# AY-Liu/Image-Editing-Framework

Hardware: AMD Instinct MI355X
Metric: denoising steps/sec (SD1.5 512x512 P2P edit step, UNet batch 4) (higher is better)
Workload: dtype f16x3; 1 GPU; sd15 UNet (859.5M params) P2P AttentionRefine edit step, 2 prompts x CFG = batch 4, 64x64 latents (512x512 px), 50-step DDIM, guidance 7.5, cross 0.8 / self 0.4, per-step null-text unconditional embeddings (P2P_NTI, edit_real.py); one independent edit per GPU; precision mode f16x3: fp32 storage; every contraction on split operands: hi + lo fp16 halves of each fp32 element, Ah Bh + Al Bh + Ah Bl =

## Files before the change

image-editing-framework_amd/control.py:

```python
from typing import Optional

import torch

from . import hip

XL = 96


def _step_hook(c):
    fn = getattr(c, "between_steps", None) or getattr(c, "after_step", None)
    if fn is not None:
        fn()


def advance_controller(c):
    c.cur_att_layer += 1
    uncond = c.num_att_layers if getattr(c, "LOW_RESOURCE", False) else 0
    if c.cur_att_layer == c.num_att_layers + uncond:
        c.cur_att_layer = 0
        c.cur_step += 1
        _step_hook(c)


class StepCounter:

    def __init__(self, num_att_layers: int = 0):
        self.cur_step, self.cur_att_layer, self.num_att_layers = 0, 0, num_att_layers

    def between_steps(self):
        pass

    def reset(self):
        self.cur_step, self.cur_att_layer = 0, 0


class ControlPlan:
    MASA_KINDS = ("masactrl", "masactrl_mask", "masactrl_mask_auto", "masactrl_union")
    GATED_KINDS = ("masactrl_mask", "masactrl_mask_auto")
    MAP_TOKENS, CTX_TOKENS = 256, 77

    def __init__(self, controller, kind: str, device, num_prompts: int = 1, num_steps: int = 0,
                 mt: Optional[torch.Tensor] = None, coef_table: Optional[torch.Tensor] = None,
                 self_window=(0, 0), self_max_tokens: int = 256, masa_steps=(), masa_layers=(),
                 pnp_layers=(), pnp_qk_steps: int = 0, pnp_conv_steps: int = 0, cond_only: bool = False,
                 mask_s: Optional[torch.Tensor] = None, mask_t: Optional[torch.Tensor] = None, mask_tokens=(),
                 auto_slots=None, auto_layers=None, auto_thres: float = 0.1, auto_ref=(), auto_cur=(), blend=None):
        self.controller = controller
        self.kind = kind
        self.device = torch.device(device)
        self.num_prompts = num_prompts
        self.cond_only = bool(cond_only)
        self.batch = num_prompts if cond_only else 2 * num_prompts
        self.num_steps = num_steps
        self.self_window = self_window
        self.self_max_tokens = self_max_tokens
        self.captured = False
        self.muted = False
        dev = self.device
        self.step = torch.zeros(1, dtype=torch.int32, device=dev)
        B, Bp = self.batch, num_prompts
        self.blend_modules = ()
        self.blend_w = self.blend_w_cur = self.blend_acc = self.blend_thres = None
        if blend is not None:
            mods, bw, thres = blend
            assert kind == "p2p" and not cond_only and tuple(bw.shape) == (num_steps + 1, Bp, 2, XL)
            self.blend_modules = tuple(int(i) for i in mods)
            self.blend_w = bw.to(device=dev, dtype=torch.float32).contiguous()
            self.blend_w_cur = torch.zeros(Bp, 2, XL, dtype=torch.float32, device=dev)
            self.blend_acc = torch.zeros(Bp, self.MAP_TOKENS, dtype=torch.float32, device=dev)
            self.blend_thres = torch.tensor([float(thres)], dtype=torch.float32, device=dev)
        if kind == "p2p":
            slots = Bp - 1
            assert mt.shape == (slots, XL, XL) and coef_table.shape == (num_steps + 1, slots, 2, XL)
            self.mt = mt.to(device=dev, dtype=torch.float16).contiguous()
            self.mt32 = mt.to(device=dev, dtype=torch.float32).contiguous()
            self.coef_table = coef_table.to(device=dev, dtype=torch.float32).contiguous()
            self.coef_cur = torch.zeros(slots, 2, XL, dtype=torch.float32, device=dev)
            ct = coef_table.detach().float()
            self.coef_bound = float((ct[:, :, 0].abs() + ct[:, :, 1].abs()).max()) if ct.numel() else 1.0
            off = 0 if cond_only else Bp
            es = torch.full((B,), -1, dtype=torch.int32)
            sl = torch.zeros(B, dtype=torch.int32)
            for k in range(slots):
                es[off + 1 + k] = off
                sl[off + 1 + k] = k
            self.edit_src, self.edit_slot = es.to(dev), sl.to(dev)
            ident = torch.arange(B, dtype=torch.int32)
            repl = ident.clone()
            repl[off + 1:] = off
            tab = ident.repeat(num_steps + 1, 1)
            lo, hi = self_window
            tab[lo:hi] = repl
            self.self_table = tab.contiguous().to(dev)
            self.self_cur = ident.clone().to(dev)
        self.masa_steps = set(int(s) for s in masa_steps)
        self.masa_layers = set(int(l) for l in masa_layers)
        self._masa = {}
        self._union = {}
        self._step_synced = -1
        self.mask_s = None if mask_s is None else mask_s.detach().float().cpu()
        self.mask_t = None if mask_t is None else mask_t.detach().float().cpu()
        self.mask_tokens = tuple(sorted(set(int(n) for n in mask_tokens)))
        self._mask_lists = {}
        self._gate = None
        self._mask_rows = {}
        self.auto_slots = dict(auto_slots or {})
        self.auto_layers = dict(auto_layers or {})
        self.auto_thres = float(auto_thres)
        self.auto_ref, self.auto_cur = [int(i) for i in auto_ref], [int(i) for i in auto_cur]
        self._auto = None
        self._auto_cls = {}
        self.pnp_layers = set(pnp_layers)
        self.pnp_qk_steps, self.pnp_conv_steps = int(pnp_qk_steps), int(pnp_conv_steps)
        self._pnp = {}

    @staticmethod
    def masa_table(masa_steps, B: int):
        n = (max(masa_steps) + 2) if masa_steps else 1
        ident = torch.arange(B, dtype=torch.int32)
        src = ident.clone()
        half = B // 2
        if half > 0:
            src[:half] = 0
            src[half:] = half
        tab = ident.repeat(n, 1)
        for st in masa_steps:
            tab[int(st)] = src
        return tab.contiguous()

    @classmethod
    def union_tables(cls, masa_steps):
        tab = cls.masa_table(masa_steps, 4)
        k2 = torch.full_like(tab, -1)
        for st in masa_steps:
            k2[int(st)] = torch.tensor([-1, 1, -1, 3], dtype=torch.int32)
        return tab, k2.contiguous()

    def prepare(self, B: int):
        if self.kind == "masactrl_union":
            if B != 4:
                raise RuntimeError(f"MasaCtrl Union acts on the UNet batch [u_src, u_tgt, c_src, c_tgt]; got batch {B}")
            if B not in self._union:
                k2 = self.union_tables(self.masa_steps)[1]
                self._union[B] = (k2.to(self.device), torch.full((B,), -1, dtype=torch.int32, device=self.device))
        if self.kind in self.GATED_KINDS:
            if B != 4:
                raise RuntimeError(f"mask-guided MasaCtrl acts on the UNet batch [u_src, u_tgt, c_src, c_tgt]; got batch {B}")
            n = (max(self.masa_steps) + 2) if self.masa_steps else 1
            if self._gate is None:
                g = torch.zeros(n, 1, dtype=torch.int32)
                for st in self.masa_steps:
                    g[st] = 1
                self._gate = (g.to(self.device), torch.zeros(1, dtype=torch.int32, device=self.device))
            if B not in self._mask_rows:
                half = B // 2
                self._mask_rows[B] = (torch.tensor([half - 1, B - 1], dtype=torch.int32, device=self.device),
                                      torch.tensor([0, half], dtype=torch.int32, device=self.device))
            for N in self.mask_tokens:
                self.mask_lists(N)
            if self.kind == "masactrl_mask_auto":
                if self._auto is None:
                    K = max(len(self.auto_slots), 1)
                    self._auto = (torch.zeros(K, 2, self.MAP_TOKENS, dtype=torch.float32, device=self.device),
                                  self.auto_weights().to(self.device),
                                  torch.tensor([self.auto_thres], dtype=torch.float32, device=self.device))
                for ei, (c, N) in self.auto_layers.items():
                    if c >= 1:
                        self._class_words(ei, N)
        if self.kind in self.MASA_KINDS and B not in self._masa:
            tab = self.masa_table(self.masa_steps, B)
            self.num_steps = max(self.num_steps, tab.shape[0] - 1)
            self._masa[B] = (tab.to(self.device), torch.arange(B, dtype=torch.int32, device=self.device))
        if self.kind == "pnp" and B not in self._pnp:
            ident = torch.arange(B, dtype=torch.int32)
            inj = ident.clone()
            s = B // 4
            if s > 0 and B == 4 * s:
                inj[s:2 * s] = ident[2 * s:3 * s]
                inj[3 * s:4 * s] = ident[2 * s:3 * s]
            n = self.num_steps + 1
            qk, cv = ident.repeat(n, 1), ident.repeat(n, 1)
            qk[: self.pnp_qk_steps] = inj
            cv[: self.pnp_conv_steps] = inj
            dev = self.device
            self._pnp[B] = (qk.contiguous().to(dev), ident.clone().to(dev), cv.contiguous().to(dev), ident.clone().to(dev))

    @staticmethod
    def resized_mask(mask, N: int):
        H = W = int(N ** 0.5)
        if H * W != N:
            raise ValueError(f"mask-guided MasaCtrl needs square token grids, got {N} tokens")
        return torch.nn.functional.interpolate(mask[None, None], (H, W)).flatten()

    def mask_lengths(self, N: int):
        ms, mt = self.resized_mask(self.mask_s, N), self.resized_mask(self.mask_t, N)
        return tuple(int((m == v).sum()) for m, v in ((ms, 1), (ms, 0), (mt, 1), (mt, 0)))

    def mask_lists(self, N: int):
        if N not in self._mask_lists:
            if self.captured:
                raise RuntimeError(f"ControlPlan.prepare(B) must build the mask lists of {N} tokens before graph capture")
            ms, mt = self.resized_mask(self.mask_s, N), self.resized_mask(self.mask_t, N)
            ls = [torch.nonzero(m == v).flatten().to(torch.int32) for m, v in ((ms, 1), (ms, 0), (mt, 1), (mt, 0))]
            if ls[0].numel() == 0 or ls[1].numel() == 0:
                raise RuntimeError(f"mask_s has an empty key class at {N} tokens: no fused rule there.  The lowering checked the "
                                   f"token counts of the UNet's configured sample size {self.mask_tokens}; run at that size, "
                                   "or register a subclass of the editor to take the generic path")
            self._mask_lists[N] = tuple(t.to(self.device) for t in ls)
            self.mask_tokens = tuple(sorted(set(self.mask_tokens) | {N}))
        return self._mask_lists[N]

    def mask_launches(self, B: int, N: int, attn):
# ... 33 lines not shown
            raise RuntimeError(f"{attn.layer_name}: the auto-mask plan was lowered for the UNet's configured sample size, where "
                               f"this module has {'256' if slot is not None else 'not 256'} queries; it runs at {N}.  Run at "
                               "that size, or register a subclass of the editor to take the generic path")
        if slot is None or self.muted:
            return
        if B != 4 or q.shape[0] != B or k.shape[0] != B or k.shape[1] != self.CTX_TOKENS:
            raise RuntimeError(f"masactrl_mask_auto: cross-attention of batch {tuple(q.shape)} x {tuple(k.shape)}; the rule is "
                               f"stated for the batch [u_src, u_tgt, c_src, c_tgt] and {self.CTX_TOKENS} prompt tokens")
        slots, w, _ = self._auto
        hip.cross_token_mass(q, k, attn.heads, attn.scale, (B // 2, B - 1), w, slots[slot])

    def _blend_mass(self, B: int, N: int, attn, q, k):
        if attn._exec_index not in self.blend_modules:
            return
        if N != self.MAP_TOKENS:
            raise RuntimeError(f"{attn.layer_name}: the blend was lowered for the UNet's configured sample size, where this module has "
                               f"{self.MAP_TOKENS} queries; it runs at {N}, where LocalBlend's 16 x 16 reshape does not hold")
        if self.muted or not self.applies(B):
            return
        if q.shape[0] != B or k.shape[0] != B or k.shape[1] != self.CTX_TOKENS:
            raise RuntimeError(f"LocalBlend: cross-attention of batch {tuple(q.shape)} x {tuple(k.shape)}; the rule is stated for the "
                               f"full CFG batch of {B} rows and {self.CTX_TOKENS} prompt tokens")
        hip.cross_blend_mass(q, k, attn.heads, attn.scale, self.num_prompts, self.blend_w_cur, self.blend_acc)

    def blend_latents(self, x):
        if self.blend_w is not None and not self.muted:
            hip.local_blend(self.blend_acc, self.blend_thres, x)
        return x

    def _rewound(self, step: int):
        if self.blend_acc is not None and step == 0:
            self.blend_acc.zero_()

    def auto_launch(self, B: int, N: int, attn):
        if self.kind != "masactrl_mask_auto" or (attn._exec_index // 2) not in self.masa_layers:
            return None
        c = self.auto_layers.get(attn._exec_index, (0, N))[0]
        if c < 1:
            return None
        kc, qc = self._class_words(attn._exec_index, N)
        if self.muted:
            return None
        tgt, src = self._mask_rows[B]
        slots, _, thres = self._auto
        hip.masa_auto_classes(slots, c, thres, int(N ** 0.5), kc, qc, gate=self._gate[1])
        return tgt, src, self._gate[1], kc, qc

    def class_bits(self, layer: int, N: int = None):
        for (ei, n), (kc, qc) in self._auto_cls.items():
            if ei // 2 == layer and (N is None or n == N):
                return hip.unpack_class_bits(kc, n), hip.unpack_class_bits(qc, n)
        raise KeyError(f"no class words for layer {layer}")

    def controls_first_self(self, unet, tokens: int) -> bool:
        blk = unet.down_blocks[0]
        if not blk.attentions:
            return False
        first = blk.attentions[0].transformer_blocks[0].attn1
        if self.kind == "p2p":
            return tokens <= self.self_max_tokens or (first._exec_index + 1) in self.blend_modules
        if self.kind == "masactrl_mask_auto" and (first._exec_index + 1) in self.auto_slots:
            return True
        if self.kind in self.MASA_KINDS:
            return (first._exec_index // 2) in self.masa_layers
        if self.kind == "pnp":
            return id(first) in self.pnp_layers
        return False

    def signature(self, unet):
        if self.kind == "p2p":
            sig = ("p2p", self.num_prompts, self.num_steps, self.self_max_tokens, tuple(self.mt.shape), self.cond_only,
                   hip.map_split_scale(self.coef_bound))
            return sig if self.blend_w is None else sig + ("blend", self.blend_modules)
        if self.kind == "masactrl":
            return ("masactrl", tuple(sorted(self.masa_layers)), (max(self.masa_steps) + 2) if self.masa_steps else 1)
        if self.kind == "masactrl_union":
            return ("masactrl_union", tuple(sorted(self.masa_layers)), (max(self.masa_steps) + 2) if self.masa_steps else 1)
        if self.kind == "masactrl_mask":
            lens = tuple((N, self.mask_lengths(N)) for N in self.mask_tokens)
            return ("masactrl_mask", tuple(sorted(self.masa_layers)), (max(self.masa_steps) + 2) if self.masa_steps else 1, lens)
        if self.kind == "masactrl_mask_auto":
            return ("masactrl_mask_auto", tuple(sorted(self.masa_layers)), (max(self.masa_steps) + 2) if self.masa_steps else 1,
                    tuple(sorted(self.auto_slots.items())), tuple(sorted(self.auto_layers.items())))
        if self.kind == "pnp":
            idx = {id(m): m._exec_index for m in unet.attention_modules()}
            inj = (unet.up_blocks[1].resnets[0 if unet.cfg.addition_embed else 1]._inject is self
                   if len(unet.up_blocks) > 1 else False)
            return ("pnp", tuple(sorted(idx[i] for i in self.pnp_layers)), self.num_steps, bool(inj))
        return (self.kind,)

    def load_from(self, other: "ControlPlan", B: int):
        self.controller = other.controller
        if self.kind == "p2p":
            self.mt.copy_(other.mt)
            self.mt32.copy_(other.mt32)
            self.coef_table.copy_(other.coef_table)
            self.coef_bound = other.coef_bound
            self.self_table.copy_(other.self_table)
            self.self_window = other.self_window
            if self.blend_w is not None:
                self.blend_w.copy_(other.blend_w)
                self.blend_thres.copy_(other.blend_thres)
                if hasattr(self.controller, "_device_blend"):
                    self.controller._device_blend = self
        elif self.kind == "masactrl":
            other.prepare(B)
            self.masa_steps = set(other.masa_steps)
            self._masa[B][0].copy_(other._masa[B][0])
        elif self.kind == "masactrl_union":
            other.prepare(B)
            self.prepare(B)
            self.masa_steps = set(other.masa_steps)
            self._masa[B][0].copy_(other._masa[B][0])
            self._union[B][0].copy_(other._union[B][0])
        elif self.kind == "masactrl_mask":
            other.prepare(B)
            self.prepare(B)
            self.masa_steps = set(other.masa_steps)
            self.mask_s, self.mask_t = other.mask_s, other.mask_t
            self._masa[B][0].copy_(other._masa[B][0])
            self._gate[0].copy_(other._gate[0])
            for N in self.mask_tokens:
                if tuple(int(t.numel()) for t in self.mask_lists(N)) != other.mask_lengths(N):
                    raise RuntimeError(f"masactrl_mask: the captured graph holds lists of other lengths at {N} tokens than "
                                       "these masks give; this loop cannot be reused for them")
                for mine, theirs in zip(self.mask_lists(N), other.mask_lists(N)):
                    mine.copy_(theirs)
        elif self.kind == "masactrl_mask_auto":
            other.prepare(B)
            self.prepare(B)
            self.masa_steps = set(other.masa_steps)
            self.auto_thres, self.auto_ref, self.auto_cur = other.auto_thres, list(other.auto_ref), list(other.auto_cur)
            self._masa[B][0].copy_(other._masa[B][0])
            self._gate[0].copy_(other._gate[0])
            self._auto[1].copy_(other._auto[1])
            self._auto[2].copy_(other._auto[2])
        elif self.kind == "pnp":
            other.prepare(B)
            self.pnp_qk_steps, self.pnp_conv_steps = other.pnp_qk_steps, other.pnp_conv_steps
            self._pnp[B][0].copy_(other._pnp[B][0])
            self._pnp[B][2].copy_(other._pnp[B][2])

    def applies(self, B: int) -> bool:
        if self.kind == "empty" or self.muted:
            return False
        if self.kind in self.MASA_KINDS or self.kind == "pnp":
            return True
        if B != self.batch:
            raise RuntimeError(
                f"controller was built for {self.num_prompts} prompts (UNet batch {self.batch}) but the UNet was "
                f"called with batch {B}; the reference's AttentionControlEdit.forward would mis-reshape here")
        return True

    def begin_forward(self, B: int):
        if not self.applies(B):
            return
        if not self.captured:
            cs = int(self.controller.cur_step)
            if cs > self.num_steps and self.kind == "p2p":
                raise IndexError(f"cur_step {cs} exceeds the controller's {self.num_steps}-step tables")
            self.step.fill_(cs)
            self._rewound(cs)
        if self.kind == "p2p":
            hip.select_step(self.coef_table, self.coef_cur, self.step)
            hip.select_step(self.self_table, self.self_cur, self.step)
            if self.blend_w is not None:
                hip.select_step(self.blend_w, self.blend_w_cur, self.step)
        elif self.kind in self.MASA_KINDS:
            if B not in self._masa:
                if self.captured:
                    raise RuntimeError("ControlPlan.prepare(B) must run before graph capture")
                self.prepare(B)
            tab, cur = self._masa[B]
            if not self.captured and int(self.controller.cur_step) >= tab.shape[0]:
                self.step.fill_(tab.shape[0] - 1)
            hip.select_step(tab, cur, self.step)
            if self.kind in self.GATED_KINDS:
                hip.select_step(self._gate[0], self._gate[1], self.step)
            if self.kind == "masactrl_union":
                hip.select_step(self._union[B][0], self._union[B][1], self.step)
        elif self.kind == "pnp":
            if B not in self._pnp:
                if self.captured:
                    raise RuntimeError("ControlPlan.prepare(B) must run before graph capture")
                self.prepare(B)
            qk, qk_cur, cv, cv_cur = self._pnp[B]
            if not self.captured and int(self.controller.cur_step) >= qk.shape[0]:
                self.step.fill_(qk.shape[0] - 1)
            hip.select_step(qk, qk_cur, self.step)
            hip.select_step(cv, cv_cur, self.step)

    def end_forward(self, B: int):
        if (self.kind in self.MASA_KINDS or self.kind == "pnp") and not self.muted:
            hip.advance_step(self.step)
        elif self.kind != "empty" and not self.muted and B == self.batch:
            hip.advance_step(self.step)

    def layer_done(self, attn):
        if not self.captured and not self.muted and self.controller is not None:
            advance_controller(self.controller)

    def sync_step(self):
        self.step.fill_(int(self.controller.cur_step))
        self._rewound(int(self.controller.cur_step))

    def replay_done(self):
        c = self.controller
        if c is not None:
            c.cur_step += 1
            _step_hook(c)

    def self_sources(self, B: int, N: int, attn):
        if self.kind == "p2p" and self.applies(B) and N <= self.self_max_tokens:
            return self.self_cur, self.self_cur, None
        if self.kind in self.MASA_KINDS and not self.muted and (attn._exec_index // 2) in self.masa_layers:
            cur = self._masa[B][1]
            return None, cur, cur
        if self.kind == "pnp" and not self.muted and id(attn) in self.pnp_layers:
            cur = self._pnp[B][1]
            return cur, cur, None
        return None, None, None

    def second_sources(self, B: int, attn):
        if self.kind == "masactrl_union" and not self.muted and (attn._exec_index // 2) in self.masa_layers:
            return self._union[B][1]
        return None

    def feature_source(self, B: int):
        if self.kind == "pnp" and not self.muted and B in self._pnp:
            return self._pnp[B][3]
        return None

    def cross_edit(self, B: int, attn):
        if self.kind == "p2p" and self.applies(B):
            mt = self.mt32 if attn.to_q.weight.dtype == torch.float32 else self.mt
            args = dict(edit_src=self.edit_src, edit_slot=self.edit_slot, mt=mt, coef=self.coef_cur)
            if attn.to_q.weight.dtype == torch.float32:
                args["coef_bound"] = self.coef_bound
            return args
        return {}
```

image-editing-framework_amd/csrc/elementwise.hip:

```cpp
#include "ief_common.h"
#include "ief_params.h"

__global__ __launch_bounds__(256) void cfg_ddim_kernel(const float* __restrict__ eu, const float* __restrict__ ec,
                                                       const float* __restrict__ x, float* __restrict__ xo,
                                                       float* __restrict__ x0o, const float* __restrict__ coef,
                                                       long long n) {
    const float a_f = coef[0], a_t = coef[1], g = coef[2];
    const float sb_f = sqrtf(1.0f - a_f), sa_f = sqrtf(a_f), sa_t = sqrtf(a_t), sb_t = sqrtf(1.0f - a_t);
    for (long long i = (long long)blockIdx.x * 256 + threadIdx.x; i < n; i += (long long)gridDim.x * 256) {
        float e = ec[i];
        if (eu) { const float u = eu[i]; e = u + g * (e - u); }
        const float x0 = (x[i] - sb_f * e) / sa_f;
        if (x0o) x0o[i] = x0;
        xo[i] = sa_t * x0 + sb_t * e;
    }
}

extern "C" int ief_cfg_ddim_step_f32(const float* eps_u, const float* eps_c, const float* x, float* x_out,
                                     float* x0_out, const float* coef, long long n, void* stream) {
    if (!eps_c || !x || !x_out || !coef) return IEF_EINVAL;
    if (n <= 0) return IEF_ESHAPE;
    int grid = (int)((n + 255) / 256);
    if (grid > 2048) grid = 2048;
    hipLaunchKernelGGL(cfg_ddim_kernel, dim3(grid), dim3(256), 0, (hipStream_t)stream, eps_u, eps_c, x, x_out, x0_out,
// ... 109 lines not shown
}

__global__ __launch_bounds__(256) void pointwise_f32_kernel(const float* __restrict__ x, const float* __restrict__ w,
                                                            const float* __restrict__ bias, float* __restrict__ out,
                                                            int B, int Cin, int Cout, int HW) {
    const long long i = (long long)blockIdx.x * 256 + threadIdx.x;
    if (i >= (long long)B * HW) return;
    const int b = (int)(i / HW), p = (int)(i - (long long)b * HW);
    float xin[8];
    for (int c = 0; c < Cin; ++c) xin[c] = x[((long long)b * Cin + c) * HW + p];
    for (int o = 0; o < Cout; ++o) {
        float a = bias ? bias[o] : 0.f;
        for (int c = 0; c < Cin; ++c) a += w[o * Cin + c] * xin[c];
        out[((long long)b * Cout + o) * HW + p] = a;
    }
}
extern "C" int ief_pointwise_f32(const float* x, const float* w, const float* bias, float* out, int B, int Cin, int Cout,
                                 int HW, void* stream) {
    if (!x || !w || !out) return IEF_EINVAL;
    if (B <= 0 || HW <= 0 || Cin <= 0 || Cin > 8 || Cout <= 0 || Cout > 8) return IEF_ESHAPE;
    const long long n = (long long)B * HW;
    hipLaunchKernelGGL(pointwise_f32_kernel, dim3((unsigned)((n + 255) / 256)), dim3(256), 0, (hipStream_t)stream, x, w, bias,
                       out, B, Cin, Cout, HW);
    IEF_LAUNCH_CHECK();
    return IEF_OK;
}

__global__ __launch_bounds__(256) void add_f16_kernel(const half_t* __restrict__ a, const half_t* __restrict__ b,
                                                      half_t* __restrict__ o, long long n8, long long n) {
    for (long long i = (long long)blockIdx.x * 256 + threadIdx.x; i < n8; i += (long long)gridDim.x * 256) {
        const half8 x = ((const half8*)a)[i], y = ((const half8*)b)[i];
        half8 r;
#pragma unroll
        for (int e = 0; e < 8; ++e) r[e] = (half_t)((float)x[e] + (float)y[e]);
        ((half8*)o)[i] = r;
    }
    if (blockIdx.x == 0) for (long long i = n8 * 8 + threadIdx.x; i < n; i += 256) o[i] = (half_t)((float)a[i] + (float)b[i]);
}
extern "C" int ief_add_f16(const ief_half* a, const ief_half* b, ief_half* out, long long n, void* stream) {
    if (!a || !b || !out) return IEF_EINVAL;
    if (n <= 0) return IEF_ESHAPE;
    if (((uintptr_t)a | (uintptr_t)b | (uintptr_t)out) & 15) return IEF_EALIGN;
    const long long n8 = n / 8;
    int grid = (int)((n8 + 255) / 256);
    if (grid < 1) grid = 1;
    if (grid > 2048) grid = 2048;
    hipLaunchKernelGGL(add_f16_kernel, dim3(grid), dim3(256), 0, (hipStream_t)stream, a, b, out, n8, n);
    IEF_LAUNCH_CHECK();
    return IEF_OK;
}

__global__ __launch_bounds__(256) void gather_rows_kernel(const half_t* __restrict__ in, half_t* __restrict__ out,
                                                          const int* __restrict__ src, int B, long long row8) {
    const long long total = (long long)B * row8;
    for (long long i = (long long)blockIdx.x * 256 + threadIdx.x; i < total; i += (long long)gridDim.x * 256) {
        const int b = (int)(i / row8);
        const long long c = i - (long long)b * row8;
        ((half8*)out)[i] = ((const half8*)in)[(long long)src[b] * row8 + c];
    }
}
extern "C" int ief_gather_rows_f16(const ief_half* in, ief_half* out, const int* src, int B, long long row_elems, void* stream) {
    if (!in || !out || !src) return IEF_EINVAL;
    if (B <= 0 || row_elems <= 0 || (row_elems & 7)) return IEF_ESHAPE;
    if (((uintptr_t)in | (uintptr_t)out) & 15) return IEF_EALIGN;
    const long long total = (long long)B * (row_elems / 8);
    int grid = (int)((total + 255) / 256);
    if (grid > 2048) grid = 2048;
    hipLaunchKernelGGL(gather_rows_kernel, dim3(grid), dim3(256), 0, (hipStream_t)stream, in, out, src, B, row_elems / 8);
    IEF_LAUNCH_CHECK();
    return IEF_OK;
}

struct RepeatJobs { IefRepeatJob j[IEF_REPEAT_MAX_JOBS]; };
__global__ __launch_bounds__(256) void repeat_batch_kernel(const RepeatJobs jobs) {
    const IefRepeatJob jb = jobs.j[blockIdx.y];
    const long long per = jb.bytes >> 4, total = per * jb.blocks;
    const f32x4* __restrict__ src = (const f32x4*)jb.src;
    f32x4* __restrict__ dst = (f32x4*)jb.dst;
    for (long long i = (long long)blockIdx.x * 256 + threadIdx.x; i < total; i += (long long)gridDim.x * 256) {
        const long long k = i / per, c = i - k * per;
        const f32x4 v = src[i];
        dst[2 * k * per + c] = v;
        dst[(2 * k + 1) * per + c] = v;
    }
}
extern "C" int ief_repeat_batch(const IefRepeatJob* jobs, int njobs, void* stream) {
    if (!jobs) return IEF_EINVAL;
    if (njobs <= 0 || njobs > IEF_REPEAT_MAX_JOBS) return IEF_ESHAPE;
    RepeatJobs a = {};
    long long most = 0;
    for (int i = 0; i < njobs; ++i) {
        const IefRepeatJob& j = jobs[i];
        if (!j.src || !j.dst) return IEF_EINVAL;
        if (j.bytes <= 0 || j.blocks <= 0) return IEF_ESHAPE;
        if ((j.bytes & 15) || (((uintptr_t)j.src | (uintptr_t)j.dst) & 15)) return IEF_EALIGN;
        a.j[i] = j;
        const long long chunks = (j.bytes >> 4) * j.blocks;
        most = chunks > most ? chunks : most;
    }
    long long grid = (most + 255) / 256;
    if (grid > 2048) grid = 2048;
    hipLaunchKernelGGL(repeat_batch_kernel, dim3((unsigned)grid, (unsigned)njobs), dim3(256), 0, (hipStream_t)stream, a);
    IEF_LAUNCH_CHECK();
    return IEF_OK;
}

__global__ __launch_bounds__(256) void cast_f32_f16_kernel(const float* __restrict__ x, half_t* __restrict__ o, long long n) {
    for (long long i = (long long)blockIdx.x * 256 + threadIdx.x; i < n; i += (long long)gridDim.x * 256) o[i] = (half_t)x[i];
}
__global__ __launch_bounds__(256) void cast_f16_f32_kernel(const half_t* __restrict__ x, float* __restrict__ o, long long n) {
    for (long long i = (long long)blockIdx.x * 256 + threadIdx.x; i < n; i += (long long)gridDim.x * 256) o[i] = (float)x[i];
}
extern "C" int ief_cast_f32_to_f16(const float* x, ief_half* out, long long n, void* stream) {
    if (!x || !out) return IEF_EINVAL;
    if (n <= 0) return IEF_ESHAPE;
    int grid = (int)((n + 255) / 256);
    if (grid > 2048) grid = 2048;
    hipLaunchKernelGGL(cast_f32_f16_kernel, dim3(grid), dim3(256), 0, (hipStream_t)stream, x, out, n);
    IEF_LAUNCH_CHECK();
    return IEF_OK;
}
extern "C" int ief_cast_f16_to_f32(const ief_half* x, float* out, long long n, void* stream) {
    if (!x || !out) return IEF_EINVAL;
    if (n <= 0) return IEF_ESHAPE;
    int grid = (int)((n + 255) / 256);
    if (grid > 2048) grid = 2048;
    hipLaunchKernelGGL(cast_f16_f32_kernel, dim3(grid), dim3(256), 0, (hipStream_t)stream, x, out, n);
    IEF_LAUNCH_CHECK();
    return IEF_OK;
}

__global__ __launch_bounds__(256) void select_step_kernel(const uint32_t* __restrict__ table, uint32_t* __restrict__ out,
                                                          const int* __restrict__ step, long long words, int n_rows) {
    int row = step[0];
    row = row < 0 ? 0 : (row >= n_rows ? n_rows - 1 : row);
    const long long base = (long long)row * words;
    for (long long i = (long long)blockIdx.x * 256 + threadIdx.x; i < words; i += (long long)gridDim.x * 256)
        out[i] = table[base + i];
}
extern "C" int ief_select_step(const void* table, void* out, const int* step, long long bytes_per_step, int n_rows,
                               void* stream) {
    if (!table || !out || !step) return IEF_EINVAL;
    if (n_rows <= 0) return IEF_ESHAPE;
    if (bytes_per_step <= 0 || (bytes_per_step & 3)) return IEF_EALIGN;
    const long long words = bytes_per_step / 4;
    int grid = (int)((words + 255) / 256);
    if (grid > 1024) grid = 1024;
    hipLaunchKernelGGL(select_step_kernel, dim3(grid), dim3(256), 0, (hipStream_t)stream, (const uint32_t*)table,
                       (uint32_t*)out, step, words, n_rows);
    IEF_LAUNCH_CHECK();
    return IEF_OK;
}

__global__ void advance_step_kernel(int* step) { if (threadIdx.x == 0 && blockIdx.x == 0) step[0] += 1; }
extern "C" int ief_advance_step(int* step, void* stream) {
    if (!step) return IEF_EINVAL;
    hipLaunchKernelGGL(advance_step_kernel, dim3(1), dim3(64), 0, (hipStream_t)stream, step);
    IEF_LAUNCH_CHECK();
    return IEF_OK;
}

extern "C" int ief_abi_version(void) { return IEF_ABI_VERSION; }
extern "C" int ief_struct_size(int which) {
    switch (which) {
        case 0: return (int)sizeof(IefGemmParams);
        case 1: return (int)sizeof(IefAttnParams);
        case 2: return (int)sizeof(IefCrossParams);
        case 3: return (int)sizeof(IefAttnBwdParams);
        case 4: return (int)sizeof(IefMapLossParams);
        case 5: return (int)sizeof(IefGemmF32Params);
        case 6: return (int)sizeof(IefAttnF32Params);
        case 7: return (int)sizeof(IefGemmX3pParams);
        default: return -1;
    }
}
extern "C" const char* ief_target_arch(void) { return "gfx950"; }
```

image-editing-framework_amd/csrc/exact_f32.hip:

```cpp
#include "ief_common.h"
#include "ief_params.h"
#include "x3_common.h"

#define XBM 128
#define XBK 32
#define XLD 36

__device__ __forceinline__ float silu_x(float x) { return x / (1.0f + expf(-x)); }

struct RowCoord { int b, oy, ox, ok; };

template <bool CONV, bool TRANSB, int NT>
__global__ __launch_bounds__(256) void igemm_f32_kernel(const IefGemmF32Params p) {
    constexpr int XBN = 64 * NT;
    __shared__ __attribute__((aligned(16))) float smem_x[2 * (XBM + XBN) * XLD];
    float* As = smem_x;
    float* Bs = smem_x + 2 * XBM * XLD;
    const int tid = threadIdx.x, lane = tid & 63, wid = tid >> 6;
    const int wm = wid >> 1, wn = wid & 1;
    const int li = lane & 31, lh = lane >> 5;
    const int ntn = (p.N + XBN - 1) / XBN;
    const int tm = blockIdx.x / ntn, tn = blockIdx.x - tm * ntn;
    const int m0 = tm * XBM, n0 = tn * XBN;
    const float* A = p.A;
// ... 1342 lines not shown
}
extern "C" int ief_gather_rows_f32(const float* in, float* out, const int* src, int B, long long row_elems, void* stream) {
    if (!in || !out || !src) return IEF_EINVAL;
    if (B <= 0 || row_elems <= 0 || (row_elems & 3)) return IEF_ESHAPE;
    if (((uintptr_t)in | (uintptr_t)out) & 15) return IEF_EALIGN;
    const long long total = (long long)B * (row_elems / 4);
    int grid = (int)((total + 255) / 256);
    if (grid > 2048) grid = 2048;
    hipLaunchKernelGGL(gather_rows_f32_kernel, dim3(grid), dim3(256), 0, (hipStream_t)stream, (const f32x4*)in, (f32x4*)out, src,
                       B, row_elems / 4);
    IEF_LAUNCH_CHECK();
    return IEF_OK;
}

template <int CIN, bool PL = false>
__global__ __launch_bounds__(256) void conv_in_f32_kernel(const float* __restrict__ x, const float* __restrict__ w,
                                                          const float* __restrict__ bias, float* __restrict__ out, int B, int Cin,
                                                          int H, int Wd, int Cout, half_t* __restrict__ outp = nullptr,
                                                          long long plane = 0) {
    const int C4 = Cout >> 2;
    const long long total = (long long)B * H * Wd * C4;
    for (long long i = (long long)blockIdx.x * 256 + threadIdx.x; i < total; i += (long long)gridDim.x * 256) {
        const long long pix = i / C4;
        const int c4 = (int)(i - pix * C4);
        const int b = (int)(pix / (H * Wd));
        const int rem = (int)(pix - (long long)b * H * Wd);
        const int oy = rem / Wd, ox = rem - oy * Wd;
        f32x4 acc = {0.f, 0.f, 0.f, 0.f};
        if constexpr (CIN > 0) {
#pragma unroll
            for (int ky = 0; ky < 3; ++ky) {
                const int iy = oy + ky - 1;
                const bool yok = (unsigned)iy < (unsigned)H;
                float v[3][CIN];
                f32x4 wv[3][CIN];
#pragma unroll
                for (int kx = 0; kx < 3; ++kx) {
                    const int ix = ox + kx - 1;
                    const bool ok = yok && (unsigned)ix < (unsigned)Wd;
#pragma unroll
                    for (int ci = 0; ci < CIN; ++ci) {
                        v[kx][ci] = ok ? x[(((long long)b * CIN + ci) * H + iy) * Wd + ix] : 0.f;
                        wv[kx][ci] = *(const f32x4*)(w + ((long long)((ky * 3 + kx) * CIN + ci)) * Cout + c4 * 4);
                    }
                }
#pragma unroll
                for (int kx = 0; kx < 3; ++kx) {
                    const int ix = ox + kx - 1;
                    if (!(yok && (unsigned)ix < (unsigned)Wd)) continue;
#pragma unroll
                    for (int ci = 0; ci < CIN; ++ci)
#pragma unroll
                        for (int e = 0; e < 4; ++e) acc[e] += v[kx][ci] * wv[kx][ci][e];
                }
            }
        } else {
            for (int tap = 0; tap < 9; ++tap) {
                const int iy = oy + tap / 3 - 1, ix = ox + tap % 3 - 1;
                if ((unsigned)iy >= (unsigned)H || (unsigned)ix >= (unsigned)Wd) continue;
                for (int ci = 0; ci < Cin; ++ci) {
                    const float v = x[(((long long)b * Cin + ci) * H + iy) * Wd + ix];
                    const f32x4 wv = *(const f32x4*)(w + ((long long)(tap * Cin + ci)) * Cout + c4 * 4);
#pragma unroll
                    for (int e = 0; e < 4; ++e) acc[e] += v * wv[e];
                }
            }
        }
        if (bias) {
#pragma unroll
            for (int e = 0; e < 4; ++e) acc[e] += bias[c4 * 4 + e];
        }
        *(f32x4*)(out + pix * Cout + c4 * 4) = acc;
        if constexpr (PL) {
            half4 hh, ll;
            split4(acc, 1.0f, hh, ll);
            half_t* op = outp + pix * Cout + c4 * 4;
            *(half4*)op = hh;
            *(half4*)(op + plane) = ll;
        }
    }
}
extern "C" int ief_conv_in_f32act(const float* x, const float* w, const float* bias, float* out, int B, int Cin, int H, int Wd,
                                  int Cout, void* stream) {
    if (!x || !w || !out) return IEF_EINVAL;
    if (B <= 0 || H <= 0 || Wd <= 0 || Cin <= 0 || Cin > 8 || Cout <= 0 || (Cout & 3)) return IEF_ESHAPE;
    if (((uintptr_t)w | (uintptr_t)out) & 15) return IEF_EALIGN;
    const long long total = (long long)B * H * Wd * (Cout / 4);
    int grid = (int)((total + 255) / 256);
    if (grid > 8192) grid = 8192;
    if (Cin == 4) hipLaunchKernelGGL((conv_in_f32_kernel<4, false>), dim3(grid), dim3(256), 0, (hipStream_t)stream, x, w, bias, out, B, Cin, H, Wd, Cout, (half_t*)nullptr, 0ll);
    else hipLaunchKernelGGL((conv_in_f32_kernel<0, false>), dim3(grid), dim3(256), 0, (hipStream_t)stream, x, w, bias, out, B, Cin, H, Wd, Cout, (half_t*)nullptr, 0ll);
    IEF_LAUNCH_CHECK();
    return IEF_OK;
}

extern "C" int ief_conv_in_f32act_planes(const float* x, const float* w, const float* bias, float* out, ief_half* outp, long long plane,
                                         int B, int Cin, int H, int Wd, int Cout, void* stream) {
    if (!x || !w || !out || !outp) return IEF_EINVAL;
    if (B <= 0 || H <= 0 || Wd <= 0 || Cin <= 0 || Cin > 8 || Cout <= 0 || (Cout & 3) || plane <= 0 || (plane & 3)) return IEF_ESHAPE;
    if ((((uintptr_t)w | (uintptr_t)out) & 15) || ((uintptr_t)outp & 7)) return IEF_EALIGN;
    const long long total = (long long)B * H * Wd * (Cout / 4);
    int grid = (int)((total + 255) / 256);
    if (grid > 8192) grid = 8192;
    if (Cin == 4) hipLaunchKernelGGL((conv_in_f32_kernel<4, true>), dim3(grid), dim3(256), 0, (hipStream_t)stream, x, w, bias, out, B, Cin, H, Wd, Cout, (half_t*)outp, plane);
    else hipLaunchKernelGGL((conv_in_f32_kernel<0, true>), dim3(grid), dim3(256), 0, (hipStream_t)stream, x, w, bias, out, B, Cin, H, Wd, Cout, (half_t*)outp, plane);
    IEF_LAUNCH_CHECK();
    return IEF_OK;
}

__global__ __launch_bounds__(256) void conv_out_f32_kernel(const float* __restrict__ x, const float* __restrict__ w,
                                                           const float* __restrict__ bias, float* __restrict__ out, int B, int C,
                                                           int H, int Wd, int Cout) {
    const int sub = threadIdx.x & 15;
    const long long pix = (long long)blockIdx.x * 16 + (threadIdx.x >> 4);
    const long long total = (long long)B * H * Wd;
    const bool live = pix < total;
    const long long pc = live ? pix : 0;
    const int b = (int)(pc / (H * Wd));
    const int rem = (int)(pc - (long long)b * H * Wd);
    const int oy = rem / Wd, ox = rem - oy * Wd;
    const int C4 = C >> 2;
    float acc[8];
#pragma unroll
    for (int o = 0; o < 8; ++o) acc[o] = 0.f;
    if (live) {
        for (int tap = 0; tap < 9; ++tap) {
            const int ky = tap / 3, kx = tap - ky * 3;
            const int iy = oy + ky - 1, ix = ox + kx - 1;
            if ((unsigned)iy >= (unsigned)H || (unsigned)ix >= (unsigned)Wd) continue;
            const float* xp = x + (((long long)b * H + iy) * Wd + ix) * C;
            for (int c4 = sub; c4 < C4; c4 += 16) {
                const f32x4 v = *(const f32x4*)(xp + c4 * 4);
#pragma unroll
                for (int o = 0; o < 8; ++o) {
                    if (o < Cout) {
                        const f32x4 wv = *(const f32x4*)(w + ((long long)o * 9 + tap) * C + c4 * 4);
#pragma unroll
                        for (int e = 0; e < 4; ++e) acc[o] += v[e] * wv[e];
                    }
                }
            }
        }
    }
#pragma unroll
    for (int o = 0; o < 8; ++o) {
#pragma unroll
        for (int off = 8; off > 0; off >>= 1) acc[o] += __shfl_xor(acc[o], off);
    }
    if (live && sub == 0) {
        for (int o = 0; o < Cout; ++o) out[(((long long)b * Cout + o) * H + oy) * Wd + ox] = acc[o] + (bias ? bias[o] : 0.f);
    }
}
template <int CH>
__global__ __launch_bounds__(256) void conv_out_f32_lds_kernel(const float* __restrict__ x, const float* __restrict__ w,
                                                               const float* __restrict__ bias, float* __restrict__ out, int B, int C,
                                                               int H, int Wd, int Cout) {
    extern __shared__ __attribute__((aligned(16))) float wl_f32[];
    const int sub = threadIdx.x & 15;
    const long long pix = (long long)blockIdx.x * 16 + (threadIdx.x >> 4);
    const long long total = (long long)B * H * Wd;
    const bool live = pix < total;
    const long long pc = live ? pix : 0;
    const int b = (int)(pc / (H * Wd));
    const int rem = (int)(pc - (long long)b * H * Wd);
    const int oy = rem / Wd, ox = rem - oy * Wd;
    const int C4 = C >> 2;
    const int nw4 = (Cout * 9 * C) >> 2;
    for (int i = threadIdx.x; i < nw4; i += 256) ((f32x4*)wl_f32)[i] = ((const f32x4*)w)[i];
    __syncthreads();
    float acc[8];
#pragma unroll
    for (int o = 0; o < 8; ++o) acc[o] = 0.f;
#pragma unroll
    for (int ky = 0; ky < 3; ++ky) {
        const int iy = oy + ky - 1;
        const bool yok = live && (unsigned)iy < (unsigned)H;
        f32x4 v[3][CH];
#pragma unroll
        for (int kx = 0; kx < 3; ++kx) {
            const int ix = ox + kx - 1;
            const bool ok = yok && (unsigned)ix < (unsigned)Wd;
            const float* xp = x + (((long long)b * H + (ok ? iy : 0)) * Wd + (ok ? ix : 0)) * C;
#pragma unroll
            for (int j = 0; j < CH; ++j) {
                const int c4 = sub + 16 * j;
                v[kx][j] = (ok && c4 < C4) ? *(const f32x4*)(xp + c4 * 4) : f32x4{0.f, 0.f, 0.f, 0.f};
            }
        }
#pragma unroll
        for (int kx = 0; kx < 3; ++kx) {
            const int ix = ox + kx - 1;
            if (!(yok && (unsigned)ix < (unsigned)Wd)) continue;
            const int tap = ky * 3 + kx;
#pragma unroll
            for (int j = 0; j < CH; ++j) {
                const int c4 = sub + 16 * j;
                if (c4 < C4) {
#pragma unroll
                    for (int o = 0; o < 8; ++o) {
                        if (o < Cout) {
                            const f32x4 wv = *(const f32x4*)(wl_f32 + (o * 9 + tap) * C + c4 * 4);
#pragma unroll
                            for (int e = 0; e < 4; ++e) acc[o] += v[kx][j][e] * wv[e];
                        }
                    }
                }
            }
        }
    }
#pragma unroll
    for (int o = 0; o < 8; ++o) {
#pragma unroll
        for (int off = 8; off > 0; off >>= 1) acc[o] += __shfl_xor(acc[o], off);
    }
    if (live && sub == 0) {
        for (int o = 0; o < Cout; ++o) out[(((long long)b * Cout + o) * H + oy) * Wd + ox] = acc[o] + (bias ? bias[o] : 0.f);
    }
}
extern "C" int ief_conv_out_f32act(const float* x, const float* w, const float* bias, float* out, int B, int C, int H, int Wd,
                                   int Cout, void* stream) {
    if (!x || !w || !out) return IEF_EINVAL;
    if (B <= 0 || H <= 0 || Wd <= 0 || C <= 0 || (C & 3) || Cout <= 0 || Cout > 8) return IEF_ESHAPE;
    if (((uintptr_t)x | (uintptr_t)w) & 15) return IEF_EALIGN;
    const long long total = (long long)B * H * Wd;
    const size_t lds = (size_t)Cout * 9 * C * sizeof(float);
    const dim3 grid((unsigned)((total + 15) / 16));
    if (lds <= 48 * 1024 && C <= 320 && Cout <= 4) {
        if (C <= 128) hipLaunchKernelGGL(conv_out_f32_lds_kernel<2>, grid, dim3(256), lds, (hipStream_t)stream, x, w, bias, out, B, C, H, Wd, Cout);
        else hipLaunchKernelGGL(conv_out_f32_lds_kernel<5>, grid, dim3(256), lds, (hipStream_t)stream, x, w, bias, out, B, C, H, Wd, Cout);
    } else {
        hipLaunchKernelGGL(conv_out_f32_kernel, grid, dim3(256), 0, (hipStream_t)stream, x, w, bias, out, B, C, H, Wd, Cout);
    }
    IEF_LAUNCH_CHECK();
    return IEF_OK;
}

__global__ __launch_bounds__(256) void image_u8_kernel(const float* __restrict__ x, uint8_t* __restrict__ out, int B, int C, int H,
                                                       int Wd) {
    const long long total = (long long)B * H * Wd * C;
    for (long long i = (long long)blockIdx.x * 256 + threadIdx.x; i < total; i += (long long)gridDim.x * 256) {
        const int c = (int)(i % C);
        const long long pix = i / C;
        const int b = (int)(pix / ((long long)H * Wd));
        const long long rem = pix - (long long)b * H * Wd;
        float v = x[((long long)b * C + c) * H * Wd + rem] / 2.0f + 0.5f;
        v = fminf(fmaxf(v, 0.f), 1.f);
        out[i] = (uint8_t)(v * 255.0f);
    }
}
extern "C" int ief_image_u8(const float* x, unsigned char* out, int B, int C, int H, int Wd, void* stream) {
    if (!x || !out) return IEF_EINVAL;
    if (B <= 0 || C <= 0 || H <= 0 || Wd <= 0) return IEF_ESHAPE;
    const long long total = (long long)B * H * Wd * C;
    int grid = (int)((total + 255) / 256);
    if (grid > 4096) grid = 4096;
    hipLaunchKernelGGL(image_u8_kernel, dim3(grid), dim3(256), 0, (hipStream_t)stream, x, out, B, C, H, Wd);
    IEF_LAUNCH_CHECK();
    return IEF_OK;
}
```

image-editing-framework_amd/csrc/gemm_x3p.hip:

```cpp
#include "ief_common.h"
#include "ief_params.h"
#include "x3_common.h"

#include "x3p_common.h"

template <int BM, int BN, int WAVES_M, int WAVES_N, int NS, int NL, bool CONV>
__global__ __launch_bounds__(64 * (WAVES_M * WAVES_N + NL)) void igemm_x3p_kernel(const IefGemmX3pParams p) {
    constexpr int BK = XP_BK;
    constexpr int NWC = WAVES_M * WAVES_N;
    constexpr int NSW = NL > 0 ? NL : NWC;
    constexpr int PA = BM / 16, PB = BN / 16;
    constexpr int P = 2 * (PA + PB);
    constexpr int G = (P + NSW - 1) / NSW;
    constexpr int WM = BM / WAVES_M, WN = BN / WAVES_N, TM = WM / 16, TN = WN / 16;
    constexpr int SLOT = P * 16 * BK;
    constexpr int DUMP = NS * SLOT;
    static_assert(BM % 16 == 0 && BN % 16 == 0 && WM % 16 == 0 && WN % 16 == 0, "tile");
    static_assert(NS >= 2 && NS <= 4, "ring depth");
    static_assert((NS * SLOT + 512) * 2 <= 160 * 1024, "LDS");
    __shared__ __attribute__((aligned(1024))) half_t smem[NS * SLOT + 512];

    const int tid = threadIdx.x, lane = tid & 63;
    const int wave = __builtin_amdgcn_readfirstlane(tid >> 6);
    const int wr = wave / WAVES_N, wc = wave % WAVES_N;
// ... 232 lines not shown
                        asm volatile("s_waitcnt lgkmcnt(0)" ::: "memory");
                    }
                    XP_BARRIER();
                    if (k > kt_lo) mfma_frags();
                    if constexpr (NL == 0) { if (k + NS - 1 < nk) stage_tile((s + NS - 1) % NS); }
                    read_frags(smem + s * SLOT);
                }
            }
        }
        if (nk > kt_lo) mfma_frags();
    }
    if (!computes) return;

    constexpr int NP2 = TN / 2;
    const int cb = n0 + wc * WN;
    const float inv = p.inv_scale;
    if (p.splits > 1) {
        float* slab = p.ws + (long long)blockIdx.y * p.M * p.N;
#pragma unroll
        for (int i = 0; i < TM; ++i) {
            const int m = m0 + wr * WM + i * 16 + fr;
            if (m >= p.M) continue;
#pragma unroll
            for (int j = 0; j < TN; ++j) {
                const int n = j < 2 * NP2 ? cb + 32 * (j >> 1) + 8 * fq + 4 * (j & 1) : cb + j * 16 + 4 * fq;
                if (n < p.N) *(f32x4*)(slab + (long long)m * p.N + n) = acc[j][i] * inv;
            }
        }
        return;
    }
    if (p.geglu) {
#pragma unroll
        for (int i = 0; i < TM; ++i) {
            const int m = m0 + wr * WM + i * 16 + fr;
            float mu = 0.f, rs = 1.f;
            if (p.rstat_in && m < p.M) xp_ln_row(p, m, mu, rs);
#pragma unroll
            for (int P = 0; P < NP2; ++P) {
                const int nh = cb + 32 * P + 16 * (fq >> 1) + 4 * (fq & 1), ng = nh + 8;
                if (m >= p.M || nh >= p.N) continue;
                f32x4 hv = acc[2 * P][i] * inv, gv = acc[2 * P + 1][i] * inv;
                if (p.rstat_in) {
                    hv = (hv - *(const f32x4*)(p.colsum + nh) * mu) * rs;
                    gv = (gv - *(const f32x4*)(p.colsum + ng) * mu) * rs;
                }
                if (p.bias) { hv += *(const f32x4*)(p.bias + nh); gv += *(const f32x4*)(p.bias + ng); }
                f32x4 o;
#pragma unroll
                for (int e = 0; e < 4; ++e) o[e] = hv[e] * gelu_nb(gv[e]) * p.out_scale;
                const int no = cb / 2 + 16 * P + 4 * fq;
                if (p.Out) *(f32x4*)(p.Out + (long long)m * p.ldo + no) = o;
                if (p.OutP) {
                    half4 h, l;
                    split4(o, 1.0f, h, l);
                    half_t* op = p.OutP + (long long)m * p.ldp + no;
                    *(half4*)op = h;
                    *(half4*)(op + p.planeO) = l;
                }
            }
            if constexpr (TN & 1) {
                constexpr int j = TN - 1;
                const int nb = cb + j * 16, n = nb + 4 * fq;
                const bool lo_half = fq < 2;
                f32x4 v = acc[j][i] * inv;
                if (p.rstat_in && n < p.N) v = (v - *(const f32x4*)(p.colsum + n) * mu) * rs;
                if (p.bias && n < p.N) v += *(const f32x4*)(p.bias + n);
                const float x0 = __shfl_xor(lo_half ? v[2] : v[0], 32), x1 = __shfl_xor(lo_half ? v[3] : v[1], 32);
                const float o0 = (lo_half ? v[0] * gelu_nb(x0) : x0 * gelu_nb(v[2])) * p.out_scale;
                const float o1 = (lo_half ? v[1] * gelu_nb(x1) : x1 * gelu_nb(v[3])) * p.out_scale;
                const int no = nb / 2 + (lo_half ? 4 * fq : 4 * (fq - 2) + 2);
                if (m < p.M && nb < p.N) {
                    if (p.Out) *(f32x2*)(p.Out + (long long)m * p.ldo + no) = f32x2{o0, o1};
                    if (p.OutP) {
                        const half2_t h = __builtin_convertvector(f32x2{o0, o1}, half2_t);
                        float r0, r1;
                        asm("v_fma_mix_f32 %0, %1, 1.0, -%2 op_sel:[0,0,0] op_sel_hi:[0,0,1]" : "=v"(r0) : "v"(o0), "v"(h));
                        asm("v_fma_mix_f32 %0, %1, 1.0, -%2 op_sel:[0,0,1] op_sel_hi:[0,0,1]" : "=v"(r1) : "v"(o1), "v"(h));
                        half_t* op = p.OutP + (long long)m * p.ldp + no;
                        *(half2_t*)op = h;
                        *(half2_t*)(op + p.planeO) = __builtin_convertvector(f32x2{r0, r1}, half2_t);
                    }
                }
            }
        }
        return;
    }
    const int slots_out = (p.N + WN - 1) / WN;
#pragma unroll
    for (int i = 0; i < TM; ++i) {
        const int m = m0 + wr * WM + i * 16 + fr;
        const bool mok = m < p.M;
        float mu = 0.f, rs = 1.f;
        if (p.rstat_in && mok) xp_ln_row(p, m, mu, rs);
        f32x4 vv[TN];
#pragma unroll
        for (int j = 0; j < TN; ++j) vv[j] = f32x4{0.f, 0.f, 0.f, 0.f};
#pragma unroll
        for (int P = 0; P < NP2; ++P) {
            const int n = cb + 32 * P + 8 * fq;
            if (!mok || n >= p.N) continue;
            f32x4 v0 = acc[2 * P][i] * inv, v1 = acc[2 * P + 1][i] * inv;
            if (n + 4 < p.N) {
                if (p.rstat_in) {
                    v0 = (v0 - *(const f32x4*)(p.colsum + n) * mu) * rs;
                    v1 = (v1 - *(const f32x4*)(p.colsum + n + 4) * mu) * rs;
                }
                xp_store8(p, v0, v1, m, n);
                vv[2 * P] = v0; vv[2 * P + 1] = v1;
            } else {
                if (p.rstat_in) v0 = (v0 - *(const f32x4*)(p.colsum + n) * mu) * rs;
                vv[2 * P] = xp_store(p, v0, m, n);
            }
        }
        if constexpr (TN & 1) {
            constexpr int j = TN - 1;
            const int n = cb + j * 16 + 4 * fq;
            if (mok && n < p.N) {
                f32x4 v = acc[j][i] * inv;
                if (p.rstat_in) v = (v - *(const f32x4*)(p.colsum + n) * mu) * rs;
                vv[j] = xp_store(p, v, m, n);
            }
        }
        if (p.rstat_out) {
            float sm, sq;
            xp_row_stats<TN>(vv, sm, sq);
            if (fq == 0 && mok && cb < p.N) {
                float* ro = p.rstat_out + ((long long)m * slots_out + cb / WN) * 2;
                ro[0] = sm; ro[1] = sq;
            }
        }
    }
}

__global__ __launch_bounds__(256) void x3p_reduce_kernel(const IefGemmX3pParams p) {
    const int N4 = p.N >> 2;
    const long long total = (long long)p.M * N4, slab = (long long)p.M * p.N;
    for (long long i = (long long)blockIdx.x * 256 + threadIdx.x; i < total; i += (long long)gridDim.x * 256) {
        const int m = (int)(i / N4), n = (int)(i - (long long)m * N4) * 4;
        const float* w = p.ws + (long long)m * p.N + n;
        f32x4 a = *(const f32x4*)w;
        int s = 1;
        for (; s + 3 < p.splits; s += 4) {
            f32x4 t[4];
#pragma unroll
            for (int u = 0; u < 4; ++u) t[u] = *(const f32x4*)(w + (s + u) * slab);
#pragma unroll
            for (int u = 0; u < 4; ++u) a += t[u];
        }
        for (; s < p.splits; ++s) a += *(const f32x4*)(w + s * slab);
        xp_store(p, a, m, n);
    }
}

__global__ __launch_bounds__(256) void x3_split_act_kernel(const float* __restrict__ x, half_t* __restrict__ planes, long long plane,
                                                           long long rows, int C4, int ldx, int ldp, float scale) {
    const long long total = rows * C4;
    for (long long i = (long long)blockIdx.x * 256 + threadIdx.x; i < total; i += (long long)gridDim.x * 256) {
        const long long r = i / C4;
        const int c = (int)(i - r * C4) * 4;
        half4 h, l;
        split4(*(const f32x4*)(x + r * ldx + c), scale, h, l);
        half_t* o = planes + r * ldp + c;
        *(half4*)o = h;
        *(half4*)(o + plane) = l;
    }
}
extern "C" int ief_x3_split_act(const float* x, ief_half* planes, long long plane, long long rows, int C, int ldx, int ldp, float scale,
                                void* stream) {
    if (!x || !planes) return IEF_EINVAL;
    if (rows <= 0 || C <= 0 || (C & 3) || (ldx & 3) || (ldp & 3) || (plane & 3) || !(scale > 0.f)) return IEF_ESHAPE;
    if (((uintptr_t)x & 15) || ((uintptr_t)planes & 7)) return IEF_EALIGN;
    long long grid = (rows * (C / 4) + 255) / 256;
    if (grid > 16384) grid = 16384;
    hipLaunchKernelGGL(x3_split_act_kernel, dim3((unsigned)grid), dim3(256), 0, (hipStream_t)stream, x, (half_t*)planes, plane, rows,
                       C / 4, ldx, ldp, scale);
    IEF_LAUNCH_CHECK();
    return IEF_OK;
}

extern "C" int ief_gemm_x3p_tile_bm(int tile) {
    switch (tile) {
        case 1: case 2: case 3: case 7: return 128;
        case 4: case 8: case 11: case 12: case 13: return 256;
        case 5: return 64;
        case 6: return 128;
        default: return 0;
    }
}
extern "C" int ief_gemm_x3p_tile_wn(int tile) { return tile == 6 ? 64 : tile == 8 ? 160 : 80; }
extern "C" int ief_gemm_x3p_tile_bn(int tile) {
    switch (tile) {
        case 1: case 2: case 4: case 5: case 7: return 160;
        case 3: case 11: case 12: case 13: return 80;
        case 6: return 64;
        case 8: return 320;
        default: return 0;
    }
}

template <int BM, int BN, int WAVES_M, int WAVES_N, int NS, int NL>
static int launch_x3p(const IefGemmX3pParams& p, hipStream_t st) {
    const int tiles = ((p.M + BM - 1) / BM) * ((p.N + BN - 1) / BN);
    const int splits = p.splits > 1 ? p.splits : 1;
    constexpr int NT = 64 * (WAVES_M * WAVES_N + NL);
    if (p.conv) hipLaunchKernelGGL((igemm_x3p_kernel<BM, BN, WAVES_M, WAVES_N, NS, NL, true>), dim3(tiles, splits), dim3(NT), 0, st, p);
    else hipLaunchKernelGGL((igemm_x3p_kernel<BM, BN, WAVES_M, WAVES_N, NS, NL, false>), dim3(tiles, splits), dim3(NT), 0, st, p);
    IEF_LAUNCH_CHECK();
    return IEF_OK;
}

int ief_conv_halo_x3p_dispatch(const IefGemmX3pParams& p, hipStream_t st);

extern "C" int ief_gemm_x3p(const IefGemmX3pParams* pp, void* stream) {
    if (!pp || !pp->A || !pp->W || !pp->zeros || (!pp->Out && !pp->OutP)) return IEF_EINVAL;
    IefGemmX3pParams p = *pp;
    if (p.M <= 0 || p.N <= 0 || p.K <= 0 || (p.K % XP_BK) || (p.N & 3)) return IEF_ESHAPE;
    if (p.rowvec && p.rows_per_batch <= 0) return IEF_ESHAPE;
    if (p.splits > 1 && (!p.ws || p.splits > 64 || p.geglu || p.rstat_out || p.cstat_out)) return IEF_EINVAL;
    if (!(p.inv_scale > 0.f)) return IEF_EINVAL;
    if ((p.ldw & 7) || (p.planeW & 7) || ((uintptr_t)p.W & 15)) return IEF_EALIGN;
    if (p.Out && ((p.ldo & 3) || ((uintptr_t)p.Out & 15))) return IEF_EALIGN;
    if (p.OutP && ((p.ldp & 3) || (p.planeO & 3) || ((uintptr_t)p.OutP & 7))) return IEF_EALIGN;
    if ((p.bias && ((uintptr_t)p.bias & 15)) || (p.rowvec && ((uintptr_t)p.rowvec & 15)) ||
        (p.residual && (((uintptr_t)p.residual & 15) || (p.ldr & 3)))) return IEF_EALIGN;
    if (p.geglu && ((p.N & 15) || p.residual || p.rowvec)) return IEF_EINVAL;
    if (p.rstat_out && (p.splits > 1 || p.geglu || p.tile == 11 || p.tile == 12 || p.tile == 13 || (p.N % ief_gemm_x3p_tile_wn(p.tile)))) return IEF_EINVAL;
    if (p.rstat_in && (!p.colsum || p.rstat_slots <= 0 || p.rstat_cnt <= 0 || p.rstat_slots * p.rstat_cnt != p.K || p.splits > 1 ||
                       p.conv || !(p.ln_eps > 0.f) || ((uintptr_t)p.colsum & 15))) return IEF_EINVAL;
    if (p.conv) {
        if (p.C1 <= 0 || p.C2 < 0 || (p.C1 % XP_BK) || (p.C2 % XP_BK) || (p.CE1 % XP_BK) || (p.CE2 % XP_BK)) return IEF_ESHAPE;
        if ((p.C2 > 0 && !p.A2) || (p.CE1 > 0 && !p.E1) || (p.CE2 > 0 && !p.E2) || (p.CE2 > 0 && p.CE1 == 0)) return IEF_EINVAL;
        if (p.stride != 1 && p.stride != 2) return IEF_ESHAPE;
        if (p.ups != 0 && p.ups != 1) return IEF_ESHAPE;
        if (p.ups && ((p.H | p.Wd) & 1)) return IEF_ESHAPE;
        if ((p.CE1 + p.CE2) > 0 && (p.stride != 1 || p.ups)) return IEF_ESHAPE;
        const int ktaps = p.tile == 13 ? 4 : 9;
        if (p.K != ktaps * (p.C1 + p.C2) + p.CE1 + p.CE2 || p.batch_images <= 0 || p.M != p.batch_images * p.Ho * p.Wo) return IEF_ESHAPE;
        const long long in_pix = (long long)p.batch_images * (p.H >> p.ups) * (p.Wd >> p.ups);
        const int cmax = p.C1 > p.C2 ? p.C1 : p.C2, emax = p.CE1 > p.CE2 ? p.CE1 : p.CE2;
        if (in_pix * cmax * 2 >= (1ll << 32) || (long long)p.M * emax * 2 >= (1ll << 32)) return IEF_ESHAPE;
        if (((uintptr_t)p.A & 15) || (p.planeA & 7) || (p.A2 && (((uintptr_t)p.A2 & 15) || (p.planeA2 & 7))) ||
            (p.E1 && (((uintptr_t)p.E1 & 15) || (p.planeE1 & 7))) || (p.E2 && (((uintptr_t)p.E2 & 15) || (p.planeE2 & 7)))) return IEF_EALIGN;
    } else {
        if ((p.lda & 7) || (p.planeA & 7) || ((uintptr_t)p.A & 15)) return IEF_EALIGN;
    }
    hipStream_t st = (hipStream_t)stream;
    int rc;
    switch (p.tile) {
        case 2: rc = launch_x3p<128, 160, 4, 2, 4, 4>(p, st); break;
        case 3: rc = launch_x3p<128, 80, 4, 1, 3, 0>(p, st); break;
        case 4: rc = launch_x3p<256, 160, 4, 2, 3, 0>(p, st); break;
        case 5: rc = launch_x3p<64, 160, 2, 2, 4, 0>(p, st); break;
        case 6: rc = launch_x3p<128, 64, 4, 1, 3, 0>(p, st); break;
        case 7: rc = launch_x3p<128, 160, 2, 2, 2, 0>(p, st); break;
        case 8: rc = launch_x3p<256, 320, 4, 2, 2, 0>(p, st); break;
        case 11: case 12: case 13: rc = ief_conv_halo_x3p_dispatch(p, st); break;
        case 1: default: rc = launch_x3p<128, 160, 4, 2, 4, 0>(p, st); break;
    }
    if (rc) return rc;
    if (p.splits > 1) {
        const long long total = (long long)p.M * (p.N / 4);
        int grid = (int)((total + 255) / 256);
        if (grid > 8192) grid = 8192;
        hipLaunchKernelGGL(x3p_reduce_kernel, dim3(grid), dim3(256), 0, st, p);
        IEF_LAUNCH_CHECK();
    }
    return IEF_OK;
}
```

image-editing-framework_amd/csrc/x3p_common.h:

```cpp
#pragma once
#include "ief_common.h"
#include "ief_params.h"
#include "x3_common.h"

typedef __attribute__((address_space(3))) void lds_void_t;
typedef const __attribute__((address_space(1))) void glb_void_t;
__device__ __forceinline__ void glds16(const char* g, half_t* lds_wave_base) {
    __builtin_amdgcn_global_load_lds((glb_void_t*)g, (lds_void_t*)lds_wave_base, 16, 0, 0);
}

#define XP_BK 32
#define XP_GROUP_M 8
#define XP_BARRIER() asm volatile("s_barrier" ::: "memory")
__device__ __forceinline__ int xp_swz(int row) { return (row >> 1) & 2; }
#define XP_LANE_CHUNK(lane) (((lane) & 3) ^ (((lane) >> 3) & 2))

__device__ __forceinline__ f32x4 xp_store(const IefGemmX3pParams& p, f32x4 v, int m, int n) {
    if (p.bias) v += *(const f32x4*)(p.bias + n);
    if (p.rowvec) v += *(const f32x4*)(p.rowvec + (long long)(m / p.rows_per_batch) * p.N + n);
    if (p.residual) v += *(const f32x4*)(p.residual + (long long)m * p.ldr + n);
    v = v * p.out_scale;
    if (p.Out) *(f32x4*)(p.Out + (long long)m * p.ldo + n) = v;
    if (p.OutP) {
        half4 h, l;
        split4(v, 1.0f, h, l);
        half_t* o = p.OutP + (long long)m * p.ldp + n;
        *(half4*)o = h;
        *(half4*)(o + p.planeO) = l;
    }
    return v;
}

template <int WN>
__device__ __forceinline__ int xp_perm_col(int q, bool geglu) {
    constexpr int TN = WN / 16, NP2 = TN / 2;
    const int w = q / WN, lq = q - w * WN, jb = lq >> 4, rho = lq & 15;
    if (jb >= 2 * NP2) return q;
    const int P = jb >> 1, b = jb & 1;
    const int off = geglu ? 32 * P + 16 * (rho >> 3) + 8 * b + (rho & 7) : 32 * P + 8 * (rho >> 2) + 4 * b + (rho & 3);
    return w * WN + off;
}

__device__ __forceinline__ void xp_store8(const IefGemmX3pParams& p, f32x4& v0, f32x4& v1, int m, int n) {
    if (p.bias) { v0 += *(const f32x4*)(p.bias + n); v1 += *(const f32x4*)(p.bias + n + 4); }
    if (p.rowvec) {
        const float* rv = p.rowvec + (long long)(m / p.rows_per_batch) * p.N + n;
        v0 += *(const f32x4*)rv; v1 += *(const f32x4*)(rv + 4);
    }
    if (p.residual) {
        const float* rr = p.residual + (long long)m * p.ldr + n;
        v0 += *(const f32x4*)rr; v1 += *(const f32x4*)(rr + 4);
    }
    v0 = v0 * p.out_scale; v1 = v1 * p.out_scale;
    if (p.Out) {
        float* o = p.Out + (long long)m * p.ldo + n;
        *(f32x4*)o = v0; *(f32x4*)(o + 4) = v1;
    }
    if (p.OutP) {
        half4 h0, l0, h1, l1;
        split4(v0, 1.0f, h0, l0);
        split4(v1, 1.0f, h1, l1);
        half_t* o = p.OutP + (long long)m * p.ldp + n;
        if ((((uintptr_t)o | (uintptr_t)(p.planeO * 2)) & 15) == 0) {
            *(half8*)o = half8{h0[0], h0[1], h0[2], h0[3], h1[0], h1[1], h1[2], h1[3]};
            *(half8*)(o + p.planeO) = half8{l0[0], l0[1], l0[2], l0[3], l1[0], l1[1], l1[2], l1[3]};
        } else {
            *(half4*)o = h0; *(half4*)(o + 4) = h1;
            *(half4*)(o + p.planeO) = l0; *(half4*)(o + p.planeO + 4) = l1;
        }
    }
}

__device__ __forceinline__ void xp_ln_row(const IefGemmX3pParams& p, int m, float& mean, float& rstd) {
    const float* rs = p.rstat_in + (long long)m * p.rstat_slots * 2;
    const float cnt = (float)p.rstat_cnt;
    float n = cnt, mu = rs[0], m2 = rs[1];
    for (int t = 1; t < p.rstat_slots; ++t) {
        const float mb = rs[2 * t], qb = rs[2 * t + 1];
        const float nn = n + cnt, d = mb - mu;
        mu += d * (cnt / nn);
        m2 += qb + d * d * (n * cnt / nn);
        n = nn;
    }
    mean = mu;
    rstd = 1.0f / sqrtf(m2 / n + p.ln_eps);
}
template <int NV>
__device__ __forceinline__ void xp_row_stats(const f32x4 (&v)[NV], float& mean, float& m2) {
    float s = 0.f;
#pragma unroll
    for (int j = 0; j < NV; ++j) s += (v[j][0] + v[j][1]) + (v[j][2] + v[j][3]);
    float mu = s * (1.0f / (4 * NV)), q = 0.f;
#pragma unroll
    for (int j = 0; j < NV; ++j) {
        const f32x4 d = v[j] - mu;
        q += (d[0] * d[0] + d[1] * d[1]) + (d[2] * d[2] + d[3] * d[3]);
    }
    float n = 4.f * NV;
#pragma unroll
    for (int off = 16; off <= 32; off <<= 1) {
        const float mb = __shfl_xor(mu, off), qb = __shfl_xor(q, off);
        const float d = mb - mu;
        q = q + qb + d * d * (n * 0.5f);
        mu = 0.5f * (mu + mb);
        n *= 2.f;
    }
    mean = mu; m2 = q;
}
```

image-editing-framework_amd/denoise.py:

```python
import logging
import os
from typing import Dict, List, Optional

import torch

from . import hip

REUSE_GRAPHS = os.environ.get("IEF_REUSE_GRAPHS", "1") == "1"
_POOL: Dict[tuple, list] = {}
_POOL_CAP = 8

CFG_SHARED_PREFIX = os.environ.get("IEF_CFG_SHARED_PREFIX", "1") == "1"
_log = logging.getLogger("ief_amd.denoise")
_said = set()


def cfg_shared_prefix_reason(*, mode, cfg, x3p, aug, first_block_cross, native, fused_cross, ln_folded, plan_on_first_self,
                             taps=False, enabled=True):
    if not enabled:
        return "switched off (IEF_CFG_SHARED_PREFIX=0)"
    if mode != "denoise" or not cfg:
        return "not a classifier-free-guidance denoising loop"
    if not x3p:
        return "the trunk does not run on f16x3 operand planes"
    if aug:
        return "the additional (text-time) embedding differs between the halves of the batch"
    if not first_block_cross:
        return "down_blocks[0] has no cross-attention"
    if not native:
        return "an attention module of down_blocks[0] is on the generic (hooked) path"
    if not fused_cross:
        return "the first cross-attention does not take the fused split-operand kernel"
    if ln_folded:
        return "the transformer LayerNorms are folded (IEF_X3P_FOLD_LN=1)"
    if taps:
        return "intermediate tensors are tapped"
    if plan_on_first_self:
        return "the control plan acts on the self-attention of the first transformer"
    return None


def _check_finite(lat, unet):
    if not bool(torch.isfinite(lat).all()):
        mode = getattr(unet, "precision", "f16")
        hint = ("an operand left the fp16 range (|x| > 65504): run this model with precision=\"f32\" (IEF_PRECISION=f32 / --precision f32), "
                "the fp32-input MFMA has the fp32 range" if mode != "f32" else "check the inputs / weights")
        raise FloatingPointError(f"non-finite latents after the denoising loop (precision={mode}): {hint}")


class FusedDenoiser:
    def __init__(self, model, context: torch.Tensor, num_latents: int, latent_hw, guidance_scale: Optional[float],
                 mode: str = "denoise", uncond_list: Optional[List[torch.Tensor]] = None, use_graph: bool = True,
                 added_cond_kwargs=None):
        self.model, self.unet, self.sched = model, model.unet, model.scheduler
        dev = self.unet.device
        self.mode = mode
        self.cfg = guidance_scale is not None
        self.Bp = num_latents
        self.B = 2 * num_latents if self.cfg else num_latents
        if context.shape[0] != self.B:
            raise ValueError(f"context batch {context.shape[0]} != UNet batch {self.B}")
        h, w = latent_hw
        C = self.unet.config.in_channels
        self.lat = torch.zeros(self.Bp, C, h, w, dtype=torch.float32, device=dev)
        self.shared_reason = self._shared_reason(context.shape[1])
        self.shared = self.shared_reason is None
        if (self.cfg and not self.shared and mode == "denoise" and CFG_SHARED_PREFIX and getattr(self.unet, "x3p", False)
                and self.shared_reason not in _said):
            _said.add(self.shared_reason)
            _log.warning("CFG step without the shared prefix: %s", self.shared_reason)
        self.lat_in = self.lat if (self.shared or not self.cfg) else torch.zeros(self.B, C, h, w, dtype=torch.float32, device=dev)
        self.step = torch.zeros(1, dtype=torch.int32, device=dev)
        self.coef_cur = torch.zeros(4, dtype=torch.float32, device=dev)
        self.coef_table = self.temb_table = self.temb_cur = self.ctx = self.ctx_table = None
        self._fill(context, guidance_scale, uncond_list, added_cond_kwargs)
        self.use_graph = use_graph
        self.graph = None
        self.plan = self.unet._plan
        self._keep, self._pooled_started, self._pool_key = None, False, None
        self._done = 0

    def _fill(self, context, guidance_scale, uncond_list, added_cond_kwargs=None):
        dev = self.unet.device
        ts = self.sched.timesteps.tolist()
        if self.mode == "invert":
            ts = ts[::-1]
            coef = [self.sched.reverse_coeffs(t) for t in ts]
        else:
            coef = [self.sched.step_coeffs(t) for t in ts]
        g = float(guidance_scale) if self.cfg else 1.0
        self.num_steps = len(ts)

        def put(name, value):
            cur = getattr(self, name)
            if cur is None:
                setattr(self, name, value)
            else:
                cur.copy_(value)

        put("coef_table", torch.tensor([[a, b, g, 0.0] for a, b in coef], dtype=torch.float32, device=dev))
        aug = self.unet.aug_embedding(added_cond_kwargs)
        if aug is not None and aug.shape[0] != self.B:
            raise ValueError(f"added_cond_kwargs batch {aug.shape[0]} != UNet batch {self.B}")
        rows = self.unet.time_rows(torch.tensor(ts, dtype=torch.float32, device=dev), aug)
        nb = 1 if aug is None else self.B
        put("temb_table", rows.reshape(len(ts), nb, -1).contiguous())
        if self.temb_cur is None:
            self.temb_cur = torch.zeros(nb, self.temb_table.shape[2], dtype=torch.float32, device=dev)
        ctx16 = self.unet._act(context.to(dev))
        if uncond_list is not None:
            rows = []
            for u in uncond_list:
                u16 = self.unet._act(u.to(dev)).expand(self.Bp, *ctx16.shape[1:])
                rows.append(torch.cat([u16, ctx16[self.Bp:]], 0))
            put("ctx_table", torch.stack(rows).contiguous())
            if self.ctx is None:
                self.ctx = torch.zeros_like(ctx16)
        else:
            put("ctx", ctx16.clone())

    def _shared_reason(self, ctx_len):
        facts = getattr(self.unet, "cfg_shared_facts", None)
        if facts is None:
            return "the UNet has no shared-prefix form"
        return cfg_shared_prefix_reason(mode=self.mode, cfg=self.cfg, enabled=CFG_SHARED_PREFIX and type(self)._step_body is FusedDenoiser._step_body,
                                        **facts(tuple(self.lat.shape[-2:]), ctx_len))

    def _key(self, context, uncond_list):
        plan = self.unet._plan
        return (id(self.unet), self.mode, self.Bp, tuple(self.lat.shape[-2:]), self.cfg, tuple(context.shape),
                None if uncond_list is None else len(uncond_list), len(self.sched.timesteps),
                None if plan is None else plan.signature(self.unet), self._shared_reason(context.shape[1]) is None,
                getattr(self.unet, "attn_key_splits", 1))

    def rebind(self, context, guidance_scale, uncond_list, added_cond_kwargs=None):
        self._fill(context, guidance_scale, uncond_list, added_cond_kwargs)
        if self.ctx_table is None:
            with hip.f32_contraction(getattr(self.unet, "contract", "f32")):
                for m, kv in self._keep:
                    hip.gemm(self.ctx, m.w_kv, out=kv)
        fresh = self.unet._plan
        if self.plan is not None:
            self.plan.load_from(fresh, self.B)
            self.plan.sync_step()
        self.step.zero_()
        self._done = 0

    def _step_body(self):
        hip.select_step(self.temb_table, self.temb_cur, self.step)
        hip.select_step(self.coef_table, self.coef_cur, self.step)
        if self.ctx_table is not None:
            hip.select_step(self.ctx_table, self.ctx, self.step)
        if self.cfg and self.shared:
            eps = self.unet(self.lat, encoder_hidden_states=self.ctx, temb_row=self.temb_cur, cfg_pair=True)["sample"]
        else:
            if self.cfg:
                self.lat_in[: self.Bp].copy_(self.lat)
                self.lat_in[self.Bp:].copy_(self.lat)
            eps = self.unet(self.lat_in, encoder_hidden_states=self.ctx, temb_row=self.temb_cur)["sample"]
        if self.cfg:
            hip.cfg_ddim_step(eps[: self.Bp], eps[self.Bp:], self.lat, self.coef_cur, out=self.lat)
        else:
            hip.cfg_ddim_step(None, eps, self.lat, self.coef_cur, out=self.lat)
        if self.plan is not None and self.cfg:
            self.plan.blend_latents(self.lat)
        hip.advance_step(self.step)

    def _set_kv_cache(self, on: bool):
        for m in self.unet.attention_modules():
            m.cache_kv = on

    def _capture(self):
        plan = self.plan
        self._set_kv_cache(self.ctx_table is None)
        saved = self.lat.clone()
        if plan is not None:
            plan.prepare(self.B)
            plan.muted = True
        used0 = hip.counters_used()
        s = torch.cuda.Stream()
        s.wait_stream(torch.cuda.current_stream())
        with torch.cuda.stream(s):
            self._step_body()
        torch.cuda.current_stream().wait_stream(s)
        torch.cuda.synchronize()
        if plan is not None:
            plan.muted = False
        self.lat.copy_(saved)
        self.step.zero_()
        if plan is not None:
            plan.sync_step()
            plan.captured = True
        self._arena = hip.counter_arena(hip.counters_used() - used0, self.lat.device)
        self.graph = torch.cuda.CUDAGraph()
        with self._arena, torch.cuda.graph(self.graph):
            self._step_body()
        self.lat.copy_(saved)
        self.step.zero_()
        if plan is not None:
            plan.sync_step()

    def start(self, latents: torch.Tensor):
        self.lat.copy_(latents.to(self.lat.device).float().expand_as(self.lat))
        self.step.zero_()
        self._done = 0
        if self.use_graph and self.graph is None:
            self._capture()
        elif not self.use_graph:
            self._set_kv_cache(self.ctx_table is None)
        if getattr(self, "_keep", None) is None or not self._pooled_started:
            self._keep = [(m, m._kv) for m in self.unet.attention_modules() if m.is_cross and m._kv is not None]
            self._pooled_started = True
        if self.plan is not None and self.graph is not None:
            self.plan.sync_step()

    def rewind(self, latents: Optional[torch.Tensor] = None):
        if latents is not None:
            self.lat.copy_(latents.to(self.lat.device).float().expand_as(self.lat))
        self.step.zero_()
        self._done = 0
        if self.plan is not None:
            self.plan.sync_step()

    def step_once(self):
        if self._done >= self.num_steps:
            raise IndexError(f"step {self._done} is past the {self.num_steps}-step schedule this loop was built for; "
                             "rewind() or start() it first")
        self._done += 1
        if self.graph is not None:
            self.graph.replay()
            if self.plan is not None:
                self.plan.replay_done()
        else:
            self._step_body()

    def result(self) -> torch.Tensor:
        return self.lat.clone()

    def run(self, latents: torch.Tensor, num_steps: Optional[int] = None, keep_all: bool = False):
        self.start(latents)
        n = self.num_steps if num_steps is None else num_steps
        traj = [self.lat.clone()] if keep_all else None
        for _ in range(n):
            self.step_once()
            if keep_all:
                traj.append(self.lat.clone())
        out = self.lat.clone()
        _check_finite(out, self.unet)
        return (out, traj) if keep_all else out

    def release(self):
        key = getattr(self, "_pool_key", None)
        if REUSE_GRAPHS and key is not None and self.graph is not None and len(_POOL.setdefault(key, [])) < _POOL_CAP:
            _POOL[key].append(self)
            return
        if self.plan is not None:
            self.plan.captured = False
        self.graph = None


def cfg_split_rows(context: torch.Tensor, num_latents: int, half: int) -> torch.Tensor:
    if context.shape[0] != 2 * num_latents or half not in (0, 1):
        raise ValueError("cfg_split_rows: context must be [2 * num_latents, ...] and half 0 or 1")
    return context[:num_latents] if half == 0 else context[num_latents:]


def exchange_eps(eps_all: torch.Tensor, mine: torch.Tensor, group=None):
    import torch.distributed as dist
    if dist.get_backend(group) == "gloo":
        parts = [torch.empty(mine.shape, dtype=mine.dtype) for _ in range(dist.get_world_size(group))]
        dist.all_gather(parts, mine.detach().cpu().contiguous(), group=group)
        eps_all.copy_(torch.cat(parts).to(eps_all.device))
    else:
        dist.all_gather_into_tensor(eps_all, mine.contiguous(), group=group)
    return eps_all


class CfgSplitDenoiser(FusedDenoiser):

    def __init__(self, model, context, num_latents, latent_hw, guidance_scale: float, group=None, uncond_list=None,
                 use_graph: bool = True):
        import torch.distributed as dist
        if dist.get_world_size(group) != 2:
            raise ValueError("a CFG split runs on a group of exactly two ranks")
        self.group = group
        self.half = dist.get_rank(group)
        self._guidance = float(guidance_scale)
        plan = model.unet._plan
        want = num_latents
        if plan is not None and plan.kind == "p2p" and (not plan.cond_only or self.half != 1 or plan.batch != want):
            raise ValueError('CFG split: register the controller with rows="cond" on rank 1 and rows="uncond" on rank 0')
        if plan is not None and plan.kind not in ("p2p", "empty"):
            raise ValueError(f"CFG split: a '{plan.kind}' control plan addresses the full CFG batch; only Prompt-to-Prompt "
                             'controllers registered with rows="cond" / "uncond" (or no controller) can be split')
        if plan is None and not all(m.is_native() for m in model.unet.attention_modules()):
            raise ValueError("CFG split: an attention hook is installed that was written for the full CFG batch")
        super().__init__(model, cfg_split_rows(context, num_latents, self.half), num_latents, latent_hw, None, mode="denoise",
                         uncond_list=uncond_list if self.half == 0 else None, use_graph=use_graph)
        C = self.unet.config.in_channels
        h, w = latent_hw
        self.eps_all = torch.zeros(2 * self.Bp, C, h, w, dtype=torch.float32, device=self.lat.device)
        self.eps_mine = torch.zeros(self.Bp, C, h, w, dtype=torch.float32, device=self.lat.device)
        self.graph_b = None

    def _fill(self, context, guidance_scale, uncond_list, added_cond_kwargs=None):
        super()._fill(context, None, uncond_list, added_cond_kwargs)
        self.coef_table[:, 2] = self._guidance

    def _forward_part(self):
        hip.select_step(self.temb_table, self.temb_cur, self.step)
        hip.select_step(self.coef_table, self.coef_cur, self.step)
        if self.ctx_table is not None:
            hip.select_step(self.ctx_table, self.ctx, self.step)
        eps = self.unet(self.lat, encoder_hidden_states=self.ctx, temb_row=self.temb_cur)["sample"]
        self.eps_mine.copy_(eps)

    def _update_part(self):
        hip.cfg_ddim_step(self.eps_all[: self.Bp], self.eps_all[self.Bp:], self.lat, self.coef_cur, out=self.lat)
        hip.advance_step(self.step)

    def _step_body(self):
        self._forward_part()
        exchange_eps(self.eps_all, self.eps_mine, self.group)
        self._update_part()

    def _capture(self):
        plan = self.plan
        self._set_kv_cache(self.ctx_table is None)
        saved = self.lat.clone()
        if plan is not None:
            plan.prepare(self.B)
            plan.muted = True
        used0 = hip.counters_used()
        s = torch.cuda.Stream()
        s.wait_stream(torch.cuda.current_stream())
        with torch.cuda.stream(s):
            self._forward_part()
        torch.cuda.current_stream().wait_stream(s)
        torch.cuda.synchronize()
        if plan is not None:
            plan.muted = False
        self.step.zero_()
        if plan is not None:
            plan.sync_step()
            plan.captured = True
        self._arena = hip.counter_arena(hip.counters_used() - used0, self.lat.device)
        self.graph = torch.cuda.CUDAGraph()
        with self._arena, torch.cuda.graph(self.graph):
            self._forward_part()
        self.graph_b = torch.cuda.CUDAGraph()
        with torch.cuda.graph(self.graph_b):
            self._update_part()
        self.lat.copy_(saved)
        self.step.zero_()
        if plan is not None:
            plan.sync_step()

    def step_once(self):
        if self._done >= self.num_steps:
            raise IndexError(f"step {self._done} is past the {self.num_steps}-step schedule this loop was built for")
        self._done += 1
        if self.graph is not None:
            self.graph.replay()
            exchange_eps(self.eps_all, self.eps_mine, self.group)
            self.graph_b.replay()
            if self.plan is not None:
                self.plan.replay_done()
        else:
            self._step_body()

    def release(self):
        if self.plan is not None:
            self.plan.captured = False
        self.graph = self.graph_b = None


def acquire(model, context, num_latents, latent_hw, guidance_scale, mode="denoise", uncond_list=None,
            use_graph=True, added_cond_kwargs=None) -> FusedDenoiser:
    if REUSE_GRAPHS and use_graph:
        probe = FusedDenoiser.__new__(FusedDenoiser)
        probe.unet, probe.sched, probe.mode = model.unet, model.scheduler, mode
        probe.cfg, probe.Bp = guidance_scale is not None, num_latents
        probe.lat = torch.empty(0, 0, *latent_hw)
        key = probe._key(context, uncond_list)
        free = _POOL.get(key)
        if free:
            loop = free.pop()
            loop.rebind(context, guidance_scale, uncond_list, added_cond_kwargs)
            return loop
        loop = FusedDenoiser(model, context, num_latents, latent_hw, guidance_scale, mode, uncond_list, use_graph,
                             added_cond_kwargs)
        loop._pool_key = key
        return loop
    return FusedDenoiser(model, context, num_latents, latent_hw, guidance_scale, mode, uncond_list, use_graph,
                         added_cond_kwargs)


def drop_pool():
    for loops in _POOL.values():
        for l in loops:
            l.graph = None
    _POOL.clear()


def run_interleaved(loops: List[FusedDenoiser], num_steps: Optional[int] = None):
    if not loops:
        return
    cur = torch.cuda.current_stream()
    streams = [torch.cuda.Stream() for _ in loops]
    for s in streams:
        s.wait_stream(cur)
    n = min(l.num_steps for l in loops) if num_steps is None else num_steps
    for _ in range(n):
        for loop, s in zip(loops, streams):
            with torch.cuda.stream(s):
                loop.step_once()
    for s in streams:
        cur.wait_stream(s)
```

image-editing-framework_amd/hip.py:

```python
import collections
import ctypes
import os
from ctypes import byref

import torch

from . import cabi

ABI_VERSION = cabi.defines["IEF_ABI_VERSION"]
REPEAT_MAX_JOBS = cabi.defines["IEF_REPEAT_MAX_JOBS"]
_LIB_PATH = os.environ.get("IEF_HIP_LIB") or os.path.join(os.path.dirname(os.path.abspath(__file__)), "libief_hip.so")
_lib = None


class HipExtensionMissing(RuntimeError):
    pass


IefGemmParams = cabi.structs["IefGemmParams"]
IefAttnParams = cabi.structs["IefAttnParams"]
IefCrossParams = cabi.structs["IefCrossParams"]
IefGemmF32Params = cabi.structs["IefGemmF32Params"]
IefAttnF32Params = cabi.structs["IefAttnF32Params"]
IefRepeatJob = cabi.structs["IefRepeatJob"]
IefGemmX3pParams = cabi.structs["IefGemmX3pParams"]
IefAttnBwdParams = cabi.structs["IefAttnBwdParams"]
IefAttnBwdF32Params = cabi.structs["IefAttnBwdF32Params"]
IefMapLossParams = cabi.structs["IefMapLossParams"]


def lib_path() -> str:
    return _LIB_PATH


def load():
    global _lib
    if _lib is not None:
        return _lib
    if not os.path.exists(_LIB_PATH):
        raise HipExtensionMissing(
            f"{_LIB_PATH} not found: build it with `python -c 'import __graft_entry__ as g; g.build()'` "
            "(or `make -C image-editing-framework_amd/csrc`).  There is no CPU fallback."
        )
    lib = ctypes.CDLL(_LIB_PATH)
    for name, (restype, argtypes) in cabi.functions.items():
        fn = getattr(lib, name)
        fn.restype, fn.argtypes = restype, argtypes
    if os.environ.get("IEF_X3_WIDE"):
        lib.ief_gemm_x3_set_variant(int(os.environ["IEF_X3_WIDE"]))
    if lib.ief_abi_version() != ABI_VERSION:
        raise HipExtensionMissing("libief_hip.so ABI version mismatch; rebuild")
    for which, st in ((0, IefGemmParams), (1, IefAttnParams), (2, IefCrossParams), (3, IefAttnBwdParams), (4, IefMapLossParams),
                      (5, IefGemmF32Params), (6, IefAttnF32Params), (7, IefGemmX3pParams)):
        if lib.ief_struct_size(which) != ctypes.sizeof(st):
            raise HipExtensionMissing(f"{st.__name__}: ctypes layout ({ctypes.sizeof(st)} B) != library "
                                      f"({lib.ief_struct_size(which)} B); rebuild libief_hip.so")
    _lib = lib
    return lib


_ERR = {-1: "IEF_EINVAL (null / missing pointer)", -2: "IEF_ESHAPE (unsupported shape)", -3: "IEF_EALIGN (alignment)"}


def _check(rc: int, what: str):
    if rc != 0:
        raise RuntimeError(f"{what} failed: {_ERR.get(rc, f'hipError {rc}')}")


def _stream() -> int:
    return torch.cuda.current_stream().cuda_stream


_prof = None
PROF_SHAPES = os.environ.get("IEF_PROF_SHAPES", "0") == "1"
_TILES = {1: (128, 128, 2, 2), 2: (64, 128, 2, 2), 3: (64, 64, 2, 2), 4: (128, 64, 2, 2), 5: (64, 160, 2, 2),
          6: (128, 160, 2, 2), 7: (128, 160, 4, 2), 8: (256, 128, 4, 2), 9: (128, 128, 4, 2),
          14: (256, 80, 8, 1), 15: (256, 80, 8, 1),
          16: (128, 160, 4, 2), 17: (128, 128, 4, 2), 18: (256, 128, 4, 2), 19: (64, 160, 2, 2), 20: (64, 64, 2, 2),
          21: (128, 160, 2, 2)}
_TILE_NL = {16: 4, 17: 4, 18: 4, 19: 2, 20: 2, 21: 2}
_HALO_TILES = (14, 15)


def _kname(tile, conv, stages=2):
    bm, bn, wm, wn = _TILES[tile]
    if tile in _HALO_TILES:
        return f"conv3x3_halo_kernel<{bm}, {bn}, {wm}, {wn}, {4 if tile == 15 else 0}>"
    return f"igemm_f16_kernel<{bm}, {bn}, {wm}, {wn}, {stages or 2}, {_TILE_NL.get(tile, 0)}, {'true' if conv else 'false'}>"


def _ring_bytes(tile, stages):
    bm, bn, wm, wn = _TILES[tile]
    if tile in _HALO_TILES:
        return 155776 if stages == 4 else 1 << 30
    rp = 64 * (_TILE_NL.get(tile, 0) or wm * wn) // 8
    rows = -(-bm // rp) * rp + -(-bn // rp) * rp
    return 2 * stages * rows * 64


_prof_staged = None


def profile_begin():
    global _prof, _prof_staged
    _prof = []
    _prof_staged = {}


def note_staged(name: str, nbytes: float):
    if _prof is not None and _prof_staged is not None:
        _prof_staged[name] = _prof_staged.get(name, 0.0) + nbytes


def profile_staged():
    return dict(_prof_staged or {})


def profile_end(with_bytes=False):
    global _prof
    rec, _prof = _prof, None
    torch.cuda.synchronize()
    if with_bytes:
        return [(name, flops, e0.elapsed_time(e1), nbytes) for name, flops, nbytes, e0, e1 in rec]
    return [(name, flops, e0.elapsed_time(e1)) for name, flops, nbytes, e0, e1 in rec]


class _Timed:

    def __init__(self, name, flops, nbytes=0.0):
        self.name, self.flops, self.nbytes = name, flops, nbytes

    def __enter__(self):
        if _prof is not None:
            self.e0, self.e1 = torch.cuda.Event(enable_timing=True), torch.cuda.Event(enable_timing=True)
            self.e0.record(torch.cuda.current_stream())

    def __exit__(self, *a):
        if _prof is not None:
            self.e1.record(torch.cuda.current_stream())
            _prof.append((self.name, self.flops, self.nbytes, self.e0, self.e1))


GN_CSTAT = os.environ.get("IEF_GN_CSTAT", "1") == "1"
HALO_HEURISTIC = os.environ.get("IEF_HALO_HEURISTIC", "1") == "1"
_CSTAT_MIN_HW = 256


class ColStats:
    __slots__ = ("buf", "bm", "hw", "ptr", "numel")

    def __init__(self, buf, bm, hw, out):
        self.buf, self.bm, self.hw = buf, bm, hw
        self.ptr, self.numel = out.data_ptr(), out.numel()

    def describes(self, t) -> bool:
        return t.data_ptr() == self.ptr and t.numel() == self.numel


def _attach_cstat(lib, p, out, M, N, hw):
    if not GN_CSTAT or hw is None or hw < _CSTAT_MIN_HW or (p.splits > 1 and not p.cnt) or (p.flags & 2) or AUTOTUNE:
        return None
    bm = lib.ief_gemm_tile_bm(p.tile_hint)
    if bm <= 0 or hw % bm or M % hw:
# ... 1175 lines not shown
            if o is not None:
                return o
        elif _F32_CONTRACT == "x3" and X3_FUSE_CROSS and k.shape[1] <= 96 and q.shape[2] // heads in (40, 64, 80, 160):
            return _attn_cross_p2p_x3(q, k, v, heads, scale, edit_src, edit_slot, mt, coef, out, out_planes, coef_bound)
        probs = _attn_scores_f32(q, k, heads, scale)
        if edit_src is not None:
            p2p_cross_edit_(probs, q.shape[0], heads, edit_src, edit_slot, mt, coef)
        o = _attn_apply_f32(probs, v, heads, None, out, map_scale=map_split_scale(coef_bound) if edit_src is not None else None)
        if out_planes:
            from . import planes as _pl
            return _pl.split(o)
        return o
    lib = load()
    if out is None:
        out = torch.empty(q.shape[0], q.shape[1], q.shape[2], dtype=torch.float16, device=q.device)
    p = IefCrossParams()
    _attn_common(p, q, k, v, out, heads)
    p.scale = scale
    p.edit_src, p.edit_slot = _ptr(_devi32(edit_src, "edit_src")), _ptr(_devi32(edit_slot, "edit_slot"))
    if edit_src is not None:
        _dev16(mt, "mt")
        _dev32(coef, "coef")
        if tuple(mt.shape[-2:]) != (96, 96) or not mt.is_contiguous() or coef.shape[-1] != 96:
            raise ValueError("attn_cross_p2p: mt must be [slots,96,96] fp16, coef [slots,2,96] fp32")
        p.MT, p.coef = mt.data_ptr(), coef.data_ptr()
    with _Timed(f"attn_cross_p2p_kernel<{p.d}>", 4.0 * p.B * p.heads * p.N * p.L * p.d,
                2.0 * p.B * p.heads * p.d * (2 * p.N + 2 * p.L)):
        _check(lib.ief_attn_cross_p2p_f16(byref(p), _stream()), "ief_attn_cross_p2p_f16")
    return out


def attn_probs(q, k, heads, scale, out=None):
    if _is32(q):
        return _attn_scores_f32(q, k, heads, scale, out=out)
    lib = load()
    B, N, C = q.shape
    L = k.shape[1]
    if out is None:
        probs = torch.empty(B * heads, N, L, dtype=torch.float16, device=q.device)
    else:
        probs = _dev16(out, "out")
        if tuple(probs.shape) != (B * heads, N, L) or not probs.is_contiguous():
            raise ValueError("attn_probs: out must be contiguous fp16 [B*heads, N, L]")
    p = IefAttnParams()
    _attn_common(p, q, k, k, q, heads)
    p.scale = scale
    _check(lib.ief_attn_probs_f16(byref(p), probs.data_ptr(), _stream()), "ief_attn_probs_f16")
    return probs


def attn_apply(probs, v, heads, out=None):
    if _is32(probs):
        return _attn_apply_f32(probs, v, heads, None, out)
    lib = load()
    _dev16(probs, "probs")
    if not probs.is_contiguous():
        raise ValueError("attn_apply: probs must be contiguous")
    B = v.shape[0]
    N, L = probs.shape[1], probs.shape[2]
    if probs.shape[0] != B * heads or v.shape[1] != L:
        raise ValueError("attn_apply: shape mismatch")
    if out is None:
        out = torch.empty(B, N, v.shape[2], dtype=torch.float16, device=v.device)
    p = IefAttnParams()
    _attn_common(p, out, v, v, out, heads)
    p.N, p.L = N, L
    _check(lib.ief_attn_apply_f16(byref(p), probs.data_ptr(), _stream()), "ief_attn_apply_f16")
    return out


def cfg_ddim_step(eps_u, eps_c, x, coef, out=None, x0_out=None):
    lib = load()
    _dev32(eps_c, "eps_c")
    _dev32(x, "x")
    _dev32(coef, "coef")
    if out is None:
        out = torch.empty_like(x)
    _check(lib.ief_cfg_ddim_step_f32(_ptr(eps_u), eps_c.data_ptr(), x.data_ptr(), out.data_ptr(), _ptr(x0_out),
                                     coef.data_ptr(), x.numel(), _stream()), "ief_cfg_ddim_step_f32")
    return out


def ddim_step(eps, x, a_from: float, a_to: float):
    coef = torch.tensor([a_from, a_to, 1.0], dtype=torch.float32, device=x.device)
    x0 = torch.empty_like(x, dtype=torch.float32)
    xf = x.float().contiguous()
    out = cfg_ddim_step(None, eps.float().contiguous(), xf, coef, x0_out=x0)
    return out, x0


def timestep_embedding(t, dim, dtype=torch.float16):
    lib = load()
    _dev32(t, "t")
    if dtype == torch.float32:
        out = torch.empty(t.shape[0], dim, dtype=torch.float32, device=t.device)
        _check(lib.ief_timestep_embedding_f32(t.data_ptr(), out.data_ptr(), t.shape[0], dim, _stream()),
               "ief_timestep_embedding_f32")
        return out
    out = torch.empty(t.shape[0], dim, dtype=torch.float16, device=t.device)
    _check(lib.ief_timestep_embedding_f16(t.data_ptr(), out.data_ptr(), t.shape[0], dim, _stream()),
           "ief_timestep_embedding_f16")
    return out


def silu(x):
    lib = load()
    if _is32(x):
        out = torch.empty_like(_act32(x, "x"))
        _check(lib.ief_silu_f32(x.contiguous().data_ptr(), out.data_ptr(), x.numel(), _stream()), "ief_silu_f32")
        return out
    _dev16(x, "x")
    out = torch.empty_like(x)
    _check(lib.ief_silu_f16(x.data_ptr(), out.data_ptr(), x.numel(), _stream()), "ief_silu_f16")
    return out


def to_f16(x, out=None):
    lib = load()
    _dev32(x, "x")
    if out is None:
        out = torch.empty(x.shape, dtype=torch.float16, device=x.device)
    _check(lib.ief_cast_f32_to_f16(x.data_ptr(), out.data_ptr(), x.numel(), _stream()), "ief_cast_f32_to_f16")
    return out


def to_f32(x, out=None):
    lib = load()
    _dev16(x, "x")
    if out is None:
        out = torch.empty(x.shape, dtype=torch.float32, device=x.device)
    _check(lib.ief_cast_f16_to_f32(x.contiguous().data_ptr(), out.data_ptr(), x.numel(), _stream()), "ief_cast_f16_to_f32")
    return out


def image_u8(x):
    lib = load()
    _dev32(x, "x")
    B, C, H, Wd = x.shape
    out = torch.empty(B, H, Wd, C, dtype=torch.uint8, device=x.device)
    _check(lib.ief_image_u8(x.data_ptr(), out.data_ptr(), B, C, H, Wd, _stream()), "ief_image_u8")
    return out


def select_step(table, out, step):
    lib = load()
    nbytes = out.numel() * out.element_size()
    if table[0].numel() * table.element_size() != nbytes or not table.is_contiguous() or not out.is_contiguous():
        raise ValueError("select_step: table[step] and out must have identical contiguous byte size")
    _check(lib.ief_select_step(table.data_ptr(), out.data_ptr(), _devi32(step, "step").data_ptr(), nbytes, table.shape[0],
                               _stream()), "ief_select_step")
    return out


def advance_step(step):
    lib = load()
    _check(lib.ief_advance_step(_devi32(step, "step").data_ptr(), _stream()), "ief_advance_step")


def cross_token_mass(q, k, heads, scale, rows, w, out):
    lib = load()
    _act32(q, "q"), _act32(k, "k"), _dev32(w, "w"), _dev32(out, "out")
    B, N, C = q.shape
    L = k.shape[1]
    if q.dim() != 3 or k.dim() != 3 or k.shape[0] != B or k.shape[2] != C or C % heads:
        raise ValueError("cross_token_mass: q [B, N, heads*d] and k [B, L, heads*d]")
    r0, r1 = int(rows[0]), int(rows[1])
    if not (0 <= r0 < B and 0 <= r1 < B):
        raise ValueError(f"cross_token_mass: rows {tuple(rows)} outside the batch of {B}")
    if tuple(w.shape) != (2, L) or tuple(out.shape) != (2, N):
        raise ValueError(f"cross_token_mass: w must be [2, {L}] and out [2, {N}]")
    with _Timed("cross_token_mass_f32_kernel", 4.0 * heads * N * L * (C // heads), 4.0 * 2 * C * (N + L)):
        _check(lib.ief_cross_token_mass_f32(q.data_ptr(), k.data_ptr(), w.data_ptr(), out.data_ptr(), r0, r1, heads, N, L, C // heads,
                                            q.stride(1), k.stride(1), q.stride(0), k.stride(0), float(scale), _stream()),
               "ief_cross_token_mass_f32")
    return out


def masa_auto_classes(slots, c, thres, res, k_cls, q_cls, gate=None):
    lib = load()
    _dev32(slots, "slots"), _dev32(thres, "thres"), _devi32(k_cls, "k_cls"), _devi32(q_cls, "q_cls"), _devi32(gate, "gate")
    c, res = int(c), int(res)
    if slots.dim() != 3 or tuple(slots.shape[1:]) != (2, 256) or not 1 <= c <= slots.shape[0]:
        raise ValueError("masa_auto_classes: slots must be [K, 2, 256] with 1 <= c <= K")
    if (res * res) % 32 or k_cls.numel() != res * res // 32 or q_cls.numel() != res * res // 32:
        raise ValueError("masa_auto_classes: k_cls / q_cls hold res*res / 32 words each")
    _check(lib.ief_masa_auto_classes(slots.data_ptr(), c, thres.data_ptr(), res, k_cls.data_ptr(), q_cls.data_ptr(), _ptr(gate),
                                     _stream()), "ief_masa_auto_classes")


def cross_blend_mass(q, k, heads, scale, row0, w, acc):
    lib = load()
    _act32(q, "q"), _act32(k, "k"), _dev32(w, "w"), _dev32(acc, "acc")
    if q.dim() != 3 or k.dim() != 3 or k.shape[0] != q.shape[0] or k.shape[2] != q.shape[2] or q.shape[2] % heads:
        raise ValueError("cross_blend_mass: q [B, N, heads*d] and k [B, L, heads*d]")
    B, N, C = q.shape
    L = k.shape[1]
    if w.dim() != 3 or w.shape[1] != 2 or w.shape[2] < L or acc.dim() != 2 or tuple(acc.shape) != (w.shape[0], N):
        raise ValueError(f"cross_blend_mass: w must be [Bp, 2, >= {L}] and acc [Bp, {N}]")
    Bp, row0 = w.shape[0], int(row0)
    if not (0 <= row0 and row0 + Bp <= B):
        raise ValueError(f"cross_blend_mass: rows {row0} .. {row0 + Bp - 1} outside the batch of {B}")
    with _Timed("cross_blend_mass_f32_kernel", 2.0 * (2 * Bp - 1) * heads * N * L * (C // heads), 4.0 * Bp * C * (N + L)):
        _check(lib.ief_cross_blend_mass_f32(q.data_ptr(), k.data_ptr(), w.data_ptr(), acc.data_ptr(), row0, Bp, heads, N, L, w.shape[2],
                                            C // heads, q.stride(1), k.stride(1), q.stride(0), k.stride(0), float(scale), _stream()),
               "ief_cross_blend_mass_f32")
    return acc


def local_blend(acc, thres, x):
    lib = load()
    _dev32(acc, "acc"), _dev32(thres, "thres"), _dev32(x, "x")
    if x.dim() != 4 or acc.dim() != 2 or tuple(acc.shape) != (x.shape[0], 256):
        raise ValueError("local_blend: x must be [Bp, C, H, W] and acc [Bp, 256]")
    Bp, C, H, W = x.shape
    _check(lib.ief_local_blend_f32(acc.data_ptr(), thres.data_ptr(), x.data_ptr(), Bp, C, H, W, _stream()), "ief_local_blend_f32")
    return x


def unpack_class_bits(words, n):
    w = words.detach().cpu().to(torch.int64) & 0xFFFFFFFF
    return ((w[:, None] >> torch.arange(32)) & 1).flatten()[:n].bool()


def pack_class_bits(bits, device=None):
    b = bits.detach().cpu().flatten().to(torch.int64)
    if b.numel() % 32:
        raise ValueError("pack_class_bits: the token count must be a multiple of 32")
    w = (b.reshape(-1, 32) << torch.arange(32)).sum(1)
    w = torch.where(w >= 2 ** 31, w - 2 ** 32, w).to(torch.int32)
    return w if device is None else w.to(device)


def map_loss_blocks(N, d):
    return load().ief_map_loss_blocks(int(N), int(d))


def attn_map_loss_bwd(q, k, ref, dq, heads, scale, gcoef, accumulate=True, loss=None, loss_coef=1.0):
    lib = load()
    if _is32(q):
        return _attn_map_loss_bwd_f32(q, k, ref, dq, heads, scale, gcoef, accumulate, loss, loss_coef)
    _dev16(q, "q"), _dev16(k, "k"), _dev16(ref, "ref"), _dev16(dq, "dq")
    B, N, C = q.shape
    L = k.shape[1]
    d = C // heads
    if tuple(ref.shape) != (B * heads, N, L) or not ref.is_contiguous():
        raise ValueError("attn_map_loss_bwd: ref must be contiguous fp16 [B*heads, N, L]")
    if tuple(dq.shape) != (B, N, C) or k.shape[0] != B or k.shape[2] != C:
        raise ValueError("attn_map_loss_bwd: shape mismatch")
    for nm, t in (("q", q), ("k", k), ("dq", dq)):
        if t.stride(2) != 1 or (t.shape[0] > 1 and t.stride(0) != t.shape[1] * t.stride(1)):
            raise ValueError(f"attn_map_loss_bwd: {nm} must be [B, rows, h*d] with batch stride rows * ld")
    p = IefMapLossParams()
    p.Q, p.K, p.ref, p.dQ = q.data_ptr(), k.data_ptr(), ref.data_ptr(), dq.data_ptr()
    p.B, p.heads, p.N, p.L, p.d = B, heads, N, L, d
    p.ldq, p.ldk, p.lddq = q.stride(1), k.stride(1), dq.stride(1)
    p.scale, p.gcoef, p.loss_coef, p.accumulate = scale, gcoef, loss_coef, 1 if accumulate else 0
    if loss is not None:
        if _dev32(loss, "loss").numel() < B * heads * lib.ief_map_loss_blocks(N, d):
            raise ValueError("attn_map_loss_bwd: loss needs B*heads*map_loss_blocks(N, d) floats")
        p.loss = loss.data_ptr()
    _check(lib.ief_attn_map_loss_bwd_f16(byref(p), _stream()), "ief_attn_map_loss_bwd_f16")
    return dq



def _transpose_maps_f32(x):
    lib = load()
    R, N, L = x.shape
    out = torch.empty(R, L, N, dtype=torch.float32, device=x.device)
    _check(lib.ief_transpose_batched_f32(_act32(x, "maps").data_ptr(), out.data_ptr(), R, N, L, _stream()), "ief_transpose_batched_f32")
    return out


def _attn_apply_t_f32(maps, x, heads, out=None):
    lib = load()
    _act32(maps, "maps"), _act32(x, "x")
    B, N, Cx = x.shape
    d = Cx // heads
    L = maps.shape[2]
    if tuple(maps.shape) != (B * heads, N, L) or not maps.is_contiguous():
        raise ValueError("attn_apply_t: maps must be contiguous [B*heads, N, L]")
    xt = x.reshape(B, N, heads, d).permute(0, 2, 3, 1).contiguous()
    tmp = torch.empty(B * heads, d, L, dtype=torch.float32, device=x.device)
    p = IefGemmF32Params()
    p.A, p.W, p.Out = xt.data_ptr(), maps.data_ptr(), tmp.data_ptr()
    p.M, p.N, p.K = d, L, N
    p.sAb, p.sAh, p.lda = heads * d * N, d * N, N
    p.sWb, p.sWh, p.ldw = heads * N * L, N * L, L
    p.sOb, p.sOh, p.ldo = heads * d * L, d * L, L
    p.batch, p.heads, p.out_scale, p.transb = B, heads, 1.0, 1
    kn = _set_x3(p, X3_SCALE_ACT, X3_SCALE_PROB)
    with _Timed(f"{kn}<apply^T {d}>", 2.0 * B * heads * N * L * d, 4.0 * B * heads * (N * d + L * d + N * L)):
        _check(lib.ief_gemm_f32(byref(p), _stream()), "ief_gemm_f32 (attention apply, transposed maps)")
    res = tmp.reshape(B, heads, d, L).permute(0, 3, 1, 2).reshape(B, L, heads * d)
    if out is None:
        return res.contiguous()
    out.copy_(res)
    return out


def _softmax_bwd_f32_(probs, dprobs, scale):
    lib = load()
    L = probs.shape[-1]
    _check(lib.ief_softmax_bwd_rows_f32(probs.data_ptr(), dprobs.data_ptr(), probs.numel() // L, L, float(scale), _stream()),
           "ief_softmax_bwd_rows_f32")
    return dprobs
# ... 437 lines not shown
```

image-editing-framework_amd/planes.py:

```python
import os
from ctypes import byref

import torch

from . import hip
from .hip import IefGemmX3pParams, _check, _dev32, _ptr, _stream, _Timed, _zeros

ACT_SCALE = 1.0
W_SCALE = hip.X3_SCALE_W


class Planes:
    __slots__ = ("t",)

    def __init__(self, t):
        if not (isinstance(t, torch.Tensor) and t.dtype == torch.float16 and t.dim() >= 2 and t.shape[0] == 2 and t.stride(-1) == 1):
            raise TypeError("Planes: expected an fp16 tensor [2, ...] with a contiguous last dimension")
        if not t.is_cuda:
            raise TypeError("Planes: device tensor expected (no CPU path)")
        self.t = t

    @staticmethod
    def empty(*shape, device):
        return Planes(torch.empty(2, *shape, dtype=torch.float16, device=device))
# ... 75 lines not shown
    global _plans
    if _plans is None:
        _plans = hip.read_plans(_PLAN_FILE)
    return _plans


def save_plans(path=None):
    hip.write_plans(path or _PLAN_FILE, _plan_table())


_TILES = {1: (128, 160), 2: (128, 160), 3: (128, 80), 4: (256, 160), 5: (64, 160), 6: (128, 64), 7: (128, 160), 8: (256, 320),
          11: (256, 80), 12: (256, 80), 13: (256, 80)}
_HALO = (11, 12, 13)


def heuristic_plan(M, N, K, conv=False):
    nk = K // 32
    if N % 80 and N % 64 == 0:
        tile = 6
    elif N % 160:
        tile = 3
    elif M <= 64:
        tile = 5
    else:
        t1 = -(-M // 128) * (N // 160)
        tile = 4 if t1 >= 1024 and M % 256 == 0 else 1
    bm, bn = _TILES[tile]
    tiles = -(-M // bm) * -(-N // bn)
    splits = 1
    if tiles < 160 and nk >= 16:
        splits = max(1, min(-(-256 // tiles), nk // 8, 16))
    return tile, splits


def pick_plan(M, N, K, conv=False, variant=""):
    hit = _plan_table().get(f"{'conv' if conv else 'gemm'}|{M}|{N}|{K}{variant}")
    if hit is None:
        hit = heuristic_plan(M, N, K, conv)
    if TILE_FORCE and (TILE_FORCE < 10 or conv):
        return TILE_FORCE, hit[1]
    return hit[0], hit[1]


AUTOTUNE = os.environ.get("IEF_AUTOTUNE_X3", "0") == "1"


def candidate_plans(M, N, K, conv=False, halo_ok=False, ncb=0, geglu=False, phase_ok=False):
    nk = K // 32
    out = []
    for t, (bm, bn) in _TILES.items():
        if t in _HALO:
            continue
        if N % bn or (t == 6 and N % 80 == 0):
            continue
        tiles = -(-M // bm) * (N // bn)
        for sp in (1, 2, 3, 4, 6, 8, 12, 16):
            if sp > 1 and (geglu or nk // sp < 4 or tiles * sp > 2048 or tiles >= 512):
                continue
            if tiles * sp < 40 and sp < 16:
                continue
            out.append((t, sp))
    if conv and halo_ok:
        tiles = -(-M // 256) * (N // 80)
        for sp in (1, 2, 3, 4, 5, 6, 8, 10, 12, 16, 20):
            if sp > 1 and (sp > ncb // 2 or tiles * sp > 1024 or tiles >= 384):
                continue
            if tiles * sp < 40 and sp < 16:
                continue
            out.append((11, sp))
    if conv and phase_ok:
        tiles = -(-(M // 4) // 256) * (N // 80) * 4
        for sp in (1, 2, 3, 4, 5, 6, 8, 10, 12, 16, 20):
            if sp > 1 and (sp > ncb // 2 or tiles * sp > 1024 or tiles >= 384):
                continue
            if tiles * sp < 40 and sp < 16:
                continue
            out.append((13, sp))
    return out


def _autotune(key, cands, run, w):
    wc = hip._cold_copies(w)
    for x in wc:
        weight_planes(x)
        if any(t == 13 for t, _ in cands):
            hip.x3_upsample_phase_planes(x, W_SCALE)
    best = None
    for t, sp in cands:
        try:
            us = hip._time_graph(lambda i: run(t, sp, wc[i % len(wc)]))
        except (RuntimeError, ValueError):
            continue
        if best is None or us < best[0]:
            best = (us, t, sp)
    for x in wc[1:]:
        hip._x3_planes.pop((x.data_ptr(), tuple(x.shape), float(W_SCALE)), None)
        hip._x3_planes.pop((x.data_ptr(), tuple(x.shape), float(W_SCALE), "phase"), None)
    if best is not None:
        _plan_table()[key] = (best[1], best[2])
    return best


def supported(N, K):
    return (N % 80 == 0 or N % 64 == 0) and K % 32 == 0


def _out_args(p, M, No, out, out_planes, device, lead_shape):
    o32 = op = None
    if out is True or isinstance(out, torch.Tensor) or (out is None and out_planes in (None, False)):
        o32 = out if isinstance(out, torch.Tensor) else torch.empty(*lead_shape, No, dtype=torch.float32, device=device)
        Mo, Nn, ldo = hip._rows_ld32(o32, "out")
        if (Mo, Nn) != (M, No):
            raise ValueError("x3p: out shape mismatch")
        p.Out, p.ldo = o32.data_ptr(), ldo
    if out_planes not in (None, False):
        op = out_planes if isinstance(out_planes, Planes) else Planes.empty(*lead_shape, No, device=device)
        Mp, Np, ldp = op.rows_ld("out_planes")
        if (Mp, Np) != (M, No):
            raise ValueError("x3p: out_planes shape mismatch")
        p.OutP, p.planeO, p.ldp = op.t.data_ptr(), op.plane, ldp
    return o32, op


def _ret(o32, op):
    if o32 is not None and op is not None:
        return o32, op
    return o32 if op is None else op


class RowStats:
    __slots__ = ("buf", "slots", "cnt")

    def __init__(self, buf, slots, cnt):
        self.buf, self.slots, self.cnt = buf, slots, cnt


class FoldedLN:
    __slots__ = ("w", "bias", "colsum", "eps")

    def __init__(self, w, bias, gamma, beta, eps):
        wf = (w * gamma[None, :]).contiguous()
        self.w = wf
        b = w @ beta
        self.bias = (b if bias is None else b + bias).contiguous()
        pl = weight_planes(wf)
        self.colsum = ((pl[0].float().sum(1) + pl[1].float().sum(1)) / W_SCALE).contiguous()
        self.eps = eps


LN_FOLD = os.environ.get("IEF_X3P_FOLD_LN", "0") == "1"


def gemm(a, w, bias=None, residual=None, rowvec=None, rows_per_batch=0, out=None, out_planes=None, out_scale=1.0,
         geglu=False, tile=0, splits=0, row_stats=False, ln=None):
    lib = hip.load()
    if not isinstance(a, Planes):
        raise TypeError("planes.gemm: a must be Planes")
    M, K, lda = a.rows_ld("a")
    N = w.shape[0]
    if w.dim() != 2 or w.shape[1] != K:
        raise ValueError(f"planes.gemm: K mismatch {tuple(w.shape)} vs {K}")
    wp = weight_planes(w)
    p = IefGemmX3pParams()
    p.A, p.planeA, p.lda = a.t.data_ptr(), a.plane, lda
    p.W, p.planeW, p.ldw = wp.data_ptr(), wp.stride(0), K
    No = N // 2 if geglu else N
    o32, op = _out_args(p, M, No, out, out_planes, a.device, a.shape[:-1])
    p.M, p.N, p.K = M, N, K
    p.out_scale, p.inv_scale = out_scale, 1.0 / (ACT_SCALE * W_SCALE)
    p.geglu, p.zeros = 1 if geglu else 0, _zeros(a.device)
    if tile:
        p.tile, p.splits = tile, max(1, splits)
    else:
        key = f"gemm|{M}|{N}|{K}" + ("|g" if geglu else "")
        if AUTOTUNE and key not in _plan_table() and not hip._capturing() and hip._prof is None:
            _autotune(key, candidate_plans(M, N, K, geglu=geglu),
                      lambda t, sp, wi: gemm(a, wi, bias=bias, residual=residual, rowvec=rowvec, rows_per_batch=rows_per_batch, out=out,
                                             out_planes=out_planes, out_scale=out_scale, geglu=geglu, tile=t, splits=sp), w)
        p.tile, p.splits = pick_plan(M, N, K, variant="|g" if geglu else "")
    if geglu or row_stats or ln is not None:
        p.splits = 1
    rs = None
    if row_stats:
        wn = lib.ief_gemm_x3p_tile_wn(p.tile)
        if N % wn:
            raise ValueError("planes.gemm: row statistics need N to be a multiple of the tile's wave width")
        rs = RowStats(torch.empty(M, N // wn, 2, dtype=torch.float32, device=a.device), N // wn, wn)
        p.rstat_out = rs.buf.data_ptr()
    if ln is not None:
        st, colsum, eps = ln
        if st.buf.shape[0] != M or st.slots * st.cnt != K or _dev32(colsum, "colsum").numel() != N:
            raise ValueError("planes.gemm: ln statistics / colsum do not match this launch")
        p.rstat_in, p.rstat_slots, p.rstat_cnt, p.colsum, p.ln_eps = st.buf.data_ptr(), st.slots, st.cnt, colsum.data_ptr(), eps
    ws = hip._fill_epilogue(p, hip._rows_ld32, "planes.gemm", M, N, a.device, bias, rowvec, rows_per_batch, residual, p.splits)
    nbytes = 4.0 * (M * K + N * K + M * No * ((1 if o32 is not None else 0) + (1 if op is not None else 0)) + (M * N if residual is not None else 0))
    kn = f"igemm_x3p_kernel<false> t{p.tile}" + (f" {M}x{N}x{K} s{p.splits}" if hip.PROF_SHAPES else "")
    bm, bn = _TILES[p.tile]
    hip.note_staged(kn, 4.0 * K * (bm + bn) * -(-M // bm) * -(-N // bn))
    with _Timed(kn, 2.0 * M * N * K, nbytes):
        _check(lib.ief_gemm_x3p(byref(p), _stream()), "ief_gemm_x3p")
    r = _ret(o32, op)
    if row_stats:
        return (r + (rs,)) if isinstance(r, tuple) else (r, rs)
    return r


def conv3x3(x, w, bias=None, x2=None, stride=1, upsample=False, rowvec=None, residual=None, out=None, out_planes=None,
            extra=None, pad_hi_only=False, tile=0, splits=0):
    lib = hip.load()
    if not isinstance(x, Planes) or (x2 is not None and not isinstance(x2, Planes)):
        raise TypeError("planes.conv3x3: x / x2 must be Planes")
    if not x.is_contiguous() or (x2 is not None and not x2.is_contiguous()) or not w.is_contiguous():
        raise ValueError("planes.conv3x3: x, x2, w must be contiguous")
    e1, e2 = (None, None) if extra is None else extra
    for e in (e1, e2):
        if e is not None and (not isinstance(e, Planes) or not e.is_contiguous()):
            raise ValueError("planes.conv3x3: extra sources must be contiguous NHWC Planes at the output resolution")
    if residual is not None and not hip._act32(residual, "residual").is_contiguous():
        raise ValueError("planes.conv3x3: residual must be contiguous fp32 [B, Ho, Wo, Cout]")
    g = hip.conv_geometry(x.shape, w.shape, hip._shape(x2), None if extra is None else (e1.shape, hip._shape(e2)), hip._shape(rowvec),
                          hip._shape(residual), stride, upsample, pad_hi_only, "planes.conv3x3")
    B, Hp, Wp, C1, C2, CE1, CE2, Cout, H, Wd, Ho, Wo, M, K = g[:14]
    p = IefGemmX3pParams()
    p.A, p.planeA = x.t.data_ptr(), x.plane
    if x2 is not None:
        p.A2, p.planeA2 = x2.t.data_ptr(), x2.plane
    if e1 is not None:
        p.E1, p.planeE1 = e1.t.data_ptr(), e1.plane
    if e2 is not None:
        p.E2, p.planeE2 = e2.t.data_ptr(), e2.plane
    o32, op = _out_args(p, M, Cout, out, out_planes, x.device, (B, Ho, Wo))
    p.M, p.N, p.K = M, Cout, K
    p.conv, p.H, p.Wd, p.C1, p.C2, p.Ho, p.Wo = 1, H, Wd, C1, C2, Ho, Wo
    p.stride, p.ups, p.batch_images, p.pad_hi_only = stride, 1 if upsample else 0, B, 1 if pad_hi_only else 0
    p.CE1, p.CE2 = CE1, CE2
    p.out_scale, p.inv_scale, p.zeros = 1.0, 1.0 / (ACT_SCALE * W_SCALE), _zeros(x.device)
    halo_ok = HALO and g.halo_geom and Cout % 80 == 0
    phase_ok = HALO and g.phase_geom and Cout % 80 == 0
    if tile:
        p.tile, p.splits = tile, max(1, splits)
    else:
        variant = ("|u" if upsample else "") + (f"|s{stride}" if stride != 1 else "") + ("|e" if extra is not None else "")
        key = f"conv|{M}|{Cout}|{K}{variant}"
        if AUTOTUNE and key not in _plan_table() and not hip._capturing() and hip._prof is None:
            _autotune(key, candidate_plans(M, Cout, K, conv=True, halo_ok=halo_ok, ncb=(C1 + C2) // 32, phase_ok=phase_ok),
                      lambda t, sp, wi: conv3x3(x, wi, bias, x2=x2, stride=stride, upsample=upsample, rowvec=rowvec, residual=residual,
                                                out=out, out_planes=out_planes, extra=extra, pad_hi_only=pad_hi_only, tile=t, splits=sp), w)
        hit = _plan_table().get(key)
        if hit is not None and (hit[0] not in _HALO or (phase_ok if hit[0] == 13 else halo_ok)):
            p.tile, p.splits = hit[0], hit[1]
        elif halo_ok:
            tiles, ncb = -(-M // 256) * (Cout // 80), (C1 + C2) // 32
            sp = 1
            while tiles * sp < 192 and sp * 2 <= ncb // 2 and sp < 16:
                sp *= 2
            p.tile, p.splits = 11, sp
        else:
            p.tile, p.splits = heuristic_plan(M, Cout, K, conv=True)
            if TILE_FORCE and TILE_FORCE < 10:
                p.tile = TILE_FORCE
    if p.tile == 13:
        if not phase_ok:
            raise ValueError("planes.conv3x3: this geometry has no phase form (tile 13)")
        p.splits = min(p.splits, (C1 + C2) // 32)
        wp = hip.x3_upsample_phase_planes(w, W_SCALE)
        if wp is None:
            raise RuntimeError("phase weight planes missing while capturing: run one eager forward first")
        K = 4 * (C1 + C2)
        p.K = K
    else:
        if p.tile in (11, 12):
            if not halo_ok:
                raise ValueError("planes.conv3x3: this geometry has no halo form (tile 11 / 12)")
            p.tile = 12 if upsample else 11
            p.splits = min(p.splits, (C1 + C2) // 32)
        wp = weight_planes(w)
    p.W, p.planeW, p.ldw = wp.data_ptr(), wp.stride(0), K
    ws = hip._fill_epilogue(p, hip._rows_ld32, "planes.conv3x3", M, Cout, x.device, bias, rowvec, g.rows_per_batch, residual, p.splits)
    nbytes = 4.0 * (B * Hp * Wp * (C1 + C2) + M * (CE1 + CE2) + Cout * K + M * Cout * ((1 if o32 is not None else 0) + (1 if op is not None else 0) + (1 if residual is not None else 0)))
    kn = "conv3x3_halo_x3p_kernel_phase" if p.tile == 13 else \
        f"conv3x3_halo_x3p_kernel<{'true' if upsample else 'false'}>" if p.tile in (11, 12) else f"igemm_x3p_kernel<true> t{p.tile}"
    kn += f" {M}x{Cout}x{K} s{p.splits}" if hip.PROF_SHAPES else ""
    if p.tile == 13:
        hip.note_staged(kn, 4.0 * (C1 + C2) * (4 * 80 + 256 + 2 * (Wp + 1)) * -(-(M // 4) // 256) * -(-Cout // 80) * 4)
    elif p.tile in (11, 12):
        hip.note_staged(kn, 4.0 * (C1 + C2) * (9 * 80 + 256 + 2 * (Wd + 1)) * -(-M // 256) * -(-Cout // 80))
    else:
        bm, bn = _TILES[p.tile]
        hip.note_staged(kn, 4.0 * K * (bm + bn) * -(-M // bm) * -(-Cout // bn))
    with _Timed(kn, 2.0 * M * Cout * K, nbytes):
        _check(lib.ief_gemm_x3p(byref(p), _stream()), "ief_gemm_x3p (conv)")
    return _ret(o32, op)


GN_SMALL_ELEMS = int(os.environ.get("IEF_GN_SMALL_ELEMS", str(3 << 20)))
GN_REG_MAX_HW = int(os.environ.get("IEF_GN_REG_MAX_HW", "1024"))
HALO = os.environ.get("IEF_X3P_HALO", "1") == "1"
ENABLED = os.environ.get("IEF_X3P", "1") == "1"


def groupnorm(x, gamma, beta, groups, eps, silu=False, x2=None, out32=False):
    lib = hip.load()
    if not hip._act32(x, "x").is_contiguous() or (x2 is not None and not hip._act32(x2, "x2").is_contiguous()):
        raise ValueError("planes.groupnorm: inputs must be contiguous")
    B, C1 = x.shape[0], x.shape[-1]
    C2 = 0 if x2 is None else x2.shape[-1]
    HW = x.numel() // (B * C1)
    out = Planes.empty(*x.shape[:-1], C1 + C2, device=x.device)
    cpg = (C1 + C2) // groups
    if HW <= GN_REG_MAX_HW and lib.ief_groupnorm_reg_fits(C1, C2, HW, groups):
        o32 = torch.empty(*x.shape[:-1], C1 + C2, dtype=torch.float32, device=x.device) if out32 else None
        with _Timed("groupnorm_reg_kernel", 0.0, (12.0 if out32 else 8.0) * (x.numel() + (0 if x2 is None else x2.numel()))):
            _check(lib.ief_groupnorm_silu_reg(x.data_ptr(), _ptr(x2), C1, C2, _ptr(o32), out.t.data_ptr(), out.plane,
                                              _dev32(gamma, "gamma").data_ptr(), _dev32(beta, "beta").data_ptr(), B, HW, groups,
                                              eps, 1 if silu else 0, _stream()), "ief_groupnorm_silu_reg")
        return (out, o32) if out32 else out
    if not out32 and HW <= GN_REG_MAX_HW and B * HW * (C1 + C2) <= GN_SMALL_ELEMS and cpg % 2 == 0 and C1 % 2 == 0 and cpg // 2 <= 256:
        with _Timed("groupnorm_f32_kernel", 0.0, 12.0 * (x.numel() + (0 if x2 is None else x2.numel()))):
            _check(lib.ief_groupnorm_silu_x3p_small(x.data_ptr(), _ptr(x2), C1, C2, out.t.data_ptr(), out.plane,
                                                    _dev32(gamma, "gamma").data_ptr(), _dev32(beta, "beta").data_ptr(), B, HW, groups,
                                                    eps, 1 if silu else 0, _stream()), "ief_groupnorm_silu_x3p_small")
        return out
    o32 = torch.empty(*x.shape[:-1], C1 + C2, dtype=torch.float32, device=x.device) if out32 else None
    nws = lib.ief_groupnorm_f32_ws_floats(B, HW, C1 + C2)
    ws = torch.empty(nws, dtype=torch.float32, device=x.device)
    with _Timed("gn3_f32 (stats + finalize + apply)", 0.0, 12.0 * (x.numel() + (0 if x2 is None else x2.numel()))):
        _check(lib.ief_groupnorm_silu_x3p_ws(x.data_ptr(), _ptr(x2), C1, C2, _ptr(o32), out.t.data_ptr(), out.plane,
                                             _dev32(gamma, "gamma").data_ptr(), _dev32(beta, "beta").data_ptr(), B, HW, groups, eps,
                                             1 if silu else 0, ws.data_ptr(), nws, _stream()), "ief_groupnorm_silu_x3p_ws")
    return (out, o32) if out32 else out


def layernorm(x, gamma, beta, eps=1e-5):
    lib = hip.load()
    if not hip._act32(x, "x").is_contiguous():
        raise ValueError("planes.layernorm: x must be contiguous")
    C = x.shape[-1]
    out = Planes.empty(*x.shape, device=x.device)
    with _Timed("layernorm_f32_vec_kernel", 0.0, 8.0 * x.numel()):
        _check(lib.ief_layernorm_x3p(x.data_ptr(), out.t.data_ptr(), out.plane, _dev32(gamma, "gamma").data_ptr(),
                                     _dev32(beta, "beta").data_ptr(), x.numel() // C, C, eps, _stream()), "ief_layernorm_x3p")
    return out


def attn_out_args(p, B, N, C, device, out32=False):
    op = Planes.empty(B, N, C, device=device)
    p.OutP, p.planeO, p.sOPb, p.ldp = op.t.data_ptr(), op.plane, N * C, C
    o32 = None
    if out32:
        o32 = torch.empty(B, N, C, dtype=torch.float32, device=device)
        p.Out, p.sOb, p.ldo = o32.data_ptr(), N * C, C
    return op, o32


FLASH_PLANES = os.environ.get("IEF_X3P_FLASH", "1") == "1"
FLASH_PLANES_DIMS = (40, 64, 80)
# ... 169 lines not shown
```

image-editing-framework_amd/unet.py:

```python
import math
import os
from typing import Dict, Optional

import torch
from torch import nn

from . import hip, planes
from .config import UNetConfig


FOLD_LN = os.environ.get("IEF_FOLD_LN", "1") == "1"
KV_ONE_GEMM = os.environ.get("IEF_KV_ONE_GEMM", "1") == "1"


def _fold_ln(w16, bias32, gamma, beta):
    wf = w16.float()
    wp = (wf * gamma[None, :]).half().contiguous()
    b = wf @ beta
    if bias32 is not None:
        b = b + bias32
    return wp, b.contiguous(), wp.float().sum(1).contiguous()


class UNetOutput(dict):
# ... 47 lines not shown

    def forward(self, x, silu=False, x2=None, return_stats=False, cstat=None, cstat2=None):
        return hip.groupnorm(x, self.weight, self.bias, self.num_groups, self.eps, silu=silu, x2=x2, return_stats=return_stats,
                             cstat=cstat, cstat2=cstat2)


class LayerNorm(nn.Module):
    def __init__(self, weight, bias, eps=1e-5):
        super().__init__()
        self.weight, self.bias, self.eps = weight, bias, eps

    def forward(self, x):
        return hip.layernorm(x, self.weight, self.bias, self.eps)


class SiLU(nn.Module):
    def forward(self, x):
        return hip.silu(x)


class Dropout(nn.Module):
    def forward(self, x):
        return x


class Attention(nn.Module):

    def __init__(self, sd, prefix, dim, heads, cross_dim, dev, name):
        super().__init__()
        self.heads = heads
        self.inner_dim = dim
        self.dim_head = dim // heads
        self.scale = self.dim_head ** -0.5
        self.is_cross = cross_dim is not None
        self.layer_name = name
        wq, wk, wv = (_f16(sd[f"{prefix}.to_{n}.weight"], dev) for n in "qkv")
        if self.is_cross:
            self.w_kv = torch.cat([wk, wv], 0).contiguous()
            self.to_q = Linear(wq)
            self.to_k, self.to_v = Linear(self.w_kv[:dim]), Linear(self.w_kv[dim:])
            self.w_qkv = None
        else:
            self.w_qkv = torch.cat([wq, wk, wv], 0).contiguous()
            self.to_q, self.to_k, self.to_v = (Linear(self.w_qkv[i * dim:(i + 1) * dim]) for i in range(3))
            self.w_kv = None
        self.to_out = nn.ModuleList([
            Linear(_f16(sd[f"{prefix}.to_out.0.weight"], dev), _f32(sd[f"{prefix}.to_out.0.bias"], dev)), Dropout()])
        self.spatial_norm = None
        self.group_norm = None
        self.norm_cross = None
        self.residual_connection = False
        self.rescale_output_factor = 1.0
        self.processor = None
        self._plan = None
        self.map_out = None
        self._kv_key, self._kv = None, None
        self.cache_kv = True
        self._kv_view = None
        self.ln_w = self.ln_b = self.ln_c1 = None
        self.ln_eps = 1e-5
        self.attn_key_splits = 1

    def fold_layernorm(self, norm):
        w = self.w_qkv if self.w_qkv is not None else self.to_q.weight
        self.ln_w, self.ln_b, self.ln_c1 = _fold_ln(w, None, norm.weight, norm.bias)
        self.ln_eps = norm.eps

    def prepare_attention_mask(self, attention_mask, target_length, batch_size, out_dim=3):
        if attention_mask is not None:
            raise NotImplementedError("attention masks are not on the reference path (always None)")
        return None

    def head_to_batch_dim(self, t, out_dim=3):
        B, L, _ = t.shape
        t = t.reshape(B, L, self.heads, self.dim_head).permute(0, 2, 1, 3)
        return t.reshape(B * self.heads, L, self.dim_head) if out_dim == 3 else t

    def batch_to_head_dim(self, t):
        BH, L, d = t.shape
        B = BH // self.heads
        return t.reshape(B, self.heads, L, d).permute(0, 2, 1, 3).reshape(B, L, self.heads * d)

    def get_attention_scores(self, query, key, attention_mask=None):
        if attention_mask is not None:
            raise NotImplementedError("attention masks are not on the reference path")
        q = self.batch_to_head_dim(query).contiguous()
        k = self.batch_to_head_dim(key).contiguous()
        return hip.attn_probs(q, k, self.heads, self.scale)

    def apply_probs(self, probs, value):
        v = self.batch_to_head_dim(value).contiguous()
        return hip.attn_apply(probs.contiguous(), v, self.heads)

    def get_processor(self):
        return self.processor

    def set_processor(self, processor):
        self.processor = processor

    def is_native(self) -> bool:
        f = self.__dict__.get("forward")
        return (f is None or getattr(f, "__func__", None) is Attention.forward) and self.processor is None

    def context_kv(self, ctx):
        if self._kv_view is not None:
            return self._kv_view
        if not self.cache_kv:
            return hip.gemm(ctx, self.w_kv)
        key = (ctx, ctx._version)
        if self._kv_key is None or self._kv_key[0] is not ctx or self._kv_key[1] != ctx._version:
            self._kv = hip.gemm(ctx, self.w_kv)
            self._kv_key = key
        return self._kv

    def forward(self, hidden_states, encoder_hidden_states=None, attention_mask=None, temb=None, residual=None,
                ln_stats=None, want_stats=False, **cross_attention_kwargs):
        if self.processor is not None:
            return self.processor(self, hidden_states, encoder_hidden_states=encoder_hidden_states,
                                  attention_mask=attention_mask, **cross_attention_kwargs)
        x = hidden_states
        B, N, C = x.shape
        self.last_tokens = N
        plan = self._plan
        ln = None if ln_stats is None else (ln_stats, self.ln_c1, self.ln_eps)
        if encoder_hidden_states is None:
            qkv = hip.gemm(x, self.w_qkv) if ln is None else hip.gemm(x, self.ln_w, bias=self.ln_b, ln=ln)
            q, k, v = qkv[..., :C], qkv[..., C:2 * C], qkv[..., 2 * C:]
            qs = ks = vs = None
            if plan is not None:
                qs, ks, vs = plan.self_sources(B, N, self)
                if plan.second_sources(B, self) is not None:
                    raise RuntimeError(f"{self.layer_name}: the Union plan's two key segments exist on the planes attention of the "
                                       "f16x3 mode only")
            o = hip.attn_flash(q, k, v, self.heads, self.scale, q_src=qs, k_src=ks, v_src=vs)
        else:
            q = hip.gemm(x, self.to_q.weight) if ln is None else hip.gemm(x, self.ln_w, bias=self.ln_b, ln=ln)
            kv = self.context_kv(encoder_hidden_states)
            args = plan.cross_edit(B, self) if plan is not None else {}
            if self.map_out is not None:
                hip.attn_probs(q, kv[..., :C], self.heads, self.scale, out=self.map_out)
            o = hip.attn_cross_p2p(q, kv[..., :C], kv[..., C:], self.heads, self.scale, **args)
        if plan is not None:
            plan.layer_done(self)
        lin = self.to_out[0]
        if want_stats:
            return hip.gemm(o, lin.weight, bias=lin.bias, residual=residual, row_stats=True)
        return lin(o, residual=residual)


    def fold_layernorm_x3p(self, norm):
        w = self.w_qkv if self.w_qkv is not None else self.to_q.weight
        self.ln3 = planes.FoldedLN(w, None, norm.weight, norm.bias, norm.eps)

    def forward_x3p(self, xp, ctx, residual, ln_stats=None, want_stats=False, cfg_rows=None):
        B, N, C = xp.shape
        if cfg_rows is not None:
            if cfg_rows.rows != B:
                raise ValueError("forward_x3p: cfg_rows was built for another batch")
            B = cfg_rows.n
        self.last_tokens = N
        plan = self._plan
        w_in, b_in, ln = (self.w_qkv if ctx is None else self.to_q.weight), None, None
        if ln_stats is not None:
            w_in, b_in, ln = self.ln3.w, self.ln3.bias, (ln_stats, self.ln3.colsum, self.ln3.eps)
        if ctx is None:
            qs = ks = vs = None
            if plan is not None:
                qs, ks, vs = plan.self_sources(B, N, self)
            if cfg_rows is not None and (qs is not None or ks is not None or vs is not None
                                         or (plan is not None and plan.mask_launches(B, N, self) is not None)
                                         or (plan is not None and plan.kind == "masactrl_mask_auto"
                                             and (self._exec_index // 2) in plan.masa_layers)):
                raise RuntimeError(f"{self.layer_name}: the control plan acts on a self-attention that runs in the shared prefix of a "
                                   "CFG step (ControlPlan.controls_first_self must say so)")
            if planes.FLASH_PLANES and self.dim_head in planes.FLASH_PLANES_DIMS:
                qkv = planes.gemm(xp, w_in, bias=b_in, ln=ln, out=False, out_planes=True)
                k2 = plan.second_sources(B, self) if plan is not None else None
                if k2 is not None:
                    o = planes.attn_flash(qkv[..., :C], qkv[..., C:2 * C], qkv[..., 2 * C:], self.heads, self.scale, q_src=qs,
                                          k_src=ks, v_src=vs, k2_src=k2, v2_src=k2, key_splits=1)
                else:
                    o = planes.attn_flash(qkv[..., :C], qkv[..., C:2 * C], qkv[..., 2 * C:], self.heads, self.scale, q_src=qs,
                                          k_src=ks, v_src=vs, key_splits=self.attn_key_splits)
                ml = plan.mask_launches(B, N, self) if plan is not None else None
                if ml is not None:
                    tgt, src, gate, pairs = ml
                    for q_idx, k_idx in pairs:
                        planes.attn_flash(qkv[..., :C], qkv[..., C:2 * C], qkv[..., 2 * C:], self.heads, self.scale, q_src=tgt,
                                          k_src=src, v_src=src, out_planes=o[1::2], q_idx=q_idx, k_idx=k_idx, gate=gate)
                al = plan.auto_launch(B, N, self) if plan is not None else None
                if al is not None:
                    tgt, src, gate, k_cls, q_cls = al
                    planes.attn_flash(qkv[..., :C], qkv[..., C:2 * C], qkv[..., 2 * C:], self.heads, self.scale, q_src=tgt,
                                      k_src=src, v_src=src, out_planes=o[1::2], q_cls=q_cls, k_cls=k_cls, gate=gate)
            else:
                qkv = planes.gemm(xp, w_in, bias=b_in, ln=ln)
                if plan is not None and (plan.mask_launches(B, N, self) is not None or plan.auto_launch(B, N, self) is not None):
                    raise RuntimeError(f"mask-guided MasaCtrl was lowered onto a layer of head dim {self.dim_head} that has no "
                                       "planes attention")
                if plan is not None and plan.second_sources(B, self) is not None:
                    raise RuntimeError(f"MasaCtrl Union was lowered onto a layer of head dim {self.dim_head} that has no planes "
                                       "attention")
                o = hip.attn_flash(qkv[..., :C], qkv[..., C:2 * C], qkv[..., 2 * C:], self.heads, self.scale, q_src=qs, k_src=ks,
                                   v_src=vs, out_planes=True)
        else:
            q = planes.gemm(xp, w_in, bias=b_in, ln=ln)
            kv = self.context_kv(ctx)
            args = plan.cross_edit(B, self) if plan is not None else {}
            if self.map_out is not None:
                hip.attn_probs(q, kv[..., :C], self.heads, self.scale, out=self.map_out)
            if plan is not None:
                plan.cross_mass(B, N, self, q, kv[..., :C])
            o = hip.attn_cross_p2p(q, kv[..., :C], kv[..., C:], self.heads, self.scale, out_planes=True, q_src=cfg_rows, **args)
        if plan is not None:
            plan.layer_done(self)
        lin = self.to_out[0]
        if want_stats:
            return planes.gemm(o, lin.weight, bias=lin.bias, residual=residual, out=True, out_planes=True, row_stats=True)
        return planes.gemm(o, lin.weight, bias=lin.bias, residual=residual)


class GEGLU(nn.Module):

    def __init__(self, sd, prefix, dev):
        super().__init__()
        w, b = sd[prefix + ".proj.weight"], sd[prefix + ".proj.bias"]
        half = w.shape[0] // 2
        il = lambda t: torch.stack([t[:half].reshape(half // 8, 8, *t.shape[1:]),
                                    t[half:].reshape(half // 8, 8, *t.shape[1:])], 1).reshape(t.shape)
        self.proj = Linear(_f16(il(w), dev), _f32(il(b), dev))
        self.proj.interleaved = True

    def fold_layernorm(self, norm):
        self.ln_w, self.ln_b, self.ln_c1 = _fold_ln(self.proj.weight, self.proj.bias, norm.weight, norm.bias)
        self.ln_eps = norm.eps

    def forward(self, x, ln_stats=None):
        if ln_stats is not None:
            return hip.gemm(x, self.ln_w, bias=self.ln_b, geglu=True, ln=(ln_stats, self.ln_c1, self.ln_eps))
        return hip.gemm(x, self.proj.weight, bias=self.proj.bias, geglu=True)


class FeedForward(nn.Module):
    def __init__(self, sd, prefix, dev):
        super().__init__()
        self.net = nn.ModuleList([GEGLU(sd, prefix + ".net.0", dev), Dropout(),
                                  Linear(_f16(sd[prefix + ".net.2.weight"], dev), _f32(sd[prefix + ".net.2.bias"], dev))])

    def forward(self, x, residual=None):
        return self.net[2](self.net[0](x), residual=residual)


class BasicTransformerBlock(nn.Module):
    def __init__(self, sd, prefix, dim, heads, cross_dim, dev, name):
        super().__init__()
        ln = lambda n: LayerNorm(_f32(sd[f"{prefix}.{n}.weight"], dev), _f32(sd[f"{prefix}.{n}.bias"], dev))
        self.norm1, self.norm2, self.norm3 = ln("norm1"), ln("norm2"), ln("norm3")
        self.attn1 = Attention(sd, prefix + ".attn1", dim, heads, None, dev, name + ".attn1")
        self.attn2 = Attention(sd, prefix + ".attn2", dim, heads, cross_dim, dev, name + ".attn2")
        self.ff = FeedForward(sd, prefix + ".ff", dev)
        if dev.type == "cuda" and _PACK == torch.float16:
            self.attn1.fold_layernorm(self.norm1)
            self.attn2.fold_layernorm(self.norm2)
            self.ff.net[0].fold_layernorm(self.norm3)

    def foldable(self):
        return FOLD_LN and self.attn1.ln_w is not None and self.attn1.is_native() and self.attn2.is_native()

    @staticmethod
    def _attend(attn, x, res, ctx):
        if attn.is_native():
            return attn(x, encoder_hidden_states=ctx, residual=res)
        out = attn(x, encoder_hidden_states=ctx)
        return hip.add(out.contiguous(), res)

    def forward(self, h, ctx, ln_stats=None, want_stats=False):
        if ln_stats is not None:
            h, st = self.attn1(h, residual=h, ln_stats=ln_stats, want_stats=True)
            h, st = self.attn2(h, encoder_hidden_states=ctx, residual=h, ln_stats=st, want_stats=True)
            g = self.ff.net[0](h, ln_stats=st)
            lin = self.ff.net[2]
            if want_stats:
                return hip.gemm(g, lin.weight, bias=lin.bias, residual=h, row_stats=True)
            return lin(g, residual=h)
        h = self._attend(self.attn1, self.norm1(h), h, None)
        h = self._attend(self.attn2, self.norm2(h), h, ctx)
        return self.ff(self.norm3(h), residual=h)


    def _attend_x3p(self, attn, norm, h, ctx):
        if attn.is_native():
            return attn.forward_x3p(planes.layernorm(h, norm.weight, norm.bias, norm.eps), ctx, residual=h)
        return self._attend(attn, norm(h), h, ctx)

    def fold_layernorm_x3p(self):
        self.attn1.fold_layernorm_x3p(self.norm1)
        self.attn2.fold_layernorm_x3p(self.norm2)
        f0 = self.ff.net[0].proj
        self.ff.net[0].ln3 = planes.FoldedLN(f0.weight, f0.bias, self.norm3.weight, self.norm3.bias, self.norm3.eps)

    def foldable_x3p(self):
        if not (planes.LN_FOLD and self.attn1.is_native() and self.attn2.is_native()):
            return False
        if getattr(self.attn1, "ln3", None) is None:
            if hip._capturing():
                return False
            self.fold_layernorm_x3p()
        return True

    def forward_x3p_folded(self, h, hp, st, ctx, last, want_stats):
        h, hp, st = self.attn1.forward_x3p(hp, None, residual=h, ln_stats=st, want_stats=True)
        h, hp, st = self.attn2.forward_x3p(hp, ctx, residual=h, ln_stats=st, want_stats=True)
        f0, lin = self.ff.net[0], self.ff.net[2]
        g = planes.gemm(hp, f0.ln3.w, bias=f0.ln3.bias, geglu=True, out=False, out_planes=True, ln=(st, f0.ln3.colsum, f0.ln3.eps))
        if last:
            return planes.gemm(g, lin.weight, bias=lin.bias, residual=h, out=False, out_planes=True)
        if want_stats:
            return planes.gemm(g, lin.weight, bias=lin.bias, residual=h, out=True, out_planes=True, row_stats=True)
        return planes.gemm(g, lin.weight, bias=lin.bias, residual=h)

    def forward_x3p(self, h, ctx, last, cfg_rows=None, carry=()):
        if cfg_rows is not None:
            h = self.attn1.forward_x3p(planes.layernorm(h, self.norm1.weight, self.norm1.bias, self.norm1.eps), None, residual=h,
                                       cfg_rows=cfg_rows)
            n2 = planes.layernorm(h, self.norm2.weight, self.norm2.bias, self.norm2.eps)
            rep = hip.repeat_batch(h, *carry)
            h, carry = (rep[0], tuple(rep[1:])) if carry else (rep, ())
            h = self.attn2.forward_x3p(n2, ctx, residual=h, cfg_rows=cfg_rows)
        else:
            h = self._attend_x3p(self.attn1, self.norm1, h, None)
            h = self._attend_x3p(self.attn2, self.norm2, h, ctx)
        n3 = planes.layernorm(h, self.norm3.weight, self.norm3.bias, self.norm3.eps)
        f0, lin = self.ff.net[0].proj, self.ff.net[2]
        g = planes.gemm(n3, f0.weight, bias=f0.bias, geglu=True, out=False, out_planes=True)
        if last:
            r = planes.gemm(g, lin.weight, bias=lin.bias, residual=h, out=False, out_planes=True)
        else:
            r = planes.gemm(g, lin.weight, bias=lin.bias, residual=h)
        return (r, carry) if cfg_rows is not None else r


class Transformer2DModel(nn.Module):
    def __init__(self, sd, prefix, dim, heads, cross_dim, groups, dev, name, depth=1):
        super().__init__()
        self.norm = GroupNorm(_f32(sd[prefix + ".norm.weight"], dev), _f32(sd[prefix + ".norm.bias"], dev), groups, 1e-6)
        c1 = lambda n: Conv2d(_f16(sd[f"{prefix}.{n}.weight"].reshape(dim, dim), dev), _f32(sd[f"{prefix}.{n}.bias"], dev), 1)
        self.proj_in, self.proj_out = c1("proj_in"), c1("proj_out")
        self.transformer_blocks = nn.ModuleList(
            [BasicTransformerBlock(sd, f"{prefix}.transformer_blocks.{k}", dim, heads, cross_dim, dev,
                                   name if k == 0 else f"{name}.b{k}") for k in range(depth)])

    def forward(self, x, encoder_hidden_states=None, cstat=None, col_stats=False):
        B, H, W, C = x.shape
        if all(blk.foldable() for blk in self.transformer_blocks):
            h, st = hip.gemm(self.norm(x, cstat=cstat), self.proj_in.weight, bias=self.proj_in.bias, row_stats=True)
            h = h.reshape(B, H * W, C)
            last = len(self.transformer_blocks) - 1
            for k, blk in enumerate(self.transformer_blocks):
                if k < last:
                    h, st = blk(h, encoder_hidden_states, ln_stats=st, want_stats=True)
                else:
                    h = blk(h, encoder_hidden_states, ln_stats=st)
            return self.proj_out(h.reshape(B, H, W, C), residual=x, col_stats=col_stats)
        h = self.proj_in(self.norm(x, cstat=cstat)).reshape(B, H * W, C)
        for blk in self.transformer_blocks:
            h = blk(h, encoder_hidden_states)
        return self.proj_out(h.reshape(B, H, W, C), residual=x, col_stats=col_stats)


    def forward_x3p(self, x, encoder_hidden_states=None, want_planes=False, cfg_rows=None, carry=()):
        B, H, W, C = x.shape
        n = self.norm
        hn = planes.groupnorm(x, n.weight, n.bias, n.num_groups, n.eps, silu=False)
        last = len(self.transformer_blocks) - 1
        if cfg_rows is not None:
            h = planes.gemm(hn.reshape(B, H * W, C), self.proj_in.weight, bias=self.proj_in.bias)
            for k, blk in enumerate(self.transformer_blocks):
                if k == 0:
                    h, rep = blk.forward_x3p(h, encoder_hidden_states, last=(k == last), cfg_rows=cfg_rows, carry=(x,) + tuple(carry))
                    x, carry = rep[0], rep[1:]
                    B = x.shape[0]
                else:
                    h = blk.forward_x3p(h, encoder_hidden_states, last=(k == last))
        elif all(blk.foldable_x3p() for blk in self.transformer_blocks):
            h, hp, st = planes.gemm(hn.reshape(B, H * W, C), self.proj_in.weight, bias=self.proj_in.bias, out=True, out_planes=True,
                                    row_stats=True)
            for k, blk in enumerate(self.transformer_blocks):
                r = blk.forward_x3p_folded(h, hp, st, encoder_hidden_states, last=(k == last), want_stats=(k < last))
                if k < last:
                    h, hp, st = r
                else:
                    h = r
        else:
            h = planes.gemm(hn.reshape(B, H * W, C), self.proj_in.weight, bias=self.proj_in.bias)
            for k, blk in enumerate(self.transformer_blocks):
                h = blk.forward_x3p(h, encoder_hidden_states, last=(k == last))
        r = planes.gemm(h, self.proj_out.weight, bias=self.proj_out.bias, residual=x.reshape(B, H * W, C), out=True,
                        out_planes=want_planes)
        if want_planes:
            r = r[0].reshape(B, H, W, C), r[1].reshape(B, H, W, C)
        else:
            r = r.reshape(B, H, W, C), None
        return r + (tuple(carry),) if cfg_rows is not None else r


class ResnetBlock2D(nn.Module):

    def __init__(self, sd, prefix, cin, cout, groups, eps, dev, temb_slot):
        super().__init__()
        self.in_channels, self.out_channels = cin, cout
        self.norm1 = GroupNorm(_f32(sd[prefix + ".norm1.weight"], dev), _f32(sd[prefix + ".norm1.bias"], dev), groups, eps)
        self.norm2 = GroupNorm(_f32(sd[prefix + ".norm2.weight"], dev), _f32(sd[prefix + ".norm2.bias"], dev), groups, eps)
        pack = lambda w: _f16(w.permute(0, 2, 3, 1), dev)
        self.conv1 = Conv2d(pack(sd[prefix + ".conv1.weight"]), _f32(sd[prefix + ".conv1.bias"], dev), 3)
        self.time_emb_proj = Linear(_f16(sd[prefix + ".time_emb_proj.weight"], dev), _f32(sd[prefix + ".time_emb_proj.bias"], dev))
        self.nonlinearity = SiLU()
        self.dropout = Dropout()
        self.upsample = self.downsample = None
        self.skip_time_act = False
        self.time_embedding_norm = "default"
        self.output_scale_factor = 1.0
        w2 = sd[prefix + ".conv2.weight"].permute(0, 2, 3, 1).reshape(cout, 9 * cout)
        b2 = sd[prefix + ".conv2.bias"]
        if cin != cout:
            ws = sd[prefix + ".conv_shortcut.weight"].reshape(cout, cin)
            self.conv_shortcut = Conv2d(_f16(ws, dev), _f32(sd[prefix + ".conv_shortcut.bias"], dev), 1)
            self.w2_fused = _f16(torch.cat([w2, ws], 1), dev)
            self.b2_fused = _f32(b2 + sd[prefix + ".conv_shortcut.bias"], dev)
        else:
            self.conv_shortcut = None
            self.w2_fused, self.b2_fused = None, None
        self.conv2 = Conv2d(_f16(w2.reshape(cout, 3, 3, cout), dev), _f32(b2, dev), 3)
        self.temb_slot = temb_slot
        self._inject = None

    def forward(self, x, temb_row, skip=None, cstat=None, cstat_skip=None, col_stats=False):
        h = self.norm1(x, silu=True, x2=skip, cstat=cstat, cstat2=cstat_skip)
        h, hs = hip.conv3x3(h, self.conv1.weight, self.conv1.bias, rowvec=temb_row, col_stats=True)
        h = self.norm2(h, silu=True, cstat=hs)
        if self._inject is not None:
            src = self._inject.feature_source(h.shape[0])
            if src is not None:
                h = hip.gather_rows(h, src)
        if self.conv_shortcut is None:
            return hip.conv3x3(h, self.conv2.weight, self.conv2.bias, residual=x, col_stats=col_stats)
        return hip.conv3x3_shortcut(h, self.w2_fused, self.b2_fused, x, skip, col_stats=col_stats)


    def forward_x3p(self, x, xp, temb_row, skip=None, skip_p=None, want_planes=False):
        n1, n2 = self.norm1, self.norm2
        g1 = planes.groupnorm(x, n1.weight, n1.bias, n1.num_groups, n1.eps, silu=True, x2=skip)
        h = planes.conv3x3(g1, self.conv1.weight, self.conv1.bias, rowvec=temb_row)
        if self._inject is not None and self._inject.feature_source(h.shape[0]) is not None:
            g2 = planes.split(hip.gather_rows(hip.groupnorm(h, n2.weight, n2.bias, n2.num_groups, n2.eps, silu=True),
                                              self._inject.feature_source(h.shape[0])))
        else:
            g2 = planes.groupnorm(h, n2.weight, n2.bias, n2.num_groups, n2.eps, silu=True)
        if self.conv_shortcut is None:
            r = planes.conv3x3(g2, self.conv2.weight, self.conv2.bias, residual=x, out=True, out_planes=want_planes)
        else:
            xp = planes.split(x) if xp is None else xp
            if skip is not None and skip_p is None:
                skip_p = planes.split(skip)
            r = planes.conv3x3(g2, self.w2_fused, self.b2_fused, extra=(xp, skip_p), out=True, out_planes=want_planes)
        return r if want_planes else (r, None)


class Downsample2D(nn.Module):
    def __init__(self, sd, prefix, dev):
        super().__init__()
        self.conv = Conv2d(_f16(sd[prefix + ".conv.weight"].permute(0, 2, 3, 1), dev), _f32(sd[prefix + ".conv.bias"], dev), 3, stride=2)

    def forward(self, x, col_stats=False):
        return self.conv(x, col_stats=col_stats)

    def forward_x3p(self, xp, want_planes=True):
        r = planes.conv3x3(xp, self.conv.weight, self.conv.bias, stride=2, out=True, out_planes=want_planes)
        return r if want_planes else (r, None)


class Upsample2D(nn.Module):

    def __init__(self, sd, prefix, dev):
        super().__init__()
        self.conv = Conv2d(_f16(sd[prefix + ".conv.weight"].permute(0, 2, 3, 1), dev), _f32(sd[prefix + ".conv.bias"], dev), 3)

    def forward(self, x, col_stats=False):
        return hip.conv3x3(x, self.conv.weight, self.conv.bias, upsample=True, col_stats=col_stats)

    def forward_x3p(self, xp, want_planes=True):
        r = planes.conv3x3(xp, self.conv.weight, self.conv.bias, upsample=True, out=True, out_planes=want_planes)
        return r if want_planes else (r, None)


class _Block(nn.Module):
    def __init__(self):
        super().__init__()
        self.resnets = nn.ModuleList()
        self.attentions = nn.ModuleList()
        self.has_cross_attention = False


class CrossAttnDownBlock2D(_Block):
    pass


class DownBlock2D(_Block):
    pass


class CrossAttnUpBlock2D(_Block):
    pass


class UpBlock2D(_Block):
    pass


class UNetMidBlock2DCrossAttn(_Block):
    pass


class Timesteps(nn.Module):
    def __init__(self, dim):
        super().__init__()
        self.num_channels = dim
        self.dtype = _PACK

    def forward(self, t):
        return hip.timestep_embedding(t, self.num_channels, dtype=self.dtype)


class TimestepEmbedding(nn.Module):
    def __init__(self, sd, dev, prefix="time_embedding"):
        super().__init__()
        self.linear_1 = Linear(_f16(sd[prefix + ".linear_1.weight"], dev), _f32(sd[prefix + ".linear_1.bias"], dev))
        self.act = SiLU()
        self.linear_2 = Linear(_f16(sd[prefix + ".linear_2.weight"], dev), _f32(sd[prefix + ".linear_2.bias"], dev))

    def forward(self, x):
        return self.linear_2(self.act(self.linear_1(x)))


class UNet2DConditionModel(nn.Module):
    def __init__(self, cfg: UNetConfig, state_dict: Dict[str, torch.Tensor], device="cuda:0", precision: str = "f16",
                 attn_key_splits=1):
        super().__init__()
        global _PACK
        if precision not in ("f16", "f32", "f16x3"):
# ... 335 lines not shown
```

include/ief_hip.h:

```cpp
#ifndef IEF_HIP_H
#define IEF_HIP_H
#include <stdint.h>

#ifdef __HIPCC__
typedef _Float16 ief_half;
#else
typedef uint16_t ief_half;
#endif

#ifdef __cplusplus
extern "C" {
#endif

#define IEF_ABI_VERSION 4
int ief_abi_version(void);
const char* ief_target_arch(void);
int ief_struct_size(int which);

typedef struct IefGemmParams {
    const ief_half* A;
    const ief_half* A2;
    const ief_half* W;
    ief_half* Out;
    const float* bias;
// ... 37 lines not shown
                           const float* gamma, const float* beta, float* partial,
                           int B, int HW, int groups, float eps, int apply_silu, void* stream);
int ief_layernorm_f16(const ief_half* x, ief_half* out, const float* gamma, const float* beta,
                      int rows, int C, float eps, void* stream);
int ief_geglu_f16(const ief_half* in, ief_half* out, int rows, int Ch, void* stream);

typedef struct IefAttnParams {
    const ief_half* Q; const ief_half* K; const ief_half* V; ief_half* Out;
    int B, heads, N, L, d;
    int ldq, ldk, ldv, ldo;
    float scale;
    const int* q_src; const int* k_src; const int* v_src;
    float* lse;
    int variant;
} IefAttnParams;
int ief_attn_flash_f16(const IefAttnParams* p, void* stream);

typedef struct IefCrossParams {
    const ief_half* Q; const ief_half* K; const ief_half* V; ief_half* Out;
    int B, heads, N, L, d;
    int ldq, ldk, ldv, ldo;
    float scale;
    const int* edit_src; const int* edit_slot;
    const ief_half* MT; const float* coef;
} IefCrossParams;
int ief_attn_cross_p2p_f16(const IefCrossParams* p, void* stream);

int ief_attn_probs_f16(const IefAttnParams* p, ief_half* probs, void* stream);
int ief_attn_apply_f16(const IefAttnParams* p, const ief_half* probs, void* stream);

int ief_cfg_ddim_step_f32(const float* eps_u, const float* eps_c, const float* x, float* x_out,
                          float* x0_out, const float* coef, long long n, void* stream);
int ief_timestep_embedding_f16(const float* t, ief_half* out, int B, int dim, void* stream);
int ief_add_f16(const ief_half* a, const ief_half* b, ief_half* out, long long n, void* stream);
int ief_gather_rows_f16(const ief_half* in, ief_half* out, const int* src, int B, long long row_elems, void* stream);
int ief_softmax_rows_f16(ief_half* x, int rows, int L, void* stream);
int ief_transpose_f16(const ief_half* in, ief_half* out, int R, int C, void* stream);
int ief_pointwise_f32(const float* x, const float* w, const float* bias, float* out, int B, int Cin, int Cout, int HW,
                      void* stream);
int ief_silu_f16(const ief_half* x, ief_half* out, long long n, void* stream);
int ief_cast_f32_to_f16(const float* x, ief_half* out, long long n, void* stream);
int ief_cast_f16_to_f32(const ief_half* x, float* out, long long n, void* stream);
int ief_select_step(const void* table, void* out, const int* step, long long bytes_per_step, int n_rows, void* stream);
int ief_advance_step(int* step, void* stream);

typedef struct IefGemmF32Params {
    const float* A;
    const float* A2;
    const float* W;
    float* Out;
    const float* bias;
    const float* rowvec;
    const float* residual;
    int M, N, K;
    int lda, ldw, ldo, ldr;
    int rows_per_batch;
    float out_scale;
    int conv, H, Wd, C1, C2, Ho, Wo, stride, ups, batch_images, pad_hi_only;
    const float* E1;
    const float* E2;
    int CE1, CE2;
    int batch, heads;
    long long sAb, sAh, sWb, sWh, sOb, sOh;
    const int* a_src;
    const int* w_src;
    int transb;
    int a_scalar;
    int splits;
    float* ws;
    int x3;
    float sa, sb;
    int vec_out, al32, fast_ok;
    unsigned bytesA, bytesW, bytesA2, bytesE1, bytesE2;
    const void* Wp;
    int geglu;
} IefGemmF32Params;
int ief_gemm_f32(const IefGemmF32Params* p, void* stream);
int ief_x3_split_weights(const float* w, void* planes, long long n, float scale, void* stream);
int ief_gemm_x3_bn(int N);
int ief_gemm_x3_bm(int M, int N);
int ief_gemm_x3_bn_k(int conv, int N, int K);
void ief_gemm_x3_set_variant(int bits);
int ief_gemm_f32_bn(int N);
typedef struct IefAttnF32Params {
    const float* Q; const float* K; const float* V; float* Out;
    int B, heads, N, L, d;
    int ldq, ldk, ldv, ldo;
    long long sQb, sKb, sVb, sOb;
    float scale;
    const int* q_src; const int* k_src; const int* v_src;
    int x3;
    ief_half* OutP;
    long long planeO, sOPb;
    int ldp;
    float p_scale;
    const ief_half* Qp; const ief_half* Kp; const ief_half* Vp;
    long long planeQ, planeK, planeV;
    const void* zeros;
    float* lse;
    int key_splits; float* ws; long long ws_floats;
    const int* k2_src; const int* v2_src;
    const unsigned* k_cls; const unsigned* q_cls;
    const int* q_idx; const int* k_idx; const int* gate;
} IefAttnF32Params;
int ief_attn_flash_f32(const IefAttnF32Params* p, void* stream);
int ief_cross_token_mass_f32(const float* q, const float* k, const float* w, float* out, int row_ref, int row_cur, int heads,
                             int N, int L, int d, int ldq, int ldk, long long sQb, long long sKb, float scale, void* stream);
int ief_masa_auto_classes(const float* slots, int c, const float* thres, int res, unsigned* k_cls, unsigned* q_cls,
                          const int* gate, void* stream);
int ief_cross_blend_mass_f32(const float* q, const float* k, const float* w, float* acc, int row0, int Bp, int heads, int N, int L,
                             int ldw, int d, int ldq, int ldk, long long sQb, long long sKb, float scale, void* stream);
int ief_local_blend_f32(const float* acc, const float* thres, float* x, int Bp, int C, int H, int W, void* stream);
long long ief_attn_flash_ws_floats(int B, int heads, int N, int L, int d, int key_splits);
int ief_softmax_rows_f32(float* x, long long rows, int L, void* stream);
int ief_p2p_cross_edit_f32(float* P, const int* edit_src, const int* edit_slot, const float* MT, const float* coef, int B,
                           int heads, int N, int L, void* stream);
int ief_attn_cross_p2p_f32(const IefAttnF32Params* p, const int* edit_src, const int* edit_slot, const float* MT, const float* coef,
                           void* stream);
int ief_groupnorm_silu_f32(const float* x, const float* x2, int C1, int C2, float* out, const float* gamma, const float* beta,
                           int B, int HW, int groups, float eps, int silu, void* stream);
long long ief_groupnorm_f32_ws_floats(int B, int HW, int C);
int ief_groupnorm_silu_f32_ws(const float* x, const float* x2, int C1, int C2, float* out, const float* gamma, const float* beta,
                              int B, int HW, int groups, float eps, int silu, float* ws, long long ws_floats, void* stream);
int ief_groupnorm_reg_fits(int C1, int C2, int HW, int groups);
int ief_groupnorm_silu_reg(const float* x, const float* x2, int C1, int C2, float* out, ief_half* outp, long long plane,
                           const float* gamma, const float* beta, int B, int HW, int groups, float eps, int silu, void* stream);
long long ief_groupnorm_bwd_f32_ws_floats(int B, int HW, int C);
int ief_groupnorm_bwd_f32_ws(const float* x, const float* x2, int C1, int C2, const float* dy, const float* add, float* dx, float* dx2,
                             const float* gamma, const float* beta, int B, int HW, int groups, float eps, int silu, float* ws,
                             long long ws_floats, void* stream);
int ief_layernorm_f32(const float* x, float* out, const float* gamma, const float* beta, long long rows, int C, float eps,
                      void* stream);
int ief_groupnorm_silu_x3p_ws(const float* x, const float* x2, int C1, int C2, float* out, ief_half* outp, long long plane,
                              const float* gamma, const float* beta, int B, int HW, int groups, float eps, int silu, float* ws,
                              long long ws_floats, void* stream);
int ief_groupnorm_silu_x3p_small(const float* x, const float* x2, int C1, int C2, ief_half* outp, long long plane, const float* gamma,
                                 const float* beta, int B, int HW, int groups, float eps, int silu, void* stream);
int ief_layernorm_x3p(const float* x, ief_half* outp, long long plane, const float* gamma, const float* beta, long long rows, int C,
                      float eps, void* stream);
int ief_add_f32(const float* a, const float* b, float* out, long long n, void* stream);
int ief_silu_f32(const float* x, float* out, long long n, void* stream);
int ief_geglu_il_f32(const float* pre, float* out, long long rows, int Ch, void* stream);
int ief_timestep_embedding_f32(const float* t, float* out, int B, int dim, void* stream);
int ief_gather_rows_f32(const float* in, float* out, const int* src, int B, long long row_elems, void* stream);
int ief_conv_in_f32act(const float* x, const float* w, const float* bias, float* out, int B, int Cin, int H, int Wd, int Cout,
                       void* stream);
int ief_conv_out_f32act(const float* x, const float* w, const float* bias, float* out, int B, int C, int H, int Wd, int Cout,
                        void* stream);
int ief_conv_in_f32act_planes(const float* x, const float* w, const float* bias, float* out, ief_half* outp, long long plane, int B,
                              int Cin, int H, int Wd, int Cout, void* stream);
#define IEF_REPEAT_MAX_JOBS 4
typedef struct IefRepeatJob { const void* src; void* dst; long long bytes; int blocks; } IefRepeatJob;
int ief_repeat_batch(const IefRepeatJob* jobs, int njobs, void* stream);
int ief_image_u8(const float* x, unsigned char* out, int B, int C, int H, int Wd, void* stream);

typedef struct IefGemmX3pParams {
    const ief_half* A;  long long planeA;
    const ief_half* A2; long long planeA2;
    const ief_half* E1; long long planeE1;
    const ief_half* E2; long long planeE2;
    const ief_half* W;  long long planeW;
    float* Out;
    ief_half* OutP; long long planeO;
    const float* bias;
    const float* rowvec;
    const float* residual;
    int M, N, K;
    int lda, ldw, ldo, ldp, ldr;
    int conv, H, Wd, C1, C2, Ho, Wo, stride, ups, batch_images, pad_hi_only, CE1, CE2;
    int rows_per_batch;
    float out_scale;
    float inv_scale;
    int tile;
    int splits;
    float* ws;
    int geglu;
    const void* zeros;
    float* rstat_out;
    float* cstat_out;
    const float* rstat_in;
    const float* colsum;
    int rstat_slots, rstat_cnt;
    float ln_eps;
} IefGemmX3pParams;
int ief_gemm_x3p(const IefGemmX3pParams* p, void* stream);
int ief_x3_upsample_phase_weights(const float* w, void* planes, int Cout, int C, float scale, void* stream);
int ief_gemm_x3p_tile_bm(int tile);
int ief_gemm_x3p_tile_bn(int tile);
int ief_gemm_x3p_tile_wn(int tile);
int ief_x3_split_act(const float* x, ief_half* planes, long long plane, long long rows, int C, int ldx, int ldp, float scale,
                     void* stream);

int ief_groupnorm_bwd_f32(const float* x, const float* x2, int C1, int C2, const float* dy, const float* add, float* dx, float* dx2,
                          const float* gamma, const float* beta, int B, int HW, int groups, float eps, int silu, void* stream);
int ief_layernorm_bwd_f32(const float* x, const float* dy, const float* add, float* dx, const float* gamma, long long rows, int C,
                          float eps, void* stream);
int ief_geglu_il_bwd_f32(const float* pre, const float* dy, float* dpre, long long rows, int Ch, void* stream);
int ief_zero_insert2x_f32(const float* in, float* out, int B, int H, int W, int C, void* stream);
int ief_pool2x2_sum_f32(const float* in, float* out, int B, int H, int W, int C, void* stream);
int ief_conv_out_bwd_f32w(const float* d_eps, const float* w, float* dh, int B, int C, int H, int W, int Cout, void* stream);
int ief_softmax_bwd_rows_f32(const float* P, float* dP, long long rows, int L, float scale, void* stream);
int ief_transpose_batched_f32(const float* in, float* out, int R, int N, int L, void* stream);
int ief_map_loss_rows_blocks(long long rows);
int ief_map_loss_rows_f32(const float* P, const float* ref, float* dP, float* loss, long long rows, int L, float gcoef,
                          float loss_coef, void* stream);
int ief_nti_adam_f32g(float* param, float* m, float* v, const float* grad, const float* stats, const float* hyper, int* step, int n,
                      void* stream);

typedef struct IefAttnBwdParams {
    const ief_half* Q; const ief_half* K; const ief_half* V; const ief_half* dO;
    const float* lse;
    const float* delta;
    ief_half* dQ; ief_half* dK; ief_half* dV;
    int B, heads, N, L, d;
    int ldq, ldk, ldv, ldo, lddq, lddk, lddv;
    float scale;
    float ds_mul;
    int kv_splits;
    float* ws;
} IefAttnBwdParams;
int ief_attn_bwd_delta_f32(const ief_half* O, const ief_half* dO, float* delta, int B, int heads, int N, int d,
                           int ldo, int lddo, void* stream);
int ief_attn_bwd_f16(const IefAttnBwdParams* p, int what, void* stream);
typedef struct IefAttnBwdF32Params {
    const float* Q; const float* K; const float* V; const float* dO;
    const float* lse;
    const float* delta;
    float* dQ; float* dK; float* dV;
    int B, heads, N, L, d;
    int ldq, ldk, ldv, ldo, lddq, lddk, lddv;
    float scale;
    float ds_mul;
} IefAttnBwdF32Params;
int ief_attn_bwd_delta_f32in(const float* O, const float* dO, float* delta, int B, int heads, int N, int d, int ldo, int lddo,
                             void* stream);
int ief_attn_bwd_x3(const IefAttnBwdF32Params* p, int what, void* stream);
typedef struct IefMapLossParams {
    const ief_half* Q; const ief_half* K; const ief_half* ref;
    ief_half* dQ;
    float* loss;
    int B, heads, N, L, d;
    int ldq, ldk, lddq;
    float scale, gcoef, loss_coef;
    int accumulate;
} IefMapLossParams;
int ief_attn_map_loss_bwd_f16(const IefMapLossParams* p, void* stream);
int ief_map_loss_blocks(int N, int d);
#define IEF_CROSS_MAP_GRAD_MAX_L 106
int ief_attn_cross_map_grad_f32(const float* Q, const float* K, const float* V, const float* dO, const float* ref, float* dQ,
                                float* loss, int B, int heads, int N, int L, int d, int ldq, int ldk, int ldv, int ldo, int lddq,
                                float scale, float gcoef, float loss_coef, void* stream);
int ief_cross_map_grad_blocks(int N, int d);
int ief_axpy_f32(float* y, const float* x, float a, long long n, void* stream);
int ief_groupnorm_cstat_f16(const ief_half* x, const ief_half* x2, int C1, int C2, ief_half* out, const float* gamma,
                            const float* beta, const float* cstat1, int bm1, const float* cstat2, int bm2, float* stats,
                            int B, int HW, int groups, float eps, int apply_silu, void* stream);
int ief_gemm_tile_bm(int tile_hint);
int ief_groupnorm_bwd_f16(const ief_half* x, const ief_half* x2, int C1, int C2, const ief_half* dy, const ief_half* add,
                          ief_half* dx, ief_half* dx2, const float* gamma, const float* beta, const float* stats,
                          float* partial, int B, int HW, int groups, float eps, int apply_silu, void* stream);
int ief_layernorm_bwd_f16(const ief_half* x, const ief_half* dy, const ief_half* add, ief_half* dx, const float* gamma,
                          int rows, int C, float eps, void* stream);
int ief_geglu_il_f16(const ief_half* pre, ief_half* out, int rows, int Ch, void* stream);
int ief_geglu_il_bwd_f16(const ief_half* pre, const ief_half* dy, ief_half* dpre, int rows, int Ch, void* stream);
int ief_zero_insert2x_f16(const ief_half* in, ief_half* out, int B, int H, int W, int C, void* stream);
int ief_pool2x2_sum_f16(const ief_half* in, ief_half* out, int B, int H, int W, int C, void* stream);
int ief_conv_out_bwd_f32(const float* d_eps, const ief_half* w, ief_half* dh, int B, int C, int H, int W, int Cout,
                         void* stream);
int ief_nti_loss_grad_f32(const float* eps_u, const float* eps_c, const float* x, const float* target, const float* coef,
                          float* d_eps, float* stats, int n, float grad_scale, void* stream);
int ief_nti_adam_f32(float* param, float* m, float* v, const ief_half* grad16, const float* stats, const float* hyper,
                     int* step, ief_half* param16, int n, void* stream);
int ief_nti_loss_grad_batched_f32(const float* eps_u, const float* eps_c, const float* x, const float* target, const float* coef,
                                  float* d_eps, float* stats, int n, int K, float grad_scale, void* stream);
int ief_nti_adam_batched_f32(float* param, float* m, float* v, const ief_half* grad16, const float* stats, const int* active,
                             const float* hyper, int* step, ief_half* param16, int n, int K, void* stream);
int ief_nti_adam_batched_f32g(float* param, float* m, float* v, const float* grad, const float* stats, const int* active,
                              const float* hyper, int* step, int n, int K, void* stream);

#ifdef __cplusplus
}
#endif
#endif
```

Before: 78.34 steps/s.

## Fuse LayerNorm into split-K reduce, batch step selects, widen conv_out blocks

Adds a split-K reduction kernel that also applies the next LayerNorm and writes its hi/lo fp16 planes. This removes separate layernorm launches after the attention output and proj_in GEMMs. It also merges the per-step table select launches (timestep embedding, coefficients, context, controller tables) into one multi-job kernel, and lets conv_out use 1024-thread blocks so the weights are loaded into LDS fewer times. The costs are more code paths, more registers in the fused reduce, and a requirement that controller selects run ahead of the UNet forward.

```diff
diff --git a/image-editing-framework_amd/control.py b/image-editing-framework_amd/control.py
--- a/image-editing-framework_amd/control.py
+++ b/image-editing-framework_amd/control.py
@@ -58,6 +58,7 @@
         self.muted = False
         dev = self.device
         self.step = torch.zeros(1, dtype=torch.int32, device=dev)
+        self._selects_ahead = False
         B, Bp = self.batch, num_prompts
         self.blend_modules = ()
         self.blend_w = self.blend_w_cur = self.blend_acc = self.blend_thres = None
@@ -397,9 +398,10 @@
                 f"called with batch {B}; the reference's AttentionControlEdit.forward would mis-reshape here")
         return True
 
-    def begin_forward(self, B: int):
+    def step_selects(self, B: int):
+        jobs = []
         if not self.applies(B):
-            return
+            return jobs
         if not self.captured:
             cs = int(self.controller.cur_step)
             if cs > self.num_steps and self.kind == "p2p":
@@ -407,10 +409,10 @@
             self.step.fill_(cs)
             self._rewound(cs)
         if self.kind == "p2p":
-            hip.select_step(self.coef_table, self.coef_cur, self.step)
-            hip.select_step(self.self_table, self.self_cur, self.step)
+            jobs.append((self.coef_table, self.coef_cur, self.step))
+            jobs.append((self.self_table, self.self_cur, self.step))
             if self.blend_w is not None:
-                hip.select_step(self.blend_w, self.blend_w_cur, self.step)
+                jobs.append((self.blend_w, self.blend_w_cur, self.step))
         elif self.kind in self.MASA_KINDS:
             if B not in self._masa:
                 if self.captured:
@@ -419,11 +421,11 @@
             tab, cur = self._masa[B]
             if not self.captured and int(self.controller.cur_step) >= tab.shape[0]:
                 self.step.fill_(tab.shape[0] - 1)
-            hip.select_step(tab, cur, self.step)
+            jobs.append((tab, cur, self.step))
             if self.kind in self.GATED_KINDS:
-                hip.select_step(self._gate[0], self._gate[1], self.step)
+                jobs.append((self._gate[0], self._gate[1], self.step))
             if self.kind == "masactrl_union":
-                hip.select_step(self._union[B][0], self._union[B][1], self.step)
+                jobs.append((self._union[B][0], self._union[B][1], self.step))
         elif self.kind == "pnp":
             if B not in self._pnp:
                 if self.captured:
@@ -432,8 +434,22 @@
             qk, qk_cur, cv, cv_cur = self._pnp[B]
             if not self.captured and int(self.controller.cur_step) >= qk.shape[0]:
                 self.step.fill_(qk.shape[0] - 1)
-            hip.select_step(qk, qk_cur, self.step)
-            hip.select_step(cv, cv_cur, self.step)
+            jobs.append((qk, qk_cur, self.step))
+            jobs.append((cv, cv_cur, self.step))
+        return jobs
+
+    def selects_ahead(self, B: int):
+        jobs = self.step_selects(B)
+        self._selects_ahead = True
+        return jobs
+
+    def begin_forward(self, B: int):
+        if self._selects_ahead:
+            self._selects_ahead = False
+            return
+        jobs = self.step_selects(B)
+        if jobs:
+            hip.select_steps(jobs)
 
     def end_forward(self, B: int):
         if (self.kind in self.MASA_KINDS or self.kind == "pnp") and not self.muted:
diff --git a/image-editing-framework_amd/csrc/elementwise.hip b/image-editing-framework_amd/csrc/elementwise.hip
--- a/image-editing-framework_amd/csrc/elementwise.hip
+++ b/image-editing-framework_amd/csrc/elementwise.hip
@@ -285,6 +285,37 @@
     return IEF_OK;
 }
 
+struct SelectJob { const uint32_t* table; uint32_t* out; const int* step; long long words; int n_rows; };
+struct SelectJobs { SelectJob j[IEF_SELECT_MAX_JOBS]; };
+__global__ __launch_bounds__(256) void select_steps_kernel(const SelectJobs jobs) {
+    const SelectJob jb = jobs.j[blockIdx.y];
+    int row = jb.step[0];
+    row = row < 0 ? 0 : (row >= jb.n_rows ? jb.n_rows - 1 : row);
+    const long long base = (long long)row * jb.words;
+    for (long long i = (long long)blockIdx.x * 256 + threadIdx.x; i < jb.words; i += (long long)gridDim.x * 256)
+        jb.out[i] = jb.table[base + i];
+}
+extern "C" int ief_select_steps(const long long* jobs, int njobs, void* stream) {
+    if (!jobs) return IEF_EINVAL;
+    if (njobs <= 0 || njobs > IEF_SELECT_MAX_JOBS) return IEF_ESHAPE;
+    SelectJobs a = {};
+    long long most = 0;
+    for (int i = 0; i < njobs; ++i) {
+        const long long* w = jobs + (long long)i * IEF_SELECT_JOB_WORDS;
+        const long long bytes = w[3], rows = w[4];
+        if (!w[0] || !w[1] || !w[2]) return IEF_EINVAL;
+        if (rows <= 0 || rows > 0x7fffffffll) return IEF_ESHAPE;
+        if (bytes <= 0 || (bytes & 3)) return IEF_EALIGN;
+        a.j[i] = SelectJob{(const uint32_t*)(uintptr_t)w[0], (uint32_t*)(uintptr_t)w[1], (const int*)(uintptr_t)w[2], bytes / 4, (int)rows};
+        most = bytes / 4 > most ? bytes / 4 : most;
+    }
+    long long grid = (most + 255) / 256;
+    if (grid > 1024) grid = 1024;
+    hipLaunchKernelGGL(select_steps_kernel, dim3((unsigned)grid, (unsigned)njobs), dim3(256), 0, (hipStream_t)stream, a);
+    IEF_LAUNCH_CHECK();
+    return IEF_OK;
+}
+
 __global__ void advance_step_kernel(int* step) { if (threadIdx.x == 0 && blockIdx.x == 0) step[0] += 1; }
 extern "C" int ief_advance_step(int* step, void* stream) {
     if (!step) return IEF_EINVAL;
diff --git a/image-editing-framework_amd/csrc/exact_f32.hip b/image-editing-framework_amd/csrc/exact_f32.hip
--- a/image-editing-framework_amd/csrc/exact_f32.hip
+++ b/image-editing-framework_amd/csrc/exact_f32.hip
@@ -1518,22 +1518,15 @@
     }
 }
 template <int CH>
-__global__ __launch_bounds__(256) void conv_out_f32_lds_kernel(const float* __restrict__ x, const float* __restrict__ w,
-                                                               const float* __restrict__ bias, float* __restrict__ out, int B, int C,
-                                                               int H, int Wd, int Cout) {
-    extern __shared__ __attribute__((aligned(16))) float wl_f32[];
-    const int sub = threadIdx.x & 15;
-    const long long pix = (long long)blockIdx.x * 16 + (threadIdx.x >> 4);
-    const long long total = (long long)B * H * Wd;
+__device__ __forceinline__ void conv_out_f32_lds_group(const float* __restrict__ x, const float* wl_f32, const float* __restrict__ bias,
+                                                       float* __restrict__ out, long long total, int C, int H, int Wd, int Cout,
+                                                       long long pix) {
+    const int sub = threadIdx.x & 15, C4 = C >> 2;
     const bool live = pix < total;
     const long long pc = live ? pix : 0;
     const int b = (int)(pc / (H * Wd));
     const int rem = (int)(pc - (long long)b * H * Wd);
     const int oy = rem / Wd, ox = rem - oy * Wd;
-    const int C4 = C >> 2;
-    const int nw4 = (Cout * 9 * C) >> 2;
-    for (int i = threadIdx.x; i < nw4; i += 256) ((f32x4*)wl_f32)[i] = ((const f32x4*)w)[i];
-    __syncthreads();
     float acc[8];
 #pragma unroll
     for (int o = 0; o < 8; ++o) acc[o] = 0.f;
@@ -1582,6 +1575,18 @@
     if (live && sub == 0) {
         for (int o = 0; o < Cout; ++o) out[(((long long)b * Cout + o) * H + oy) * Wd + ox] = acc[o] + (bias ? bias[o] : 0.f);
     }
+}
+template <int CH>
+__global__ __launch_bounds__(1024) void conv_out_f32_lds_kernel(const float* __restrict__ x, const float* __restrict__ w,
+                                                                const float* __restrict__ bias, float* __restrict__ out, int B, int C,
+                                                                int H, int Wd, int Cout) {
+    extern __shared__ __attribute__((aligned(16))) float wl_f32[];
+    const long long total = (long long)B * H * Wd;
+    const int nw4 = (Cout * 9 * C) >> 2;
+    for (int i = threadIdx.x; i < nw4; i += blockDim.x) ((f32x4*)wl_f32)[i] = ((const f32x4*)w)[i];
+    __syncthreads();
+    conv_out_f32_lds_group<CH>(x, wl_f32, bias, out, total, C, H, Wd, Cout,
+                               (long long)blockIdx.x * (blockDim.x >> 4) + (threadIdx.x >> 4));
 }
 extern "C" int ief_conv_out_f32act(const float* x, const float* w, const float* bias, float* out, int B, int C, int H, int Wd,
                                    int Cout, void* stream) {
@@ -1592,8 +1597,10 @@
     const size_t lds = (size_t)Cout * 9 * C * sizeof(float);
     const dim3 grid((unsigned)((total + 15) / 16));
     if (lds <= 48 * 1024 && C <= 320 && Cout <= 4) {
-        if (C <= 128) hipLaunchKernelGGL(conv_out_f32_lds_kernel<2>, grid, dim3(256), lds, (hipStream_t)stream, x, w, bias, out, B, C, H, Wd, Cout);
-        else hipLaunchKernelGGL(conv_out_f32_lds_kernel<5>, grid, dim3(256), lds, (hipStream_t)stream, x, w, bias, out, B, C, H, Wd, Cout);
+        const int threads = total >= 64 * 256 ? 1024 : 256;
+        const dim3 lgrid((unsigned)((total * 16 + threads - 1) / threads));
+        if (C <= 128) hipLaunchKernelGGL(conv_out_f32_lds_kernel<2>, lgrid, dim3(threads), lds, (hipStream_t)stream, x, w, bias, out, B, C, H, Wd, Cout);
+        else hipLaunchKernelGGL(conv_out_f32_lds_kernel<5>, lgrid, dim3(threads), lds, (hipStream_t)stream, x, w, bias, out, B, C, H, Wd, Cout);
     } else {
         hipLaunchKernelGGL(conv_out_f32_kernel, grid, dim3(256), 0, (hipStream_t)stream, x, w, bias, out, B, C, H, Wd, Cout);
     }
diff --git a/image-editing-framework_amd/csrc/gemm_x3p.hip b/image-editing-framework_amd/csrc/gemm_x3p.hip
--- a/image-editing-framework_amd/csrc/gemm_x3p.hip
+++ b/image-editing-framework_amd/csrc/gemm_x3p.hip
@@ -408,6 +408,84 @@
     }
 }
 
+__device__ __forceinline__ f32x4 xp_as_loaded(f32x4 v) {
+    float a = v[0], b = v[1], c = v[2], d = v[3];
+    asm volatile("" : "+v"(a), "+v"(b), "+v"(c), "+v"(d));
+    return f32x4{a, b, c, d};
+}
+template <int NV>
+__global__ __launch_bounds__(256) void x3p_reduce_ln_kernel(const IefGemmX3pParams p) {
+    const int m = blockIdx.x * 4 + (threadIdx.x >> 6);
+    if (m >= p.M) return;
+    const int lane = threadIdx.x & 63, NQ = p.N >> 2;
+    const long long slab = (long long)p.M * p.N;
+    constexpr int U = NV > 5 ? 2 : 4;
+    const f32x4 zero = f32x4{0.f, 0.f, 0.f, 0.f};
+    const float* w = p.ws + (long long)m * p.N + lane * 4;
+    f32x4 v[NV], eb[NV], er[NV];
+#pragma unroll
+    for (int j = 0; j < NV; ++j) {
+        const bool ok = lane + 64 * j < NQ;
+        eb[j] = (ok && p.bias) ? *(const f32x4*)(p.bias + lane * 4 + 256 * j) : zero;
+        er[j] = (ok && p.residual) ? *(const f32x4*)(p.residual + (long long)m * p.ldr + lane * 4 + 256 * j) : zero;
+        v[j] = ok ? *(const f32x4*)(w + 256 * j) : zero;
+    }
+    int s = 1;
+    for (; s + U - 1 < p.splits; s += U) {
+        f32x4 t[U][NV];
+#pragma unroll
+        for (int u = 0; u < U; ++u)
+#pragma unroll
+            for (int j = 0; j < NV; ++j) t[u][j] = lane + 64 * j < NQ ? *(const f32x4*)(w + (s + u) * slab + 256 * j) : zero;
+#pragma unroll
+        for (int u = 0; u < U; ++u)
+#pragma unroll
+            for (int j = 0; j < NV; ++j) v[j] += t[u][j];
+    }
+    for (; s < p.splits; ++s) {
+        f32x4 t[NV];
+#pragma unroll
+        for (int j = 0; j < NV; ++j) t[j] = lane + 64 * j < NQ ? *(const f32x4*)(w + s * slab + 256 * j) : zero;
+#pragma unroll
+        for (int j = 0; j < NV; ++j) v[j] += t[j];
+    }
+    float sum = 0.f;
+#pragma unroll
+    for (int j = 0; j < NV; ++j) {
+        if (lane + 64 * j < NQ) v[j] = xp_as_loaded(xp_store_loaded(p, v[j], eb[j], er[j], m, lane * 4 + 256 * j));
+        sum += (v[j][0] + v[j][1]) + (v[j][2] + v[j][3]);
+    }
+    f32x4 g[NV], bt[NV];
+#pragma unroll
+    for (int j = 0; j < NV; ++j) {
+        const bool ok = lane + 64 * j < NQ;
+        g[j] = ok ? *(const f32x4*)(p.lnt_gamma + lane * 4 + 256 * j) : zero;
+        bt[j] = ok ? *(const f32x4*)(p.lnt_beta + lane * 4 + 256 * j) : zero;
+    }
+    const float mean = wave_sum(sum) / (float)p.N;
+    float q = 0.f;
+#pragma unroll
+    for (int j = 0; j < NV; ++j) {
+        if (lane + 64 * j < NQ) {
+            const f32x4 d = v[j] - mean;
+            q += (d[0] * d[0] + d[1] * d[1]) + (d[2] * d[2] + d[3] * d[3]);
+        }
+    }
+    const float rstd = 1.0f / sqrtf(wave_sum(q) / (float)p.N + p.lnt_eps);
+#pragma unroll
+    for (int j = 0; j < NV; ++j) {
+        const int qd = lane + 64 * j;
+        if (qd < NQ) {
+            const f32x4 y = (v[j] - mean) * rstd * g[j] + bt[j];
+            half4 h, l;
+            split4(y, 1.0f, h, l);
+            half_t* op = p.LnP + (long long)m * p.ldl + qd * 4;
+            *(half4*)op = h;
+            *(half4*)(op + p.planeLn) = l;
+        }
+    }
+}
+
 __global__ __launch_bounds__(256) void x3_split_act_kernel(const float* __restrict__ x, half_t* __restrict__ planes, long long plane,
                                                            long long rows, int C4, int ldx, int ldp, float scale) {
     const long long total = rows * C4;
@@ -483,6 +561,12 @@
     if (p.rstat_out && (p.splits > 1 || p.geglu || p.tile == 11 || p.tile == 12 || p.tile == 13 || (p.N % ief_gemm_x3p_tile_wn(p.tile)))) return IEF_EINVAL;
     if (p.rstat_in && (!p.colsum || p.rstat_slots <= 0 || p.rstat_cnt <= 0 || p.rstat_slots * p.rstat_cnt != p.K || p.splits > 1 ||
                        p.conv || !(p.ln_eps > 0.f) || ((uintptr_t)p.colsum & 15))) return IEF_EINVAL;
+    if (p.LnP) {
+        if (p.splits <= 1 || p.geglu || p.rstat_out || p.rstat_in || p.cstat_out || !p.lnt_gamma || !p.lnt_beta || !(p.lnt_eps > 0.f))
+            return IEF_EINVAL;
+        if (p.N > 2560) return IEF_ESHAPE;
+        if ((((uintptr_t)p.lnt_gamma | (uintptr_t)p.lnt_beta) & 15) || ((uintptr_t)p.LnP & 7) || (p.ldl & 3) || (p.planeLn & 3)) return IEF_EALIGN;
+    }
     if (p.conv) {
         if (p.C1 <= 0 || p.C2 < 0 || (p.C1 % XP_BK) || (p.C2 % XP_BK) || (p.CE1 % XP_BK) || (p.CE2 % XP_BK)) return IEF_ESHAPE;
         if ((p.C2 > 0 && !p.A2) || (p.CE1 > 0 && !p.E1) || (p.CE2 > 0 && !p.E2) || (p.CE2 > 0 && p.CE1 == 0)) return IEF_EINVAL;
@@ -514,7 +598,13 @@
         case 1: default: rc = launch_x3p<128, 160, 4, 2, 4, 0>(p, st); break;
     }
     if (rc) return rc;
-    if (p.splits > 1) {
+    if (p.splits > 1 && p.LnP) {
+        const dim3 grid((unsigned)((p.M + 3) / 4));
+        if (p.N <= 512) hipLaunchKernelGGL(x3p_reduce_ln_kernel<2>, grid, dim3(256), 0, st, p);
+        else if (p.N <= 1280) hipLaunchKernelGGL(x3p_reduce_ln_kernel<5>, grid, dim3(256), 0, st, p);
+        else hipLaunchKernelGGL(x3p_reduce_ln_kernel<10>, grid, dim3(256), 0, st, p);
+        IEF_LAUNCH_CHECK();
+    } else if (p.splits > 1) {
         const long long total = (long long)p.M * (p.N / 4);
         int grid = (int)((total + 255) / 256);
         if (grid > 8192) grid = 8192;
diff --git a/image-editing-framework_amd/csrc/x3p_common.h b/image-editing-framework_amd/csrc/x3p_common.h
--- a/image-editing-framework_amd/csrc/x3p_common.h
+++ b/image-editing-framework_amd/csrc/x3p_common.h
@@ -19,6 +19,22 @@
     if (p.bias) v += *(const f32x4*)(p.bias + n);
     if (p.rowvec) v += *(const f32x4*)(p.rowvec + (long long)(m / p.rows_per_batch) * p.N + n);
     if (p.residual) v += *(const f32x4*)(p.residual + (long long)m * p.ldr + n);
+    v = v * p.out_scale;
+    if (p.Out) *(f32x4*)(p.Out + (long long)m * p.ldo + n) = v;
+    if (p.OutP) {
+        half4 h, l;
+        split4(v, 1.0f, h, l);
+        half_t* o = p.OutP + (long long)m * p.ldp + n;
+        *(half4*)o = h;
+        *(half4*)(o + p.planeO) = l;
+    }
+    return v;
+}
+
+__device__ __forceinline__ f32x4 xp_store_loaded(const IefGemmX3pParams& p, f32x4 v, f32x4 b, f32x4 r, int m, int n) {
+    if (p.bias) v += b;
+    if (p.rowvec) v += *(const f32x4*)(p.rowvec + (long long)(m / p.rows_per_batch) * p.N + n);
+    if (p.residual) v += r;
     v = v * p.out_scale;
     if (p.Out) *(f32x4*)(p.Out + (long long)m * p.ldo + n) = v;
     if (p.OutP) {
diff --git a/image-editing-framework_amd/denoise.py b/image-editing-framework_amd/denoise.py
--- a/image-editing-framework_amd/denoise.py
+++ b/image-editing-framework_amd/denoise.py
@@ -146,11 +146,17 @@
         self.step.zero_()
         self._done = 0
 
+    def _select_rows(self):
+        jobs = [(self.temb_table, self.temb_cur, self.step), (self.coef_table, self.coef_cur, self.step)]
+        if self.ctx_table is not None:
+            jobs.append((self.ctx_table, self.ctx, self.step))
+        plan = self.unet._plan
+        if plan is not None:
+            jobs += plan.selects_ahead(self.B)
+        hip.select_steps(jobs)
+
     def _step_body(self):
-        hip.select_step(self.temb_table, self.temb_cur, self.step)
-        hip.select_step(self.coef_table, self.coef_cur, self.step)
-        if self.ctx_table is not None:
-            hip.select_step(self.ctx_table, self.ctx, self.step)
+        self._select_rows()
         if self.cfg and self.shared:
             eps = self.unet(self.lat, encoder_hidden_states=self.ctx, temb_row=self.temb_cur, cfg_pair=True)["sample"]
         else:
@@ -308,10 +314,7 @@
         self.coef_table[:, 2] = self._guidance
 
     def _forward_part(self):
-        hip.select_step(self.temb_table, self.temb_cur, self.step)
-        hip.select_step(self.coef_table, self.coef_cur, self.step)
-        if self.ctx_table is not None:
-            hip.select_step(self.ctx_table, self.ctx, self.step)
+        self._select_rows()
         eps = self.unet(self.lat, encoder_hidden_states=self.ctx, temb_row=self.temb_cur)["sample"]
         self.eps_mine.copy_(eps)
 
diff --git a/image-editing-framework_amd/hip.py b/image-editing-framework_amd/hip.py
--- a/image-editing-framework_amd/hip.py
+++ b/image-editing-framework_amd/hip.py
@@ -9,6 +9,7 @@
 
 ABI_VERSION = cabi.defines["IEF_ABI_VERSION"]
 REPEAT_MAX_JOBS = cabi.defines["IEF_REPEAT_MAX_JOBS"]
+SELECT_MAX_JOBS, SELECT_JOB_WORDS = cabi.defines["IEF_SELECT_MAX_JOBS"], cabi.defines["IEF_SELECT_JOB_WORDS"]
 _LIB_PATH = os.environ.get("IEF_HIP_LIB") or os.path.join(os.path.dirname(os.path.abspath(__file__)), "libief_hip.so")
 _lib = None
 
@@ -1490,6 +1491,21 @@
     return out
 
 
+def select_steps(jobs):
+    lib = load()
+    jobs = list(jobs)
+    if not 1 <= len(jobs) <= SELECT_MAX_JOBS:
+        raise ValueError(f"select_steps: 1 .. {SELECT_MAX_JOBS} jobs per launch")
+    words = (ctypes.c_longlong * (SELECT_JOB_WORDS * len(jobs)))()
+    for i, (table, out, step) in enumerate(jobs):
+        nbytes = out.numel() * out.element_size()
+        if table[0].numel() * table.element_size() != nbytes or not table.is_contiguous() or not out.is_contiguous():
+            raise ValueError("select_steps: table[step] and out must have identical contiguous byte size")
+        words[SELECT_JOB_WORDS * i:SELECT_JOB_WORDS * (i + 1)] = [table.data_ptr(), out.data_ptr(), _devi32(step, "step").data_ptr(),
+                                                                 nbytes, table.shape[0]]
+    _check(lib.ief_select_steps(words, len(jobs), _stream()), "ief_select_steps")
+
+
 def advance_step(step):
     lib = load()
     _check(lib.ief_advance_step(_devi32(step, "step").data_ptr(), _stream()), "ief_advance_step")
diff --git a/image-editing-framework_amd/planes.py b/image-editing-framework_amd/planes.py
--- a/image-editing-framework_amd/planes.py
+++ b/image-editing-framework_amd/planes.py
@@ -251,7 +251,7 @@
 
 
 def gemm(a, w, bias=None, residual=None, rowvec=None, rows_per_batch=0, out=None, out_planes=None, out_scale=1.0,
-         geglu=False, tile=0, splits=0, row_stats=False, ln=None):
+         geglu=False, tile=0, splits=0, row_stats=False, ln=None, ln_out=None):
     lib = hip.load()
     if not isinstance(a, Planes):
         raise TypeError("planes.gemm: a must be Planes")
@@ -279,6 +279,23 @@
         p.tile, p.splits = pick_plan(M, N, K, variant="|g" if geglu else "")
     if geglu or row_stats or ln is not None:
         p.splits = 1
+    lnp = None
+    if ln_out is not None:
+        if geglu or row_stats or ln is not None:
+            raise ValueError("planes.gemm: ln_out goes with a plain epilogue (no GEGLU, row statistics or folded LayerNorm)")
+        gamma, beta, eps = ln_out
+        if N > 2560:
+            raise ValueError("planes.gemm: ln_out takes rows of up to 2560 columns")
+    ln_src = None
+    if ln_out is not None and p.splits <= 1:
+        ln_src = o32
+        if ln_src is None:
+            ln_src = torch.empty(*a.shape[:-1], N, dtype=torch.float32, device=a.device)
+            p.Out, p.ldo = ln_src.data_ptr(), N
+    elif ln_out is not None:
+        lnp = Planes.empty(*a.shape[:-1], N, device=a.device)
+        p.LnP, p.planeLn, p.ldl = lnp.t.data_ptr(), lnp.plane, N
+        p.lnt_gamma, p.lnt_beta, p.lnt_eps = _dev32(gamma, "gamma").data_ptr(), _dev32(beta, "beta").data_ptr(), eps
     rs = None
     if row_stats:
         wn = lib.ief_gemm_x3p_tile_wn(p.tile)
@@ -301,6 +318,10 @@
     r = _ret(o32, op)
     if row_stats:
         return (r + (rs,)) if isinstance(r, tuple) else (r, rs)
+    if ln_out is not None:
+        if ln_src is not None:
+            lnp = layernorm(ln_src, gamma, beta, eps)
+        return (r + (lnp,)) if isinstance(r, tuple) else (r, lnp)
     return r
 
 
diff --git a/image-editing-framework_amd/unet.py b/image-editing-framework_amd/unet.py
--- a/image-editing-framework_amd/unet.py
+++ b/image-editing-framework_amd/unet.py
@@ -223,7 +223,7 @@
         w = self.w_qkv if self.w_qkv is not None else self.to_q.weight
         self.ln3 = planes.FoldedLN(w, None, norm.weight, norm.bias, norm.eps)
 
-    def forward_x3p(self, xp, ctx, residual, ln_stats=None, want_stats=False, cfg_rows=None):
+    def forward_x3p(self, xp, ctx, residual, ln_stats=None, want_stats=False, cfg_rows=None, ln_next=None):
         B, N, C = xp.shape
         if cfg_rows is not None:
             if cfg_rows.rows != B:
@@ -288,6 +288,8 @@
         lin = self.to_out[0]
         if want_stats:
             return planes.gemm(o, lin.weight, bias=lin.bias, residual=residual, out=True, out_planes=True, row_stats=True)
+        if ln_next is not None:
+            return planes.gemm(o, lin.weight, bias=lin.bias, residual=residual, ln_out=(ln_next.weight, ln_next.bias, ln_next.eps))
         return planes.gemm(o, lin.weight, bias=lin.bias, residual=residual)
 
 
@@ -359,10 +361,14 @@
         return self.ff(self.norm3(h), residual=h)
 
 
-    def _attend_x3p(self, attn, norm, h, ctx):
+    def _attend_x3p(self, attn, norm, h, ctx, n, ln_next, cfg_rows=None):
         if attn.is_native():
-            return attn.forward_x3p(planes.layernorm(h, norm.weight, norm.bias, norm.eps), ctx, residual=h)
-        return self._attend(attn, norm(h), h, ctx)
+            if n is None:
+                n = planes.layernorm(h, norm.weight, norm.bias, norm.eps)
+            r = attn.forward_x3p(n, ctx, residual=h, cfg_rows=cfg_rows, ln_next=ln_next)
+            return r if ln_next is not None else (r, None)
+        h = self._attend(attn, norm(h), h, ctx)
+        return h, (None if ln_next is None else planes.layernorm(h, ln_next.weight, ln_next.bias, ln_next.eps))
 
     def fold_layernorm_x3p(self):
         self.attn1.fold_layernorm_x3p(self.norm1)
@@ -390,18 +396,16 @@
             return planes.gemm(g, lin.weight, bias=lin.bias, residual=h, out=True, out_planes=True, row_stats=True)
         return planes.gemm(g, lin.weight, bias=lin.bias, residual=h)
 
-    def forward_x3p(self, h, ctx, last, cfg_rows=None, carry=()):
+    def forward_x3p(self, h, ctx, last, cfg_rows=None, carry=(), n1=None):
+        ln2 = self.norm2 if self.attn2.is_native() else None
         if cfg_rows is not None:
-            h = self.attn1.forward_x3p(planes.layernorm(h, self.norm1.weight, self.norm1.bias, self.norm1.eps), None, residual=h,
-                                       cfg_rows=cfg_rows)
-            n2 = planes.layernorm(h, self.norm2.weight, self.norm2.bias, self.norm2.eps)
+            h, n2 = self._attend_x3p(self.attn1, self.norm1, h, None, n1, ln2, cfg_rows=cfg_rows)
             rep = hip.repeat_batch(h, *carry)
             h, carry = (rep[0], tuple(rep[1:])) if carry else (rep, ())
-            h = self.attn2.forward_x3p(n2, ctx, residual=h, cfg_rows=cfg_rows)
+            h, n3 = self._attend_x3p(self.attn2, self.norm2, h, ctx, n2, self.norm3, cfg_rows=cfg_rows)
         else:
-            h = self._attend_x3p(self.attn1, self.norm1, h, None)
-            h = self._attend_x3p(self.attn2, self.norm2, h, ctx)
-        n3 = planes.layernorm(h, self.norm3.weight, self.norm3.bias, self.norm3.eps)
+            h, n2 = self._attend_x3p(self.attn1, self.norm1, h, None, n1, ln2)
+            h, n3 = self._attend_x3p(self.attn2, self.norm2, h, ctx, n2, self.norm3)
         f0, lin = self.ff.net[0].proj, self.ff.net[2]
         g = planes.gemm(n3, f0.weight, bias=f0.bias, geglu=True, out=False, out_planes=True)
         if last:
@@ -444,11 +448,15 @@
         n = self.norm
         hn = planes.groupnorm(x, n.weight, n.bias, n.num_groups, n.eps, silu=False)
         last = len(self.transformer_blocks) - 1
+        b0 = self.transformer_blocks[0]
+        ln1 = (b0.norm1.weight, b0.norm1.bias, b0.norm1.eps) if b0.attn1.is_native() else None
         if cfg_rows is not None:
-            h = planes.gemm(hn.reshape(B, H * W, C), self.proj_in.weight, bias=self.proj_in.bias)
+            h = planes.gemm(hn.reshape(B, H * W, C), self.proj_in.weight, bias=self.proj_in.bias, ln_out=ln1)
+            h, n1 = h if ln1 is not None else (h, None)
             for k, blk in enumerate(self.transformer_blocks):
                 if k == 0:
-                    h, rep = blk.forward_x3p(h, encoder_hidden_states, last=(k == last), cfg_rows=cfg_rows, carry=(x,) + tuple(carry))
+                    h, rep = blk.forward_x3p(h, encoder_hidden_states, last=(k == last), cfg_rows=cfg_rows, carry=(x,) + tuple(carry),
+                                             n1=n1)
                     x, carry = rep[0], rep[1:]
                     B = x.shape[0]
                 else:
@@ -463,9 +471,10 @@
                 else:
                     h = r
         else:
-            h = planes.gemm(hn.reshape(B, H * W, C), self.proj_in.weight, bias=self.proj_in.bias)
+            h = planes.gemm(hn.reshape(B, H * W, C), self.proj_in.weight, bias=self.proj_in.bias, ln_out=ln1)
+            h, n1 = h if ln1 is not None else (h, None)
             for k, blk in enumerate(self.transformer_blocks):
-                h = blk.forward_x3p(h, encoder_hidden_states, last=(k == last))
+                h = blk.forward_x3p(h, encoder_hidden_states, last=(k == last), n1=n1 if k == 0 else None)
         r = planes.gemm(h, self.proj_out.weight, bias=self.proj_out.bias, residual=x.reshape(B, H * W, C), out=True,
                         out_planes=want_planes)
         if want_planes:
diff --git a/include/ief_hip.h b/include/ief_hip.h
--- a/include/ief_hip.h
+++ b/include/ief_hip.h
@@ -213,6 +213,9 @@
 #define IEF_REPEAT_MAX_JOBS 4
 typedef struct IefRepeatJob { const void* src; void* dst; long long bytes; int blocks; } IefRepeatJob;
 int ief_repeat_batch(const IefRepeatJob* jobs, int njobs, void* stream);
+#define IEF_SELECT_MAX_JOBS 8
+#define IEF_SELECT_JOB_WORDS 5
+int ief_select_steps(const long long* jobs, int njobs, void* stream);
 int ief_image_u8(const float* x, unsigned char* out, int B, int C, int H, int Wd, void* stream);
 
 typedef struct IefGemmX3pParams {
@@ -243,6 +246,11 @@
     const float* colsum;
     int rstat_slots, rstat_cnt;
     float ln_eps;
+    const float* lnt_gamma;
+    const float* lnt_beta;
+    ief_half* LnP; long long planeLn;
+    int ldl;
+    float lnt_eps;
 } IefGemmX3pParams;
 int ief_gemm_x3p(const IefGemmX3pParams* p, void* stream);
 int ief_x3_upsample_phase_weights(const float* w, void* planes, int Cout, int C, float scale, void* stream);
```

Measured after the change: 78.65 steps/s, median of 6. Within noise of the previous version (+0.4%).
